# patrikhuber/superviseddescent

Hardware: AMD Instinct MI355X
Metric: faces/sec RCR-22 detect (batch 4096) (higher is better)
Workload: dtype f32; 1 GPU; RCR-22 detect, batch 4096 synthetic 256x256 u8 faces per GPU, 4 cascade levels (UoCTTI HOG 5x5 cells, cell 11/10/8/6, 4 orientations, F=8801, M=44), model trained on-GPU on 100000 synthetic faces (shipped .bin absent from the reference checkout); batch_per_gpu=4096, levels=4

## Files before the change

include/sdm.h:

```cpp
#ifndef SDM_H_
#define SDM_H_

#include <stddef.h>
#include <stdint.h>

#ifdef __cplusplus
extern "C" {
#endif

#define SDM_OK 0
#define SDM_ERR_INVALID (-1)
#define SDM_ERR_NO_DEVICE (-2)
#define SDM_ERR_HIP (-3)
#define SDM_ERR_EMPTY_PATCH (-4)
#define SDM_ERR_NOT_SPD (-5)
#define SDM_ERR_COMM (-6)

#define SDM_VARIANT_DALALTRIGGS 0
#define SDM_VARIANT_UOCTTI 1

#define SDM_REG_MANUAL 0
#define SDM_REG_MATRIX_NORM 1

typedef struct sdm_hog_param {
// ... 68 lines not shown
typedef int (*sdm_allreduce_fn)(void* dev_ptr, size_t count_f32, void* hip_stream, void* user);
int sdm_set_allreduce(sdm_ctx* ctx, sdm_allreduce_fn fn, void* user, int world_size);
int sdm_set_allreduce_rccl(sdm_ctx* ctx, void* nccl_comm, void* nccl_allreduce_fn, int world_size);
int sdm_allreduce_gram_rhs(sdm_ctx* ctx);
typedef int (*sdm_bcast_fn)(void* dev_ptr, size_t count_f32, int root, void* hip_stream, void* user);
typedef int (*sdm_allgather_fn)(const void* send_ptr, void* recv_ptr, size_t count_f32, void* hip_stream, void* user);
int sdm_set_solve_sharding(sdm_ctx* ctx, int rank, int world_size, sdm_bcast_fn bcast, sdm_allgather_fn allgather, void* user);
int sdm_set_solve_sharding_rccl(sdm_ctx* ctx, void* nccl_comm, int rank, int world_size, void* nccl_broadcast_fn,
                                void* nccl_allgather_fn);
typedef int (*sdm_reduce_scatter_fn)(const void* send_ptr, void* recv_ptr, size_t count_f32, void* hip_stream, void* user);
int sdm_set_reduce_scatter(sdm_ctx* ctx, sdm_reduce_scatter_fn fn, void* user);
int sdm_set_reduce_scatter_rccl(sdm_ctx* ctx, int enable, void* nccl_reduce_scatter_fn);
int sdm_solve(sdm_ctx* ctx, int level, int reg_type, float reg_param, int regularise_last_row,
              long long n_train_global, float* R_host, float* lambda_out);
#define SDM_SOLVER_CHOLESKY 0
#define SDM_SOLVER_COLPIV_QR 1
int sdm_set_solver(sdm_ctx* ctx, int solver);
int sdm_last_rank(sdm_ctx* ctx, int* rank, int* full_rank);
int sdm_solve_normal_equations(sdm_ctx* ctx, const float* A_host, int n_rows, int n_features,
                               const float* b_host, int n_outputs, int reg_type, float reg_param,
                               int regularise_last_row, float* R_host, float* lambda_out);
int sdm_solve_normal_equations_with(sdm_ctx* ctx, int solver, const float* A_host, int n_rows, int n_features,
                                    const float* b_host, int n_outputs, int reg_type, float reg_param,
                                    int regularise_last_row, float* R_host, float* lambda_out, int* rank, int* full_rank);
int sdm_train_level(sdm_ctx* ctx, int level, int reg_type, float reg_param, int regularise_last_row,
                    long long n_train_global);

int sdm_train_level_sweep(sdm_ctx* ctx, int level, int reg_type, const float* reg_params, int K, int regularise_last_row,
                          long long n_train_global, int n_fit_rows, double* holdout_err , double* fit_err ,
                          float* lambdas , int* status , int* best);
int sdm_sweep_get_regressor(sdm_ctx* ctx, int k, float* R_host);

int sdm_gram_device_ptr(sdm_ctx* ctx, void** dev_ptr, size_t* count_f32);
int sdm_x_device_ptr(sdm_ctx* ctx, void** dev_ptr, size_t* count_f32);
int sdm_features_device_ptr(sdm_ctx* ctx, void** dev_ptr, long long* ld, int* n_rows);

int sdm_enable_timing(sdm_ctx* ctx, int on);
int sdm_get_timing(sdm_ctx* ctx, float* ms , int* launches , int reset);

int sdm_debug_patch(sdm_ctx* ctx, int level, int sample, int landmark, uint8_t* resized_SxS,
                    uint8_t* bins_SxS, float* hist_2OxCxC, float* desc_P);
int sdm_debug_hog_profile(sdm_ctx* ctx, int level, unsigned long long* out8);
int sdm_debug_gradient_table(sdm_ctx* ctx, int level, float* g_511x511, int* bin_511x511);
int sdm_debug_set_option(sdm_ctx* ctx, const char* name, int value);
int sdm_debug_update_f16(sdm_ctx* ctx, const float* P_host, int rows, int wcols, int wcols_factor, float factor_bound, float* C_host);
int sdm_debug_download_images(sdm_ctx* ctx, uint8_t* out, int n, int width, int height);
int sdm_debug_set_hog_packing(sdm_ctx* ctx, int on);
int sdm_debug_gram_fallbacks(sdm_ctx* ctx);
int sdm_debug_update_fallbacks(sdm_ctx* ctx);
int sdm_debug_hog_plan(int num_cells, int cell_size, int num_bins, int num_landmarks, int* info5, unsigned* lane_tab,
                       float* wb, int* pass_info, int max_passes);
int sdm_debug_hog_plan_cut(int num_cells, int cell_size, int num_bins, int num_landmarks, int* cut);
int sdm_debug_hog_taps(sdm_ctx* ctx, int level, int* table, int* info3);
int sdm_debug_set_detect_path(sdm_ctx* ctx, int fused, int split_store);

int sdm_pose_set_model(sdm_ctx* ctx, const float* points, int K, float focal, float width, float height, float near_, float far_);
int sdm_pose_set_x(sdm_ctx* ctx, const float* x_host, int n_samples);
int sdm_pose_get_x(sdm_ctx* ctx, float* x_host);
int sdm_pose_set_x_device(sdm_ctx* ctx, const float* x_dev, int n_samples);
int sdm_pose_set_templates(sdm_ctx* ctx, const float* templates, int n_samples, int feature_dim);
int sdm_pose_templates_from_landmarks(sdm_ctx* ctx, const int* landmark_index, int K, float focal);
int sdm_pose_set_targets(sdm_ctx* ctx, const float* xstar_host, int n_samples);
int sdm_pose_features(sdm_ctx* ctx, int level, float* out_host);
int sdm_pose_train_level(sdm_ctx* ctx, int level, int reg_type, float reg_param, int regularise_last_row, float* R_host, float* lambda_out);
int sdm_pose_set_regressor(sdm_ctx* ctx, int level, const float* R_host);
int sdm_pose_get_regressor(sdm_ctx* ctx, int level, float* R_host);
int sdm_pose_test(sdm_ctx* ctx, int first_level, int n_levels);

#define SDM_TRACK_FREE 0
#define SDM_TRACK_STARTED 1
#define SDM_TRACK_TRACKED 2
#define SDM_TRACK_LOST 3
#define SDM_TRACK_INIT_PREVIOUS 0
#define SDM_TRACK_INIT_REALIGN 1
#define SDM_TRACK_LOST_NONFINITE 1
#define SDM_TRACK_LOST_SMALL 2
#define SDM_TRACK_LOST_OUTSIDE 4
#define SDM_TRACK_LOST_SCALE 8
int sdm_track_configure(sdm_ctx* ctx, int capacity, const float* mean, int init_mode, float min_size, float max_scale_change);
int sdm_track_start(sdm_ctx* ctx, const int* ids, const int* boxes, int n);
int sdm_track_stop(sdm_ctx* ctx, const int* ids, int n);
int sdm_track_step(sdm_ctx* ctx, const int* ids, int n, float* landmarks_host, int* lost_host);
int sdm_track_get(sdm_ctx* ctx, const int* ids, int n, float* landmarks_host, int* status_host);

#define SDM_ALIGN_DEGENERATE 1
#define SDM_ALIGN_PARTIAL 2
int sdm_align_set_source(sdm_ctx* ctx, const uint8_t* base, int n_images, int width, int height, int stride_bytes, int channels,
                         int on_device);
int sdm_align_crops(sdm_ctx* ctx, const int* landmark_index, const float* template_xy, int K, int out_width, int out_height,
                    uint8_t* out, int out_on_device, float* matrices_host, int* flags_host);

#ifdef __cplusplus
}
#endif
#endif
```

superviseddescent_amd/_lib.py:

```python
from __future__ import annotations

import ctypes
import os

_HERE = os.path.dirname(os.path.abspath(__file__))
LIB_PATH = os.environ.get("SDM_HIP_LIB") or os.path.join(_HERE, "lib", "libsdm_hip.so")

SDM_OK = 0
SDM_ERR_INVALID, SDM_ERR_NO_DEVICE, SDM_ERR_HIP, SDM_ERR_EMPTY_PATCH, SDM_ERR_NOT_SPD, SDM_ERR_COMM = \
    -1, -2, -3, -4, -5, -6
SDM_T_HOG, SDM_T_APPLY, SDM_T_GRAM, SDM_T_REG, SDM_T_FACTOR, SDM_T_BACKSOLVE, SDM_T_ALLREDUCE = range(7)
SDM_T_COUNT = 8
SDM_HOG_EXACT_ORDER, SDM_HOG_FAST, SDM_HOG_COLUMNS = 0, 1, 2
TIMING_NAMES = ["hog", "apply", "gram", "reg", "factor_solve", "backsolve", "allreduce", "_"]

EXPORTED = [
    "sdm_last_error", "sdm_device_count", "sdm_create", "sdm_destroy", "sdm_set_stream", "sdm_synchronize",
    "sdm_set_model_geometry", "sdm_set_hog_mode", "sdm_get_hog_info", "sdm_feature_dim", "sdm_upload_images_u8", "sdm_set_images_device",
    "sdm_set_sample_image_index", "sdm_set_x", "sdm_get_x", "sdm_set_x_device", "sdm_get_x_device",
    "sdm_hog_features", "sdm_get_patch_indices", "sdm_set_regressor", "sdm_get_regressor", "sdm_apply",
    "sdm_detect_batch", "sdm_detect_level", "sdm_set_targets", "sdm_gram_rhs", "sdm_set_allreduce", "sdm_set_allreduce_rccl", "sdm_allreduce_gram_rhs",
    "sdm_set_solve_sharding", "sdm_set_solve_sharding_rccl", "sdm_set_reduce_scatter", "sdm_set_reduce_scatter_rccl",
    "sdm_set_templates", "sdm_init_from_boxes", "sdm_normalised_errors", "sdm_solve", "sdm_set_solver", "sdm_last_rank", "sdm_solve_normal_equations", "sdm_solve_normal_equations_with", "sdm_train_level", "sdm_gram_device_ptr", "sdm_x_device_ptr", "sdm_features_device_ptr",
    "sdm_enable_timing", "sdm_get_timing", "sdm_debug_patch", "sdm_debug_hog_profile", "sdm_debug_gradient_table", "sdm_debug_update_f16", "sdm_debug_set_option",
    "sdm_debug_set_hog_packing", "sdm_debug_gram_fallbacks", "sdm_debug_update_fallbacks", "sdm_debug_hog_plan", "sdm_debug_hog_plan_cut", "sdm_debug_hog_taps", "sdm_debug_set_detect_path", "sdm_upload_images_bgr_u8", "sdm_debug_download_images",
    "sdm_pose_set_model", "sdm_pose_set_x", "sdm_pose_get_x", "sdm_pose_set_x_device", "sdm_pose_set_templates",
    "sdm_pose_templates_from_landmarks", "sdm_pose_set_targets", "sdm_pose_features", "sdm_pose_train_level",
    "sdm_pose_set_regressor", "sdm_pose_get_regressor", "sdm_pose_test",
    "sdm_track_configure", "sdm_track_start", "sdm_track_stop", "sdm_track_step", "sdm_track_get",
    "sdm_align_set_source", "sdm_align_crops",
    "sdm_train_level_sweep", "sdm_sweep_get_regressor",
]

SDM_TRACK_FREE, SDM_TRACK_STARTED, SDM_TRACK_TRACKED, SDM_TRACK_LOST = 0, 1, 2, 3
SDM_TRACK_INIT_PREVIOUS, SDM_TRACK_INIT_REALIGN = 0, 1
SDM_TRACK_LOST_NONFINITE, SDM_TRACK_LOST_SMALL, SDM_TRACK_LOST_OUTSIDE, SDM_TRACK_LOST_SCALE = 1, 2, 4, 8

SDM_ALIGN_DEGENERATE, SDM_ALIGN_PARTIAL = 1, 2


class SdmHogParam(ctypes.Structure):

    _fields_ = [("variant", ctypes.c_int), ("num_cells", ctypes.c_int), ("cell_size", ctypes.c_int),
                ("num_bins", ctypes.c_int), ("relative_patch_size", ctypes.c_float)]


ALLREDUCE_FN = ctypes.CFUNCTYPE(ctypes.c_int, ctypes.c_void_p, ctypes.c_size_t, ctypes.c_void_p,
                                ctypes.c_void_p)
BCAST_FN = ctypes.CFUNCTYPE(ctypes.c_int, ctypes.c_void_p, ctypes.c_size_t, ctypes.c_int, ctypes.c_void_p, ctypes.c_void_p)
ALLGATHER_FN = ctypes.CFUNCTYPE(ctypes.c_int, ctypes.c_void_p, ctypes.c_void_p, ctypes.c_size_t, ctypes.c_void_p, ctypes.c_void_p)

_LIB = None


class SdmError(RuntimeError):

    def __init__(self, code: int, msg: str):
        super().__init__(f"sdm error {code}: {msg}")
        self.code = code


def _share_hip_runtime_with_torch() -> None:
    import importlib.util
    import sys
    if "torch" in sys.modules:
        return
    try:
        spec = importlib.util.find_spec("torch")
    except (ImportError, ValueError):
        spec = None
    if spec is None or not spec.origin:
        return
    cand = os.path.join(os.path.dirname(spec.origin), "lib", "libamdhip64.so")
    if os.path.exists(cand):
        try:
            ctypes.CDLL(cand, mode=ctypes.RTLD_GLOBAL)
        except OSError:
            pass
# ... 26 lines not shown
            "sdm_upload_images_u8": [c_void_p, ctypes.POINTER(c_void_p), c_int_p, c_int_p, c_int_p, c_int],
            "sdm_set_images_device": [c_void_p, c_void_p, c_int, c_int, c_int, c_int],
            "sdm_upload_images_bgr_u8": [c_void_p, ctypes.POINTER(c_void_p), c_int_p, c_int_p, c_int_p, c_int, c_int],
            "sdm_debug_download_images": [c_void_p, c_void_p, c_int, c_int, c_int],
            "sdm_set_sample_image_index": [c_void_p, c_int_p, c_int],
            "sdm_set_x": [c_void_p, c_float_p, c_int],
            "sdm_get_x": [c_void_p, c_float_p],
            "sdm_set_x_device": [c_void_p, c_void_p, c_int],
            "sdm_get_x_device": [c_void_p, c_void_p],
            "sdm_hog_features": [c_void_p, c_int, c_float_p],
            "sdm_get_patch_indices": [c_void_p, c_int_p],
            "sdm_set_regressor": [c_void_p, c_int, c_float_p],
            "sdm_get_regressor": [c_void_p, c_int, c_float_p],
            "sdm_apply": [c_void_p, c_int],
            "sdm_detect_batch": [c_void_p, c_float_p],
            "sdm_detect_level": [c_void_p, c_int],
            "sdm_set_targets": [c_void_p, c_float_p, c_int],
            "sdm_gram_rhs": [c_void_p, c_int],
            "sdm_set_allreduce": [c_void_p, ALLREDUCE_FN, c_void_p, c_int],
            "sdm_allreduce_gram_rhs": [c_void_p],
            "sdm_set_allreduce_rccl": [c_void_p, c_void_p, c_void_p, c_int],
            "sdm_set_solve_sharding": [c_void_p, c_int, c_int, BCAST_FN, ALLGATHER_FN, c_void_p],
            "sdm_set_solve_sharding_rccl": [c_void_p, c_void_p, c_int, c_int, c_void_p, c_void_p],
            "sdm_set_reduce_scatter": [c_void_p, ALLGATHER_FN, c_void_p],
            "sdm_set_reduce_scatter_rccl": [c_void_p, c_int, c_void_p],
            "sdm_solve": [c_void_p, c_int, c_int, ctypes.c_float, c_int, ctypes.c_longlong, c_float_p, c_float_p],
            "sdm_train_level": [c_void_p, c_int, c_int, ctypes.c_float, c_int, ctypes.c_longlong],
            "sdm_set_solver": [c_void_p, c_int],
            "sdm_last_rank": [c_void_p, c_int_p, c_int_p],
            "sdm_solve_normal_equations": [c_void_p, c_float_p, c_int, c_int, c_float_p, c_int, c_int, ctypes.c_float, c_int,
                                           c_float_p, c_float_p],
            "sdm_solve_normal_equations_with": [c_void_p, c_int, c_float_p, c_int, c_int, c_float_p, c_int, c_int, ctypes.c_float, c_int,
                                                c_float_p, c_float_p, c_int_p, c_int_p],
            "sdm_set_templates": [c_void_p, c_void_p, c_int, c_int],
            "sdm_init_from_boxes": [c_void_p, c_void_p, c_void_p, c_void_p, c_int, c_void_p],
            "sdm_normalised_errors": [c_void_p, c_void_p, ctypes.POINTER(ctypes.c_double)],
            "sdm_gram_device_ptr": [c_void_p, ctypes.POINTER(c_void_p), ctypes.POINTER(ctypes.c_size_t)],
            "sdm_x_device_ptr": [c_void_p, ctypes.POINTER(c_void_p), ctypes.POINTER(ctypes.c_size_t)],
            "sdm_features_device_ptr": [c_void_p, ctypes.POINTER(c_void_p), ctypes.POINTER(ctypes.c_longlong), c_int_p],
            "sdm_enable_timing": [c_void_p, c_int],
            "sdm_get_timing": [c_void_p, c_float_p, c_int_p, c_int],
            "sdm_debug_patch": [c_void_p, c_int, c_int, c_int, ctypes.POINTER(ctypes.c_uint8),
                                ctypes.POINTER(ctypes.c_uint8), c_float_p, c_float_p],
            "sdm_debug_gradient_table": [c_void_p, c_int, c_float_p, c_int_p],
            "sdm_debug_set_option": [c_void_p, ctypes.c_char_p, c_int],
            "sdm_debug_update_f16": [c_void_p, c_float_p, c_int, c_int, c_int, ctypes.c_float, c_float_p],
            "sdm_debug_hog_profile": [c_void_p, c_int, ctypes.POINTER(ctypes.c_ulonglong)],
            "sdm_debug_set_hog_packing": [c_void_p, c_int],
            "sdm_debug_gram_fallbacks": [c_void_p],
            "sdm_debug_update_fallbacks": [c_void_p],
            "sdm_debug_hog_plan": [c_int, c_int, c_int, c_int, c_int_p, c_void_p, c_void_p, c_void_p, c_int],
            "sdm_debug_hog_plan_cut": [c_int, c_int, c_int, c_int, c_int_p],
            "sdm_debug_hog_taps": [c_void_p, c_int, c_int_p, c_int_p],
            "sdm_debug_set_detect_path": [c_void_p, c_int, c_int],
            "sdm_pose_set_model": [c_void_p, c_void_p, c_int, ctypes.c_float, ctypes.c_float, ctypes.c_float, ctypes.c_float,
                                   ctypes.c_float],
            "sdm_pose_set_x": [c_void_p, c_void_p, c_int],
            "sdm_pose_get_x": [c_void_p, c_void_p],
            "sdm_pose_set_x_device": [c_void_p, c_void_p, c_int],
            "sdm_pose_set_templates": [c_void_p, c_void_p, c_int, c_int],
            "sdm_pose_templates_from_landmarks": [c_void_p, c_void_p, c_int, ctypes.c_float],
            "sdm_pose_set_targets": [c_void_p, c_void_p, c_int],
            "sdm_pose_features": [c_void_p, c_int, c_void_p],
            "sdm_pose_train_level": [c_void_p, c_int, c_int, ctypes.c_float, c_int, c_void_p, c_float_p],
            "sdm_pose_set_regressor": [c_void_p, c_int, c_void_p],
            "sdm_pose_get_regressor": [c_void_p, c_int, c_void_p],
            "sdm_pose_test": [c_void_p, c_int, c_int],
            "sdm_track_configure": [c_void_p, c_int, c_void_p, c_int, ctypes.c_float, ctypes.c_float],
            "sdm_track_start": [c_void_p, c_void_p, c_void_p, c_int],
            "sdm_track_stop": [c_void_p, c_void_p, c_int],
            "sdm_track_step": [c_void_p, c_void_p, c_int, c_void_p, c_void_p],
            "sdm_track_get": [c_void_p, c_void_p, c_int, c_void_p, c_void_p],
            "sdm_align_set_source": [c_void_p, c_void_p, c_int, c_int, c_int, c_int, c_int, c_int],
            "sdm_align_crops": [c_void_p, c_void_p, c_void_p, c_int, c_int, c_int, c_void_p, c_int, c_void_p, c_void_p],
            "sdm_train_level_sweep": [c_void_p, c_int, c_int, c_void_p, c_int, c_int, ctypes.c_longlong, c_int, c_void_p, c_void_p,
                                      c_void_p, c_void_p, c_int_p],
            "sdm_sweep_get_regressor": [c_void_p, c_int, c_float_p],
        }
        for name, args in sigs.items():
            fn = getattr(L, name)
            fn.argtypes = args
            fn.restype = c_int
        L.sdm_device_count.restype = c_int
        _LIB = L
    return _LIB


def check(rc: int) -> int:
    if rc < 0:
        raise SdmError(rc, lib().sdm_last_error().decode("utf-8", "replace"))
    return rc
```

superviseddescent_amd/csrc/sdm_apply.hip:

```cpp
#include "sdm_kernels.h"
#include <stdlib.h>

#pragma clang fp contract(off)
#include "sdm_ied.h"

namespace {

typedef float f32x4 __attribute__((ext_vector_type(4)));

#define APPLY_WAVES 4

template <int RT, int NT>
__global__ void __launch_bounds__(APPLY_WAVES * 64)
apply_partial_kernel(const float* __restrict__ feat, long long ldf, int N, int kgroups,
                     const float* __restrict__ Rt, long long ldr, float* __restrict__ partial, int splits)
{
    __shared__ float red[APPLY_WAVES - 1][RT * NT][4][64];
    const int lane = threadIdx.x & 63, wave = threadIdx.x >> 6;
    const int li = lane & 15, lq = lane >> 4;
    const int row0 = blockIdx.x * (16 * RT);
    const int split = blockIdx.y;
    const int g0 = (int)(((long long)kgroups * split) / splits);
    const int g1 = (int)(((long long)kgroups * (split + 1)) / splits);

    f32x4 acc[RT][NT];
#pragma unroll
    for (int r = 0; r < RT; ++r)
#pragma unroll
        for (int c = 0; c < NT; ++c) acc[r][c] = (f32x4){0.f, 0.f, 0.f, 0.f};

    const float* arow[RT];
#pragma unroll
    for (int r = 0; r < RT; ++r) {
        int row = row0 + 16 * r + li;
        if (row > N - 1) row = N - 1;
        arow[r] = feat + (long long)row * ldf + 4 * lq;
    }
    const float* brow[NT];
#pragma unroll
    for (int c = 0; c < NT; ++c) brow[c] = Rt + (long long)(16 * c + li) * ldr + 4 * lq;

    f32x4 a[RT], b[NT], an[RT], bn[NT];
    int g = g0 + wave;
    if (g < g1) {
        const long long k0 = (long long)g * 16;
#pragma unroll
        for (int r = 0; r < RT; ++r) a[r] = *(const f32x4*)(arow[r] + k0);
#pragma unroll
        for (int c = 0; c < NT; ++c) b[c] = *(const f32x4*)(brow[c] + k0);
    }
    for (; g < g1; g += APPLY_WAVES) {
        const int gn = g + APPLY_WAVES;
        if (gn < g1) {
            const long long k1 = (long long)gn * 16;
#pragma unroll
            for (int r = 0; r < RT; ++r) an[r] = *(const f32x4*)(arow[r] + k1);
#pragma unroll
// ... 229 lines not shown
    const float* row = Rt + (long long)blockIdx.x * ldr;
    float v = 0.0f;
    for (long long i = threadIdx.x; i < ldr; i += 256) v = __builtin_fmaxf(v, __builtin_fabsf(row[i]));
    for (int o = 32; o; o >>= 1) v = __builtin_fmaxf(v, __shfl_xor(v, o));
    if ((threadIdx.x & 63) == 0) part[threadIdx.x >> 6] = v;
    __syncthreads();
    if (threadIdx.x == 0) out[blockIdx.x] = __builtin_bit_cast(unsigned, __builtin_fmaxf(__builtin_fmaxf(part[0], part[1]), __builtin_fmaxf(part[2], part[3])));
}

__global__ void __launch_bounds__(256) apply_planes_kernel(const float* __restrict__ Rt, long long ldr, int Mp, int KG, af16x8* __restrict__ planes,
                                                           const unsigned* __restrict__ rmax)
{
    const long long u = (long long)blockIdx.x * 256 + threadIdx.x;
    if (u >= (long long)KG * Mp) return;
    const int kg = (int)(u / Mp), col = (int)(u % Mp);
    const float scale = __builtin_ldexpf(1.0f, 14 - apply_f16_exponent(rmax[col]));
    const float* src = Rt + (long long)col * ldr + 8 * kg;
    af16x8 p1, p2;
#pragma unroll
    for (int j = 0; j < 8; ++j) {
        const float v = src[j] * scale;
        const _Float16 h1 = (_Float16)v;
        p1[j] = h1; p2[j] = (_Float16)(v - (float)h1);
    }
    planes[u] = p1; planes[(size_t)KG * Mp + u] = p2;
}

__global__ void apply_reduce_kernel(const float* __restrict__ partial, int splits, int N, int Mp, int M,
                                    const float* __restrict__ x_in, float* __restrict__ x_out, int L,
                                    EyeIdxDev eyes)
{
    const long long t = (long long)blockIdx.x * blockDim.x + threadIdx.x;
    if (t >= (long long)N * M) return;
    const int row = (int)(t / M), col = (int)(t - (long long)row * M);
    const float* xr = x_in + (long long)row * M;
    const float xc = xr[col];
    float scale = 1.0f;
    if (eyes.nre > 0) {
        const float n = (float)(1.0 / device_ied_rows(xr, L, eyes));
        scale = 1.0f / n;
    }
    float u = 0.0f;
    const float* pp = partial + (long long)row * Mp + col;
    const long long sstride = (long long)N * Mp;
    constexpr int RB = 24;
    for (int s0 = 0; s0 < splits; s0 += RB) {
        float v[RB];
#pragma unroll
        for (int j = 0; j < RB; ++j) v[j] = pp[(long long)(s0 + j < splits ? s0 + j : splits - 1) * sstride];
#pragma unroll
        for (int j = 0; j < RB; ++j) u = s0 + j < splits ? u + v[j] : u;
    }
    x_out[t] = xc - u * scale;
}

__global__ void targets_kernel(const float* __restrict__ x, const float* __restrict__ xstar, int N, int L,
                               EyeIdxDev eyes, float* __restrict__ feat, long long ldf, int bcol0)
{
    const int M = 2 * L;
    const long long t = (long long)blockIdx.x * blockDim.x + threadIdx.x;
    if (t >= (long long)N * M) return;
    const int row = (int)(t / M), col = (int)(t - (long long)row * M);
    const float* xr = x + (long long)row * M;
    float n = 1.0f;
    if (eyes.nre > 0) n = (float)(1.0 / device_ied_rows(xr, L, eyes));
    feat[(long long)row * ldf + bcol0 + col] = (xr[col] - xstar[t]) * n;
}

__global__ void pack_regressor_kernel(const float* __restrict__ Rsol, int F, int M, int Mp, float* __restrict__ Rt,
                                      long long ldf, float* __restrict__ Rc)
{
    const long long t = (long long)blockIdx.x * blockDim.x + threadIdx.x;
    if (t >= (long long)Mp * ldf) return;
    const int j = (int)(t / ldf);
    const long long k = t - (long long)j * ldf;
    const float v = (k < F && j < M) ? Rsol[k * Mp + j] : 0.0f;
    Rt[t] = v;
    if (Rc && k < F && j < M) Rc[k * M + j] = v;
}

__global__ void subtract_templates_kernel(float* __restrict__ feat, long long ldf, const float* __restrict__ tmpl, int N, int F)
{
    const long long t = (long long)blockIdx.x * blockDim.x + threadIdx.x;
    if (t >= (long long)N * F) return;
    const int row = (int)(t / F), col = (int)(t - (long long)row * F);
    feat[(long long)row * ldf + col] -= tmpl[t];
}

__global__ void init_boxes_kernel(const float* __restrict__ mean, const int* __restrict__ boxes,
                                  const float* __restrict__ pert, int N, int L, float* __restrict__ x)
{
    const int M = 2 * L;
    const long long t = (long long)blockIdx.x * blockDim.x + threadIdx.x;
    if (t >= (long long)N * M) return;
    const int row = (int)(t / M), col = (int)(t - (long long)row * M);
    int bx = boxes[4 * row], by = boxes[4 * row + 1], bw = boxes[4 * row + 2], bh = boxes[4 * row + 3];
    if (pert) {
        const float tx = pert[3 * row], ty = pert[3 * row + 1], sc = pert[3 * row + 2];
        const float tx_pixel = tx * (float)bw, ty_pixel = ty * (float)bh;
        const float pw = (float)bw * sc, ph = (float)bh * sc;
        const float nx = (float)bx + ((float)bw - pw) / 2.0f + tx_pixel;
        const float ny = (float)by + ((float)bh - ph) / 2.0f + ty_pixel;
        bx = (int)nx; by = (int)ny; bw = (int)pw; bh = (int)ph;
    }
    const float m = mean[col];
    x[t] = col < L ? (m * 1.0f + 0.5f + 0.0f) * (float)bw + (float)bx
// ... 169 lines not shown
        if (planes && rmax) {
            static unsigned long long attr16 = 0;
            if (sdm_first_use_on_device(attr16)) {
#define AFATTR(...) SDM_SET_ATTR((const void*)apply_tiled_f16_kernel<__VA_ARGS__>, hipFuncAttributeMaxDynamicSharedMemorySize, 160 * 1024)
                AFATTR(1, 64); AFATTR(2, 64); AFATTR(3, 64); AFATTR(1, 128); AFATTR(2, 128); AFATTR(3, 128); AFATTR(4, 128); AFATTR(5, 128); AFATTR(6, 128); AFATTR(7, 128); AFATTR(8, 128); AFATTR(9, 128);
#undef AFATTR
            }
#define AFL(...) hipLaunchKernelGGL((apply_tiled_f16_kernel<__VA_ARGS__>), grid, dim3(bm * 4), lds, stream, feat, ldf, N, kslabs, \
                                    (const f32x4*)planes, (int)(ldr / 8), rmax, partial, splits)
            switch (NT) {
                case 1: if (bm == 128) AFL(1, 128); else AFL(1, 64); break;
                case 2: if (bm == 128) AFL(2, 128); else AFL(2, 64); break;
                case 3: if (bm == 128) AFL(3, 128); else AFL(3, 64); break;
                case 4: AFL(4, 128); break; case 5: AFL(5, 128); break; case 6: AFL(6, 128); break;
                case 7: AFL(7, 128); break; case 8: AFL(8, 128); break; default: AFL(9, 128); break;
            }
#undef AFL
        } else {
#define ATL(...) hipLaunchKernelGGL((apply_tiled_kernel<__VA_ARGS__>), grid, dim3(bm * 4), lds, stream, feat, ldf, N, kslabs, Rt, ldr, partial, splits)
        switch (NT) {
            case 1: ATL(1); break; case 2: ATL(2); break; case 3: ATL(3); break;
            case 4: ATL(4, 128); break; case 5: ATL(5, 128); break; case 6: ATL(6, 128); break;
            case 7: ATL(7, 128); break; case 8: ATL(8, 128); break; default: ATL(9, 128); break;
        }
#undef ATL
        }
    } else
    switch (NT) {
        case 1: launch_partial<2, 1>(feat, ldf, N, kgroups, Rt, ldr, partial, splits, stream); break;
        case 2: launch_partial<2, 2>(feat, ldf, N, kgroups, Rt, ldr, partial, splits, stream); break;
        case 3: launch_partial<2, 3>(feat, ldf, N, kgroups, Rt, ldr, partial, splits, stream); break;
        case 4: launch_partial<2, 4>(feat, ldf, N, kgroups, Rt, ldr, partial, splits, stream); break;
        case 5: launch_partial<2, 5>(feat, ldf, N, kgroups, Rt, ldr, partial, splits, stream); break;
        case 6: launch_partial<2, 6>(feat, ldf, N, kgroups, Rt, ldr, partial, splits, stream); break;
        case 7: launch_partial<2, 7>(feat, ldf, N, kgroups, Rt, ldr, partial, splits, stream); break;
        case 8: launch_partial<2, 8>(feat, ldf, N, kgroups, Rt, ldr, partial, splits, stream); break;
        case 9: launch_partial<2, 9>(feat, ldf, N, kgroups, Rt, ldr, partial, splits, stream); break;
        default: return;
    }
    const long long total = (long long)N * M;
    hipLaunchKernelGGL(apply_reduce_kernel, dim3((unsigned)((total + 255) / 256)), dim3(256), 0, stream,
                       partial, splits, N, NT * 16, M, x_in, x_out, L, eyes);
}

void sdm_launch_apply_reduce(const float* partial, int splits, int N, int M, const float* x_in, float* x_out, int L,
                             const EyeIdxDev& eyes, hipStream_t stream)
{
    const long long total = (long long)N * M;
    if (total <= 0) return;
    hipLaunchKernelGGL(apply_reduce_kernel, dim3((unsigned)((total + 255) / 256)), dim3(256), 0, stream,
                       partial, splits, N, ((M + 15) / 16) * 16, M, x_in, x_out, L, eyes);
}

void sdm_launch_targets(const float* x, const float* xstar, int N, int L, const EyeIdxDev& eyes,
                        float* feat, long long ldf, int bcol0, hipStream_t stream)
{
    const long long total = (long long)N * 2 * L;
    if (total <= 0) return;
    hipLaunchKernelGGL(targets_kernel, dim3((unsigned)((total + 255) / 256)), dim3(256), 0, stream, x, xstar,
                       N, L, eyes, feat, ldf, bcol0);
}
```

superviseddescent_amd/csrc/sdm_capi_align.hip:

```cpp
#include "sdm_capi_internal.h"

#include <cmath>

extern "C" {

int sdm_align_set_source(sdm_ctx* c, const uint8_t* base, int n_images, int width, int height, int stride_bytes, int channels,
                         int on_device)
{
    if (!c) return fail(SDM_ERR_INVALID, "null context");
    sdm_ctx::Align& a = c->align;
    if (!base) { a.base = nullptr; a.n = 0; a.C = 1; return SDM_OK; }
    if (n_images < 1 || width < 1 || height < 1) return fail(SDM_ERR_INVALID, "an image stack needs n_images, width and height >= 1");
    if (channels != 1 && channels != 3 && channels != 4) return fail(SDM_ERR_INVALID, "channels must be 1, 3 or 4");
    if ((long long)stride_bytes < (long long)width * channels) return fail(SDM_ERR_INVALID, "stride_bytes < width * channels");
    HIP_TRY(hipSetDevice(c->device));
    const uint8_t* dev = base;
    if (!on_device) {
        const size_t bytes = ((size_t)n_images * height - 1) * (size_t)stride_bytes + (size_t)width * channels;
        if (a.base == a.owned.p) { a.base = nullptr; a.n = 0; a.C = 1; }
        int rc = a.owned.ensure(bytes);
        if (rc) return rc;
        HIP_TRY(hipMemcpyAsync(a.owned.p, base, bytes, hipMemcpyHostToDevice, c->stream));
        HIP_TRY(hipStreamSynchronize(c->stream));
        dev = a.owned.p;
// ... 8 lines not shown
    if (!c) return fail(SDM_ERR_INVALID, "null context");
    if (c->L <= 0) return fail(SDM_ERR_INVALID, "geometry not set");
    const int L = c->L, N = c->N;
    if (N < 1) return fail(SDM_ERR_INVALID, "no current rows (sdm_set_x, sdm_detect_batch or sdm_track_step first)");
    if (!lm || !tmpl) return fail(SDM_ERR_INVALID, "no landmark indices or template");
    if (K < 2 || K > L) return fail(SDM_ERR_INVALID, "K must be in [2, L]");
    std::vector<char> seen(L, 0);
    for (int k = 0; k < K; ++k) {
        if (lm[k] < 0 || lm[k] >= L) return fail(SDM_ERR_INVALID, "landmark index " + std::to_string(lm[k]) + " out of range");
        if (seen[lm[k]]) return fail(SDM_ERR_INVALID, "landmark index " + std::to_string(lm[k]) + " named twice");
        seen[lm[k]] = 1;
    }
    bool spread = false;
    for (int k = 0; k < 2 * K; ++k)
        if (!std::isfinite(tmpl[k])) return fail(SDM_ERR_INVALID, "a template point is not finite");
    for (int k = 1; k < K && !spread; ++k) spread = tmpl[2 * k] != tmpl[0] || tmpl[2 * k + 1] != tmpl[1];
    if (!spread) return fail(SDM_ERR_INVALID, "the K template points coincide");
    if (out_w < 1 || out_w > 1024 || out_h < 1 || out_h > 1024) return fail(SDM_ERR_INVALID, "crop width and height must be in [1, 1024]");
    sdm_ctx::Align& a = c->align;
    const bool external = a.base != nullptr;
    const int C = external ? a.C : 1;
    if (!out) return fail(SDM_ERR_INVALID, "no output");
    if (out_on_device && ((uintptr_t)out % (C == 4 ? 16 : 4)) != 0)
        return fail(SDM_ERR_INVALID, "a device output must be 4-byte aligned (16 when C = 4)");
    if (!c->img_base || c->n_images < 1) return fail(SDM_ERR_INVALID, "no images set");
    const int n_src = external ? std::min(a.n, c->n_images) : c->n_images;
    if (c->idx_identity && N > n_src) return fail(SDM_ERR_INVALID, "more rows than source images and no sample->image index set");
    if (!c->idx_identity && N > c->n_idx) return fail(SDM_ERR_INVALID, "sample->image index is shorter than the rows");
    for (int r = 0; r < N; ++r) {
        const int im = c->idx_identity ? r : c->img_idx_host[r];
        if (im >= n_src) return fail(SDM_ERR_INVALID, "row " + std::to_string(r) + " maps to image " + std::to_string(im) + ", beyond the source");
        if (external && (c->img_w_host[im] != a.w || c->img_h_host[im] != a.h))
            return fail(SDM_ERR_INVALID, "the source stack's image size differs from image " + std::to_string(im) + " of the context");
    }
    HIP_TRY(hipSetDevice(c->device));
    const size_t crop_bytes = (size_t)N * out_w * out_h * C;
    int rc;
    if ((rc = a.in.ensure((size_t)3 * K)) || (rc = a.faces.ensure((size_t)N)) || (!out_on_device && (rc = a.crops.ensure(crop_bytes))))
        return rc;
    std::vector<int> in((size_t)3 * K);
    memcpy(in.data(), lm, (size_t)K * sizeof(int));
    memcpy(in.data() + K, tmpl, (size_t)2 * K * sizeof(float));
    HIP_TRY(hipMemcpyAsync(a.in.p, in.data(), in.size() * sizeof(int), hipMemcpyHostToDevice, c->stream));
    AlignSourceDev src{};
    const uint8_t* img;
    if (external) {
        src.ctx.base = nullptr;
        src.width = a.w; src.height = a.h; src.stride = a.stride;
        img = a.base;
    } else {
        src.ctx = image_set(c);
        img = c->img_base;
    }
    sdm_launch_align_fit(c->x[c->cur].p, N, L, a.in.p, (const float*)(a.in.p + K), K, src, c->idx_identity ? nullptr : c->img_idx.p,
                         out_w, out_h, a.faces.p, c->stream);
    HIP_TRY(hipGetLastError());
    uint8_t* dst = out_on_device ? out : a.crops.p;
    sdm_launch_align_warp(img, a.faces.p, N, out_w, out_h, C, dst, c->stream);
    HIP_TRY(hipGetLastError());
    std::vector<AlignFace> faces;
    if (matrices_host || flags_host) {
        faces.resize((size_t)N);
        HIP_TRY(hipMemcpyAsync(faces.data(), a.faces.p, (size_t)N * sizeof(AlignFace), hipMemcpyDeviceToHost, c->stream));
    }
    if (!out_on_device) HIP_TRY(hipMemcpyAsync(out, a.crops.p, crop_bytes, hipMemcpyDeviceToHost, c->stream));
    HIP_TRY(hipStreamSynchronize(c->stream));
    for (int r = 0; r < (int)faces.size(); ++r) {
        if (matrices_host) memcpy(matrices_host + (size_t)6 * r, faces[r].m, 6 * sizeof(float));
        if (flags_host) flags_host[r] = faces[r].flags;
    }
    return SDM_OK;
}

}
```

superviseddescent_amd/csrc/sdm_capi_context.hip:

```cpp
#include "sdm_capi_internal.h"

extern "C" {

const char* sdm_last_error(void) { return err_string().c_str(); }

int sdm_device_count(void)
{
    int n = 0;
    if (hipGetDeviceCount(&n) != hipSuccess) return 0;
    return n;
}

sdm_ctx* sdm_create(int device)
{
    int n = 0;
    if (hipGetDeviceCount(&n) != hipSuccess || n <= 0) {
        fail(SDM_ERR_NO_DEVICE, "no HIP device available: this engine has no CPU fallback");
        return nullptr;
    }
    if (device < 0 || device >= n) { fail(SDM_ERR_INVALID, "device index out of range"); return nullptr; }
    hipDeviceProp_t prop;
    if (hipGetDeviceProperties(&prop, device) != hipSuccess) { fail(SDM_ERR_HIP, "hipGetDeviceProperties failed"); return nullptr; }
    if (strncmp(prop.gcnArchName, "gfx950", 6) != 0) {
        fail(SDM_ERR_NO_DEVICE, std::string("device is ") + prop.gcnArchName + ", kernels are built for gfx950 only");
        return nullptr;
    }
    if (hipSetDevice(device) != hipSuccess) { fail(SDM_ERR_HIP, "hipSetDevice failed"); return nullptr; }
    sdm_ctx* c = new sdm_ctx();
    c->device = device;
    if (hipStreamCreateWithFlags(&c->stream, hipStreamNonBlocking) != hipSuccess) {
        fail(SDM_ERR_HIP, "hipStreamCreate failed"); delete c; return nullptr;
    }
    c->own_stream = true;
    int prio_least = 0, prio_greatest = 0;
    (void)hipDeviceGetStreamPriorityRange(&prio_least, &prio_greatest);
    if (hipStreamCreateWithPriority(&c->solve_aux.stream, hipStreamNonBlocking, prio_least) != hipSuccess ||
        hipEventCreateWithFlags(&c->solve_aux.chain_done, hipEventDisableTiming) != hipSuccess ||
        hipEventCreateWithFlags(&c->solve_aux.tail_done, hipEventDisableTiming) != hipSuccess) {
        fail(SDM_ERR_HIP, "hipStreamCreate failed"); delete c; return nullptr;
    }
    if (c->status.ensure(1, true, c->stream) || c->lambda_dev.ensure(1, true, c->stream)) { delete c; return nullptr; }
    for (int b = 0; b < sdm_ctx::XBLOCKS_MAX; ++b)
        if (hipEventCreateWithFlags(&c->gram_ev[b], hipEventDisableTiming) != hipSuccess) { fail(SDM_ERR_HIP, "hipEventCreate failed"); delete c; return nullptr; }
    if (hipEventCreateWithFlags(&c->gram_xdone, hipEventDisableTiming) != hipSuccess) { fail(SDM_ERR_HIP, "hipEventCreate failed"); delete c; return nullptr; }
    return c;
}

void sdm_destroy(sdm_ctx* c)
{
    if (!c) return;
    hipError_t e = hipSetDevice(c->device); (void)e;
    e = hipStreamSynchronize(c->stream);
    if (c->solve_aux.stream) {
        e = hipStreamSynchronize(c->solve_aux.stream);
        e = hipEventDestroy(c->solve_aux.chain_done); e = hipEventDestroy(c->solve_aux.tail_done);
        for (int b = 0; b < sdm_ctx::XBLOCKS_MAX; ++b) if (c->gram_ev[b]) e = hipEventDestroy(c->gram_ev[b]);
        if (c->gram_xdone) e = hipEventDestroy(c->gram_xdone);
        e = hipStreamDestroy(c->solve_aux.stream);
    }
    drain_timing(c);
    for (auto ev : c->pool) { e = hipEventDestroy(ev); }
    c->img_owned.release(); c->img_off.release(); c->img_w.release(); c->img_h.release();
    c->img_stride.release(); c->img_idx.release(); c->x[0].release(); c->x[1].release();
    c->xstar.release(); c->tmpl.release(); c->feat.release(); c->patch_idx.release(); c->status.release();
    c->partial.release(); c->shard_stage.release(); c->G.release(); c->gpack.release(); c->fro.release(); c->Rsol.release(); c->winv.release(); c->gram_planes.release(); c->gram_flag.release(); c->upd_planes.release(); c->upd_maxdiag.release(); c->lambda_dev.release();
    for (auto& r : c->Rp) r.release();
    for (auto& r : c->Rd) r.release();
    c->cells.release(); c->qr_work.release();
    c->Rmax.release();
    c->pose.release();
    c->track.release();
    c->align.release();
    c->sweep.release();
    for (auto& r : c->Rt) r.release();
    for (auto& q : c->plans) { q.lane_tab.release(); q.wb.release(); q.wb16.release(); q.pass_info.release(); q.cut.release(); q.taps.release(); }
    if (c->own_stream) e = hipStreamDestroy(c->stream);
    delete c;
}

int sdm_set_stream(sdm_ctx* c, void* hip_stream)
{
    if (!c) return fail(SDM_ERR_INVALID, "null context");
    HIP_TRY(hipStreamSynchronize(c->stream));
    if (c->own_stream) { HIP_TRY(hipStreamDestroy(c->stream)); c->own_stream = false; }
    c->stream = (hipStream_t)hip_stream;
    return SDM_OK;
}

int sdm_synchronize(sdm_ctx* c)
{
    if (!c) return fail(SDM_ERR_INVALID, "null context");
    HIP_TRY(hipStreamSynchronize(c->stream));
    drain_timing(c);
    return SDM_OK;
}

int sdm_set_model_geometry(sdm_ctx* c, int L, const int* re, int nre, const int* le, int nle, int n_levels,
                           const sdm_hog_param* levels)
{
    if (!c) return fail(SDM_ERR_INVALID, "null context");
    if (L <= 0 || n_levels <= 0 || !levels) return fail(SDM_ERR_INVALID, "bad geometry");
    if (nre < 0 || nle < 0 || nre > SDM_MAX_EYE || nle > SDM_MAX_EYE || ((nre == 0) != (nle == 0)))
        return fail(SDM_ERR_INVALID, "eye index lists must both be empty or hold 1..4 entries each");
    if (2 * L > 144) return fail(SDM_ERR_INVALID, "at most 72 landmarks (2L <= 144) supported");
    for (int i = 0; i < nre; ++i) if (re[i] < 0 || re[i] >= L) return fail(SDM_ERR_INVALID, "right eye index out of range");
    for (int i = 0; i < nle; ++i) if (le[i] < 0 || le[i] >= L) return fail(SDM_ERR_INVALID, "left eye index out of range");
    if (c->L == L && (int)c->params.size() == n_levels && c->eyes.nre == nre && c->eyes.nle == nle) {
        bool same = true;
        for (int i = 0; i < nre && same; ++i) same = c->eyes.re[i] == re[i];
        for (int i = 0; i < nle && same; ++i) same = c->eyes.le[i] == le[i];
        for (int l = 0; l < n_levels && same; ++l)
            same = c->params[l].variant == levels[l].variant && c->params[l].num_cells == levels[l].num_cells &&
                   c->params[l].cell_size == levels[l].cell_size && c->params[l].num_bins == levels[l].num_bins &&
                   c->params[l].relative_patch_size == levels[l].relative_patch_size;
        if (same) return SDM_OK;
    }
// ... 57 lines not shown
                verdict = mism[1] == 0 ? 2 : (mism[0] == 0 ? 1 : 0);
                raw_ok = (mism[2] == 0 && (lv.O != 4 || mism[3] == 0)) ? 1 : 0;
            }
            n_fast_bins.push_back(verdict);
            n_raw_sqrt.push_back(raw_ok);
            n_fast_kernel.push_back(sdm_hog_fast_supported(lv) ? 1 : 0);
        }
        const int F = L * lv.P + (lv.fixed_h > 0 ? 0 : 1);
        if (F > Fmax) Fmax = F;
    }
    std::vector<sdm_ctx::Plan> n_plans(n_levels);
    struct PlanGuard {
        std::vector<sdm_ctx::Plan>& v;
        ~PlanGuard() { for (auto& q : v) { q.lane_tab.release(); q.wb.release(); q.wb16.release(); q.pass_info.release(); q.cut.release(); q.taps.release(); } }
    } plan_guard{n_plans};
    for (int l = 0; l < n_levels; ++l) {
        HogPlanHost hp;
        if (!n_fast_kernel[l] || n_fast_bins[l] != 2 || !sdm_hog_plan_build(n_levels_dev[l], L, hp)) continue;
        sdm_ctx::Plan& pl = n_plans[l];
        int rcp;
        if ((rcp = pl.lane_tab.ensure(hp.lane_tab.size())) || (rcp = pl.wb.ensure(hp.wb.size())) || (rcp = pl.wb16.ensure(hp.wb16.size())) ||
            (rcp = pl.pass_info.ensure(hp.pass_info.size())) || (rcp = pl.cut.ensure(hp.cut.size())))
            return rcp;
        HIP_TRY(hipMemcpyAsync(pl.cut.p, hp.cut.data(), hp.cut.size() * sizeof(int), hipMemcpyHostToDevice, c->stream));
        if ((rcp = pl.taps.ensure((size_t)SDM_SCALE_TAB * 64 * 8))) return rcp;
        sdm_launch_taps_table(n_levels_dev[l], pl.taps.p, c->stream);
        HIP_TRY(hipMemcpyAsync(pl.lane_tab.p, hp.lane_tab.data(), hp.lane_tab.size() * sizeof(unsigned), hipMemcpyHostToDevice, c->stream));
        HIP_TRY(hipMemcpyAsync(pl.wb.p, hp.wb.data(), hp.wb.size() * sizeof(float), hipMemcpyHostToDevice, c->stream));
        HIP_TRY(hipMemcpyAsync(pl.wb16.p, hp.wb16.data(), hp.wb16.size() * sizeof(unsigned short), hipMemcpyHostToDevice, c->stream));
        HIP_TRY(hipMemcpyAsync(pl.pass_info.p, hp.pass_info.data(), hp.pass_info.size() * sizeof(int), hipMemcpyHostToDevice, c->stream));
        HIP_TRY(hipStreamSynchronize(c->stream));
        pl.dev.G = hp.G; pl.dev.P = hp.P; pl.dev.n_main = hp.n_main; pl.dev.Gt = hp.Gt; pl.dev.Pt = hp.Pt; pl.dev.hist_slots = hp.hist_slots;
        pl.dev.raw_sqrt = n_raw_sqrt[l];
        pl.dev.lane_tab = pl.lane_tab.p; pl.dev.wb = pl.wb.p; pl.dev.wb16 = pl.wb16.p; pl.dev.pass_info = pl.pass_info.p; pl.dev.taps = pl.taps.p;
        pl.ok = true;
    }
    c->plans.swap(n_plans);
    c->L = L; c->M = 2 * L;
    c->eyes = eyes;
    c->levels.swap(n_levels_dev); c->params.swap(n_params); c->fast_kernel.swap(n_fast_kernel); c->fast_bins.swap(n_fast_bins);
    c->Fmax = Fmax;
    c->rhs_tiles = (round_up(c->M, 16) + 127) / 128;
    c->ldf = (long long)round_up(c->Fmax, 128) + 128 * c->rhs_tiles;
    for (auto& r : c->Rt) r.release();
    c->Rt.assign(n_levels, DevBuf<float>());
    for (auto& r : c->Rp) r.release();
    c->Rp.assign(n_levels, DevBuf<unsigned char>());
    for (auto& r : c->Rd) r.release();
    c->Rd.assign(n_levels, DevBuf<unsigned char>());
    c->cells.release();
    c->have_R.assign(n_levels, false);
    c->feat.release(); c->feat_level = -1; c->feat_wide_F = 0; c->feat_wide_N = 0; c->have_patch_idx = false;
    c->N = 0; c->have_targets = false; c->g_level = -1;
    c->sweep.K = 0; c->sweep.level = -1; c->sweep.ok = 0;
    return SDM_OK;
}

int sdm_set_hog_mode(sdm_ctx* c, int mode)
{
    if (!c || (mode != SDM_HOG_EXACT_ORDER && mode != SDM_HOG_FAST && mode != SDM_HOG_COLUMNS)) return fail(SDM_ERR_INVALID, "bad HOG mode");
    c->hog_mode = mode;
    return SDM_OK;
}

int sdm_get_hog_info(sdm_ctx* c, int level, int* fast_kernel, int* fast_bins)
{
    if (!c || level < 0 || level >= (int)c->levels.size()) return fail(SDM_ERR_INVALID, "bad level");
    if (fast_kernel) *fast_kernel = c->fast_kernel[level];
    if (fast_bins) *fast_bins = c->fast_bins[level];
    return SDM_OK;
}

int sdm_feature_dim(const sdm_ctx* c, int level)
{
    if (!c || level < 0 || level >= (int)c->levels.size()) return fail(SDM_ERR_INVALID, "bad level");
    return level_F(c, level);
}

int sdm_upload_images_u8(sdm_ctx* c, const uint8_t* const* images, const int* w, const int* h,
                         const int* stride, int n)
{
    if (!c || !images || n <= 0) return fail(SDM_ERR_INVALID, "bad image list");
    HIP_TRY(hipSetDevice(c->device));
    std::vector<long long> off(n);
    long long total = 0;
    for (int i = 0; i < n; ++i) {
        if (w[i] <= 0 || h[i] <= 0 || stride[i] < w[i]) return fail(SDM_ERR_INVALID, "bad image size");
        off[i] = total;
        total += (long long)w[i] * h[i];
    }
    int rc;
    if ((rc = c->img_owned.ensure((size_t)total))) return rc;
    if ((rc = c->img_off.ensure(n)) || (rc = c->img_w.ensure(n)) || (rc = c->img_h.ensure(n)) || (rc = c->img_stride.ensure(n)))
        return rc;
    bool contiguous = true;
    for (int i = 0; i < n && contiguous; ++i)
        contiguous = stride[i] == w[i] && images[i] == images[0] + off[i];
    if (contiguous) {
        HIP_TRY(hipMemcpyAsync(c->img_owned.p, images[0], (size_t)total, hipMemcpyHostToDevice, c->stream));
    } else {
        for (int i = 0; i < n; ++i)
            HIP_TRY(hipMemcpy2DAsync(c->img_owned.p + off[i], w[i], images[i], stride[i], w[i], h[i],
                                     hipMemcpyHostToDevice, c->stream));
    }
    std::vector<int> dense(w, w + n);
    HIP_TRY(hipMemcpyAsync(c->img_off.p, off.data(), n * sizeof(long long), hipMemcpyHostToDevice, c->stream));
    HIP_TRY(hipMemcpyAsync(c->img_w.p, w, n * sizeof(int), hipMemcpyHostToDevice, c->stream));
    HIP_TRY(hipMemcpyAsync(c->img_h.p, h, n * sizeof(int), hipMemcpyHostToDevice, c->stream));
    HIP_TRY(hipMemcpyAsync(c->img_stride.p, dense.data(), n * sizeof(int), hipMemcpyHostToDevice, c->stream));
    HIP_TRY(hipStreamSynchronize(c->stream));
    c->img_base = c->img_owned.p;
    c->n_images = n;
    c->img_w_host.assign(w, w + n); c->img_h_host.assign(h, h + n);
    c->narrow_images = false;
    for (int i = 0; i < n; ++i) c->narrow_images = c->narrow_images || w[i] < 2 || h[i] > 65535;
    return SDM_OK;
}

int sdm_upload_images_bgr_u8(sdm_ctx* c, const uint8_t* const* images, const int* w, const int* h, const int* stride, int n,
                             int gray_shift)
{
    if (!c || !images || n <= 0) return fail(SDM_ERR_INVALID, "bad image list");
    if (gray_shift != 14 && gray_shift != 15) return fail(SDM_ERR_INVALID, "gray_shift must be 14 (OpenCV 2.4 - 3.x) or 15");
    HIP_TRY(hipSetDevice(c->device));
    std::vector<long long> off(n);
    long long total = 0;
    for (int i = 0; i < n; ++i) {
        if (w[i] <= 0 || h[i] <= 0 || stride[i] < 3 * w[i]) return fail(SDM_ERR_INVALID, "bad image size");
        off[i] = total;
        total += (long long)w[i] * h[i];
    }
    int rc;
    ScopedBuf<uint8_t> staging;
    if ((rc = staging.ensure((size_t)total * 3 + 16))) return rc;
    if ((rc = c->img_owned.ensure((size_t)total + 16))) return rc;
    if ((rc = c->img_off.ensure(n)) || (rc = c->img_w.ensure(n)) || (rc = c->img_h.ensure(n)) || (rc = c->img_stride.ensure(n)))
        return rc;
    bool contiguous = true;
    for (int i = 0; i < n && contiguous; ++i)
        contiguous = stride[i] == 3 * w[i] && images[i] == images[0] + 3 * off[i];
    if (contiguous) {
        HIP_TRY(hipMemcpyAsync(staging.p, images[0], (size_t)total * 3, hipMemcpyHostToDevice, c->stream));
    } else {
        for (int i = 0; i < n; ++i)
            HIP_TRY(hipMemcpy2DAsync(staging.p + 3 * off[i], (size_t)3 * w[i], images[i], stride[i], (size_t)3 * w[i], h[i],
                                     hipMemcpyHostToDevice, c->stream));
    }
    sdm_launch_bgr2gray(staging.p, c->img_owned.p, total, gray_shift, c->stream);
    HIP_TRY(hipGetLastError());
    std::vector<int> dense(w, w + n);
    HIP_TRY(hipMemcpyAsync(c->img_off.p, off.data(), n * sizeof(long long), hipMemcpyHostToDevice, c->stream));
    HIP_TRY(hipMemcpyAsync(c->img_w.p, w, n * sizeof(int), hipMemcpyHostToDevice, c->stream));
    HIP_TRY(hipMemcpyAsync(c->img_h.p, h, n * sizeof(int), hipMemcpyHostToDevice, c->stream));
    HIP_TRY(hipMemcpyAsync(c->img_stride.p, dense.data(), n * sizeof(int), hipMemcpyHostToDevice, c->stream));
    HIP_TRY(hipStreamSynchronize(c->stream));
    staging.release();
    c->img_base = c->img_owned.p;
    c->n_images = n;
    c->img_w_host.assign(w, w + n); c->img_h_host.assign(h, h + n);
    c->narrow_images = false;
    for (int i = 0; i < n; ++i) c->narrow_images = c->narrow_images || w[i] < 2 || h[i] > 65535;
    return SDM_OK;
}

int sdm_debug_download_images(sdm_ctx* c, uint8_t* out, int n, int w, int h)
{
    if (!c || !out || n <= 0 || n > c->n_images || w <= 0 || h <= 0) return fail(SDM_ERR_INVALID, "bad arguments");
    if (c->img_base != c->img_owned.p) return fail(SDM_ERR_INVALID, "the image set is not owned by the context");
    HIP_TRY(hipMemcpyAsync(out, c->img_owned.p, (size_t)n * w * h, hipMemcpyDeviceToHost, c->stream));
    HIP_TRY(hipStreamSynchronize(c->stream));
    return SDM_OK;
}

int sdm_set_images_device(sdm_ctx* c, const uint8_t* dev_base, int n, int w, int h, int stride)
{
    if (!c || !dev_base || n <= 0 || w <= 0 || h <= 0 || stride < w) return fail(SDM_ERR_INVALID, "bad device image stack");
    HIP_TRY(hipSetDevice(c->device));
    int rc;
    if ((rc = c->img_off.ensure(n)) || (rc = c->img_w.ensure(n)) || (rc = c->img_h.ensure(n)) || (rc = c->img_stride.ensure(n)))
        return rc;
    std::vector<long long> off(n);
    std::vector<int> vw(n, w), vh(n, h), vs(n, stride);
    for (int i = 0; i < n; ++i) off[i] = (long long)i * h * stride;
    HIP_TRY(hipMemcpyAsync(c->img_off.p, off.data(), n * sizeof(long long), hipMemcpyHostToDevice, c->stream));
    HIP_TRY(hipMemcpyAsync(c->img_w.p, vw.data(), n * sizeof(int), hipMemcpyHostToDevice, c->stream));
    HIP_TRY(hipMemcpyAsync(c->img_h.p, vh.data(), n * sizeof(int), hipMemcpyHostToDevice, c->stream));
    HIP_TRY(hipMemcpyAsync(c->img_stride.p, vs.data(), n * sizeof(int), hipMemcpyHostToDevice, c->stream));
    HIP_TRY(hipStreamSynchronize(c->stream));
    c->img_base = dev_base;
    c->n_images = n;
    c->img_w_host.assign(n, w); c->img_h_host.assign(n, h);
    c->narrow_images = w < 2 || h > 65535;
    return SDM_OK;
}

int sdm_set_sample_image_index(sdm_ctx* c, const int* idx, int n)
{
    if (!c) return fail(SDM_ERR_INVALID, "null context");
    if (!idx) { c->idx_identity = true; c->n_idx = 0; c->max_idx = -1; return SDM_OK; }
    if (n <= 0) return fail(SDM_ERR_INVALID, "bad sample count");
    int mx = -1;
    for (int i = 0; i < n; ++i) {
        if (idx[i] < 0 || (c->n_images > 0 && idx[i] >= c->n_images)) return fail(SDM_ERR_INVALID, "image index out of range");
        if (idx[i] > mx) mx = idx[i];
    }
    HIP_TRY(hipSetDevice(c->device));
    int rc = c->img_idx.ensure(n);
    if (rc) return rc;
    HIP_TRY(hipMemcpyAsync(c->img_idx.p, idx, n * sizeof(int), hipMemcpyHostToDevice, c->stream));
    HIP_TRY(hipStreamSynchronize(c->stream));
    c->idx_identity = false; c->n_idx = n; c->max_idx = mx;
    c->img_idx_host.assign(idx, idx + n);
    return SDM_OK;
}

static int set_x_common(sdm_ctx* c, const float* x, int N, hipMemcpyKind kind)
{
    if (!c || !x || N <= 0) return fail(SDM_ERR_INVALID, "bad x");
    if (c->L <= 0) return fail(SDM_ERR_INVALID, "geometry not set");
    HIP_TRY(hipSetDevice(c->device));
    int rc = ensure_sample_buffers(c, N);
    if (rc) return rc;
    if (N != c->N) { c->have_targets = false; c->feat_level = -1; c->have_patch_idx = false; }
    c->N = N; c->cur = 0;
    HIP_TRY(hipMemcpyAsync(c->x[0].p, x, (size_t)N * c->M * sizeof(float), kind, c->stream));
    if (kind == hipMemcpyHostToDevice) HIP_TRY(hipStreamSynchronize(c->stream));
    return SDM_OK;
}

int sdm_set_x(sdm_ctx* c, const float* x, int N) { return set_x_common(c, x, N, hipMemcpyHostToDevice); }
int sdm_set_x_device(sdm_ctx* c, const float* x, int N) { return set_x_common(c, x, N, hipMemcpyDeviceToDevice); }

int sdm_set_templates(sdm_ctx* c, const float* templates, int n_samples, int feature_dim)
{
    if (!c) return fail(SDM_ERR_INVALID, "null context");
    if (!templates) { c->tmpl_N = 0; c->tmpl_F = 0; return SDM_OK; }
    if (n_samples <= 0 || feature_dim <= 0) return fail(SDM_ERR_INVALID, "bad template matrix");
    HIP_TRY(hipSetDevice(c->device));
    int rc = c->tmpl.ensure((size_t)n_samples * feature_dim);
    if (rc) return rc;
    HIP_TRY(hipMemcpyAsync(c->tmpl.p, templates, (size_t)n_samples * feature_dim * sizeof(float), hipMemcpyHostToDevice, c->stream));
    HIP_TRY(hipStreamSynchronize(c->stream));
    c->tmpl_N = n_samples; c->tmpl_F = feature_dim;
    return SDM_OK;
}

int sdm_init_from_boxes(sdm_ctx* c, const float* mean, const int* boxes, const float* perturbations, int N, float* x_host)
{
    if (!c || !mean || !boxes || N <= 0) return fail(SDM_ERR_INVALID, "bad initialisation arguments");
    if (c->L <= 0) return fail(SDM_ERR_INVALID, "geometry not set");
    HIP_TRY(hipSetDevice(c->device));
    int rc = ensure_sample_buffers(c, N);
    if (rc) return rc;
    ScopedBuf<float> d_mean, d_pert;
    ScopedBuf<int> d_box;
    if ((rc = d_mean.ensure(c->M)) || (rc = d_box.ensure((size_t)4 * N))) return rc;
    if (perturbations && (rc = d_pert.ensure((size_t)3 * N))) return rc;
    HIP_TRY(hipMemcpyAsync(d_mean.p, mean, c->M * sizeof(float), hipMemcpyHostToDevice, c->stream));
    HIP_TRY(hipMemcpyAsync(d_box.p, boxes, (size_t)4 * N * sizeof(int), hipMemcpyHostToDevice, c->stream));
    if (perturbations)
        HIP_TRY(hipMemcpyAsync(d_pert.p, perturbations, (size_t)3 * N * sizeof(float), hipMemcpyHostToDevice, c->stream));
    if (N != c->N) { c->have_targets = false; c->feat_level = -1; c->have_patch_idx = false; }
    c->N = N; c->cur = 0;
    sdm_launch_init_boxes(d_mean.p, d_box.p, perturbations ? d_pert.p : nullptr, N, c->L, c->x[0].p, c->stream);
    HIP_TRY(hipGetLastError());
    if (x_host)
        HIP_TRY(hipMemcpyAsync(x_host, c->x[0].p, (size_t)N * c->M * sizeof(float), hipMemcpyDeviceToHost, c->stream));
    HIP_TRY(hipStreamSynchronize(c->stream));
    d_mean.release(); d_box.release(); d_pert.release();
    return SDM_OK;
}

int sdm_normalised_errors(sdm_ctx* c, float* errors_host, double* mean_out)
{
    if (!c || c->N <= 0) return fail(SDM_ERR_INVALID, "no x to evaluate");
    if (!c->have_targets) return fail(SDM_ERR_INVALID, "sdm_normalised_errors: no targets set");
    if (c->eyes.nre <= 0 || c->eyes.nle <= 0) return fail(SDM_ERR_INVALID, "sdm_normalised_errors: no eye landmarks");
    HIP_TRY(hipSetDevice(c->device));
    ScopedBuf<float> d_err;
    ScopedBuf<double> d_work;
    int rc;
    if ((rc = d_err.ensure((size_t)c->N * c->L)) || (rc = d_work.ensure(SDM_SUM_PARTS + 2))) return rc;
    sdm_launch_landmark_errors(c->x[c->cur].p, c->xstar.p, c->N, c->L, c->eyes, d_err.p, d_work.p, c->stream);
    HIP_TRY(hipGetLastError());
    double res[2] = {0.0, 0.0};
    HIP_TRY(hipMemcpyAsync(res, d_work.p + SDM_SUM_PARTS, 2 * sizeof(double), hipMemcpyDeviceToHost, c->stream));
    if (errors_host)
        HIP_TRY(hipMemcpyAsync(errors_host, d_err.p, (size_t)c->N * c->L * sizeof(float), hipMemcpyDeviceToHost, c->stream));
    HIP_TRY(hipStreamSynchronize(c->stream));
    d_err.release(); d_work.release();
    if (mean_out) *mean_out = res[1];
    return SDM_OK;
}

int sdm_get_x(sdm_ctx* c, float* x)
{
    if (!c || !x || c->N <= 0) return fail(SDM_ERR_INVALID, "no x to get");
    HIP_TRY(hipMemcpyAsync(x, c->x[c->cur].p, (size_t)c->N * c->M * sizeof(float), hipMemcpyDeviceToHost, c->stream));
    HIP_TRY(hipStreamSynchronize(c->stream));
    return check_status(c);
}

int sdm_get_x_device(sdm_ctx* c, float* x)
{
    if (!c || !x || c->N <= 0) return fail(SDM_ERR_INVALID, "no x to get");
    HIP_TRY(hipMemcpyAsync(x, c->x[c->cur].p, (size_t)c->N * c->M * sizeof(float), hipMemcpyDeviceToDevice, c->stream));
    return SDM_OK;
}


}
```

superviseddescent_amd/csrc/sdm_capi_debug.hip:

```cpp
#include "sdm_capi_internal.h"

extern "C" {

int sdm_gram_device_ptr(sdm_ctx* c, void** p, size_t* count)
{
    if (!c || c->g_level < 0) return fail(SDM_ERR_INVALID, "no Gram matrix");
    *p = c->G.p; *count = (size_t)c->g_fp * c->g_ncols;
    return SDM_OK;
}

int sdm_x_device_ptr(sdm_ctx* c, void** p, size_t* count)
{
    if (!c || c->N <= 0) return fail(SDM_ERR_INVALID, "no x");
    *p = c->x[c->cur].p; *count = (size_t)c->N * c->M;
    return SDM_OK;
}

int sdm_features_device_ptr(sdm_ctx* c, void** p, long long* ld, int* n_rows)
{
    if (!c || c->feat_level < 0) return fail(SDM_ERR_INVALID, "no features");
    *p = c->feat.p; *ld = c->ldf; *n_rows = c->N;
    c->feat_bounded = false;
    return SDM_OK;
}

int sdm_enable_timing(sdm_ctx* c, int on)
{
    if (!c) return fail(SDM_ERR_INVALID, "null context");
    c->timing = on != 0;
    return SDM_OK;
}

int sdm_get_timing(sdm_ctx* c, float* ms, int* launches, int reset)
{
    if (!c) return fail(SDM_ERR_INVALID, "null context");
    HIP_TRY(hipStreamSynchronize(c->stream));
    drain_timing(c);
    for (int i = 0; i < SDM_T_COUNT; ++i) {
        if (ms) ms[i] = c->t_ms[i];
        if (launches) launches[i] = c->t_n[i];
        if (reset) { c->t_ms[i] = 0.f; c->t_n[i] = 0; }
    }
    return SDM_OK;
}

int sdm_debug_patch(sdm_ctx* c, int level, int sample, int landmark, uint8_t* rsz, uint8_t* bins, float* hist, float* desc)
{
    if (!c || level < 0 || level >= (int)c->levels.size()) return fail(SDM_ERR_INVALID, "bad level");
    if (sample < 0 || sample >= c->N || landmark < 0 || landmark >= c->L) return fail(SDM_ERR_INVALID, "bad patch");
    if (!c->img_base) return fail(SDM_ERR_INVALID, "no images set");
    { const int rci = check_sample_index(c); if (rci) return rci; }
    HIP_TRY(hipSetDevice(c->device));
    const HogLevelDev& lv = c->levels[level];
    const size_t nS = (size_t)lv.S * lv.S, nH = (size_t)2 * lv.O * lv.C * lv.C, nP = lv.P;
    ScopedBuf<uint8_t> d_r, d_b; ScopedBuf<float> d_h, d_d;
    int rc;
    if ((rc = d_r.ensure(nS)) || (rc = d_b.ensure(nS)) || (rc = d_h.ensure(nH)) || (rc = d_d.ensure(nP))) return rc;
    sdm_launch_hog_debug(image_set(c), c->idx_identity ? nullptr : c->img_idx.p, c->x[c->cur].p, c->N, c->L,
                         c->eyes, lv, sample, landmark, d_r.p, d_b.p, d_h.p, d_d.p, c->status.p, c->stream);
    HIP_TRY(hipGetLastError());
    if (rsz) HIP_TRY(hipMemcpyAsync(rsz, d_r.p, nS, hipMemcpyDeviceToHost, c->stream));
    if (bins) HIP_TRY(hipMemcpyAsync(bins, d_b.p, nS, hipMemcpyDeviceToHost, c->stream));
    if (hist) HIP_TRY(hipMemcpyAsync(hist, d_h.p, nH * sizeof(float), hipMemcpyDeviceToHost, c->stream));
    if (desc) HIP_TRY(hipMemcpyAsync(desc, d_d.p, nP * sizeof(float), hipMemcpyDeviceToHost, c->stream));
    HIP_TRY(hipStreamSynchronize(c->stream));
    d_r.release(); d_b.release(); d_h.release(); d_d.release();
    return SDM_OK;
}

int sdm_debug_hog_profile(sdm_ctx* c, int level, unsigned long long* out8)
{
    if (!c || level < 0 || level >= (int)c->levels.size() || !out8) return fail(SDM_ERR_INVALID, "bad arguments");
    if (!c->img_base || c->N <= 0) return fail(SDM_ERR_INVALID, "no images / samples set");
    { const int rci = check_sample_index(c); if (rci) return rci; }
    HIP_TRY(hipSetDevice(c->device));
    ScopedBuf<unsigned long long> d;
    int rc = d.ensure(8, true, c->stream);
    if (rc) return rc;
    sdm_launch_hog_fast_profile(image_set(c), c->idx_identity ? nullptr : c->img_idx.p, c->x[c->cur].p, c->N, c->L,
                                c->eyes, c->levels[level], c->feat.p, c->ldf, c->status.p, d.p, c->stream);
    HIP_TRY(hipGetLastError());
    HIP_TRY(hipMemcpyAsync(out8, d.p, 8 * sizeof(unsigned long long), hipMemcpyDeviceToHost, c->stream));
    HIP_TRY(hipStreamSynchronize(c->stream));
    d.release();
    c->feat_level = level;
    if (level_F(c, level) > c->feat_wide_F) c->feat_wide_F = level_F(c, level);
    if (c->N > c->feat_wide_N) c->feat_wide_N = c->N;
    return SDM_OK;
}

int sdm_debug_gram_fallbacks(sdm_ctx* c)
{
    if (!c) return fail(SDM_ERR_INVALID, "null context");
    return c->gram_fallbacks;
}

int sdm_debug_update_fallbacks(sdm_ctx* c)
{
    if (!c) return fail(SDM_ERR_INVALID, "null context");
    return c->update_range_fallbacks;
}

int sdm_debug_set_hog_packing(sdm_ctx* c, int on)
{
    if (!c) return fail(SDM_ERR_INVALID, "null context");
    c->packing = on != 0;
    return SDM_OK;
}

int sdm_debug_hog_plan(int num_cells, int cell_size, int num_bins, int num_landmarks, int* info5, unsigned* lane_tab,
                       float* wb, int* pass_info, int max_passes)
{
    HogLevelDev lv;
    memset(&lv, 0, sizeof(lv));
    lv.variant = SDM_VARIANT_UOCTTI; lv.C = num_cells; lv.cell = cell_size; lv.O = num_bins; lv.S = num_cells * cell_size;
    fill_row_tab(lv);
    HogPlanHost hp;
    if (!info5) return fail(SDM_ERR_INVALID, "bad arguments");
    if (!sdm_hog_plan_build(lv, num_landmarks, hp)) { info5[0] = 0; return SDM_OK; }
    info5[0] = hp.G; info5[1] = hp.P; info5[2] = hp.n_main; info5[3] = hp.Gt; info5[4] = hp.Pt;
    const int np = hp.P + hp.Pt;
    if (np > max_passes) return fail(SDM_ERR_INVALID, "plan has more passes than the output buffers hold");
    if (lane_tab) memcpy(lane_tab, hp.lane_tab.data(), hp.lane_tab.size() * sizeof(unsigned));
    if (wb) memcpy(wb, hp.wb.data(), hp.wb.size() * sizeof(float));
    if (pass_info) memcpy(pass_info, hp.pass_info.data(), hp.pass_info.size() * sizeof(int));
    return SDM_OK;
}

int sdm_debug_hog_plan_cut(int num_cells, int cell_size, int num_bins, int num_landmarks, int* cut)
{
    if (!cut || num_landmarks <= 0) return fail(SDM_ERR_INVALID, "bad arguments");
    HogLevelDev lv;
    memset(&lv, 0, sizeof(lv));
    lv.variant = SDM_VARIANT_UOCTTI; lv.C = num_cells; lv.cell = cell_size; lv.O = num_bins; lv.S = num_cells * cell_size;
    fill_row_tab(lv);
    HogPlanHost hp;
    if (!sdm_hog_plan_build(lv, num_landmarks, hp)) return fail(SDM_ERR_INVALID, "no packed instance for this geometry");
    memcpy(cut, hp.cut.data(), (size_t)num_landmarks * sizeof(int));
    return SDM_OK;
}

int sdm_debug_hog_taps(sdm_ctx* c, int level, int* table, int* info3)
{
    if (!c || level < 0 || level >= (int)c->levels.size() || !table || !info3) return fail(SDM_ERR_INVALID, "bad arguments");
    if (!c->plans[level].ok || !c->plans[level].taps.p) return fail(SDM_ERR_INVALID, "no packed plan for this level");
    HIP_TRY(hipSetDevice(c->device));
    HIP_TRY(hipMemcpyAsync(table, c->plans[level].taps.p, (size_t)SDM_SCALE_TAB * 64 * 8 * sizeof(int), hipMemcpyDeviceToHost, c->stream));
    HIP_TRY(hipStreamSynchronize(c->stream));
    info3[0] = split_ok(c, level) ? 1 : 0;
    info3[1] = sdm_hog_cells_row_carry(c->levels[level], c->plans[level].dev) ? 1 : 0;
    info3[2] = c->hog_two_load ? 1 : 0;
    return SDM_OK;
}

int sdm_debug_set_detect_path(sdm_ctx* c, int fused, int split_store)
{
    if (!c) return fail(SDM_ERR_INVALID, "null context");
    c->fuse_apply = fused != 0;
    c->fuse_wide = fused == 2;
    c->split_store = split_store != 0;
    return SDM_OK;
}

int sdm_debug_gradient_table(sdm_ctx* c, int level, float* g, int* bin)
{
    if (!c || level < 0 || level >= (int)c->levels.size() || !g || !bin) return fail(SDM_ERR_INVALID, "bad arguments");
    HIP_TRY(hipSetDevice(c->device));
    const size_t n = 511 * 511;
    ScopedBuf<float> d_g; ScopedBuf<int> d_b;
    int rc;
    if ((rc = d_g.ensure(n)) || (rc = d_b.ensure(n))) return rc;
    sdm_launch_gradient_table(c->levels[level], d_g.p, d_b.p, c->stream);
    HIP_TRY(hipGetLastError());
    HIP_TRY(hipMemcpyAsync(g, d_g.p, n * sizeof(float), hipMemcpyDeviceToHost, c->stream));
    HIP_TRY(hipMemcpyAsync(bin, d_b.p, n * sizeof(int), hipMemcpyDeviceToHost, c->stream));
    HIP_TRY(hipStreamSynchronize(c->stream));
    d_g.release(); d_b.release();
    return SDM_OK;
}

int sdm_debug_set_option(sdm_ctx* c, const char* name, int value)
{
    if (!c || !name) return fail(SDM_ERR_INVALID, "bad arguments");
    const std::string n(name);
    if (n == "hog_no_pack") c->packing = value == 0;
    else if (n == "hog_two_load") c->hog_two_load = value != 0;
    else if (n == "hog_split_store") c->split_store = value != 0;
    else if (n == "detect_unfused") c->fuse_apply = value == 0;
    else if (n == "detect_fuse_wide") c->env_fuse_wide = value != 0;
    else if (n == "apply_f32") c->env_apply_f32 = value != 0;
    else if (n == "gram_f32") c->env_gram_f32 = value != 0;
// ... 38 lines not shown
```

superviseddescent_amd/csrc/sdm_capi_detect.hip:

```cpp
#include "sdm_capi_internal.h"

namespace sdm_capi {

void fill_row_tab(HogLevelDev& lv)
{
    for (int d = 0; d < 64 && d < lv.S; ++d) {
        const float hx = (float)((d + 0.5) / (double)lv.cell - 0.5);
        int b = (int)hx;
        if (!(hx >= 0.0f || (float)b == hx)) b -= 1;
        const float w2 = hx - (float)b, w1 = (float)(1.0 - w2);
        const float wlo = b >= 0 ? w1 : 0.0f, whi = b + 1 <= lv.C - 1 ? w2 : 0.0f;
        lv.row_tab[d][0] = (b & 1) ? whi : wlo;
        lv.row_tab[d][1] = (b & 1) ? wlo : whi;
        memcpy(&lv.row_tab[d][2], &b, sizeof(int));
        lv.row_tab[d][3] = w2;
    }
}



void drain_timing(sdm_ctx* c)
{
    for (auto& p : c->pending) {
        hipError_t e = hipEventSynchronize(p.b); (void)e;
        float ms = 0.f;
        if (hipEventElapsedTime(&ms, p.a, p.b) == hipSuccess) { c->t_ms[p.slot] += ms; c->t_n[p.slot] += 1; }
        if (!p.a_shared) c->pool.push_back(p.a);
        c->pool.push_back(p.b);
    }
    c->pending.clear();
    c->ev_fresh = false;
}

int check_status(sdm_ctx* c)
{
    int st = 0;
    HIP_TRY(hipMemcpyAsync(&st, c->status.p, sizeof(int), hipMemcpyDeviceToHost, c->stream));
    HIP_TRY(hipStreamSynchronize(c->stream));
    if (st) {
        HIP_TRY(hipMemsetAsync(c->status.p, 0, sizeof(int), c->stream));
        if (st & SDM_DEV_ERR_EMPTY_PATCH)
            return fail(SDM_ERR_EMPTY_PATCH, "patch_width_half <= 0 for at least one sample (inter-eye distance too small)");
        if (st & 2) return fail(SDM_ERR_NOT_SPD, "regularised Gram matrix is not positive definite; increase lambda");
        if (st & 4) return fail(SDM_ERR_HIP, "back substitution: a tile row waited for its predecessor beyond the spin limit");
        if (st & 8) return fail(SDM_ERR_NOT_SPD, "Cholesky update: a factor entry exceeds the square root of the largest diagonal entry (matrix not positive definite?)");
    }
    return SDM_OK;
}


ImageSetDev image_set(const sdm_ctx* c)
{
    ImageSetDev s;
    s.base = c->img_base; s.offset = c->img_off.p; s.w = c->img_w.p; s.h = c->img_h.p;
    s.stride = c->img_stride.p; s.n_images = c->n_images;
    return s;
}

int ensure_sample_buffers(sdm_ctx* c, int N)
{
    int rc;
    const size_t nx = (size_t)N * c->M;
    if ((rc = c->x[0].ensure(nx))) return rc;
    if ((rc = c->x[1].ensure(nx))) return rc;
    const size_t nf = (size_t)N * (size_t)c->ldf;
    if (nf > c->feat.cap) {
        if ((rc = c->feat.ensure(nf, true, c->stream))) return rc;
        c->feat_level = -1; c->feat_wide_F = 0; c->feat_wide_N = 0;
    }
    if ((rc = c->patch_idx.ensure((size_t)N * (1 + 2 * c->L)))) return rc;
    return SDM_OK;
}

int check_sample_index(const sdm_ctx* c)
{
    if (c->idx_identity && c->N > c->n_images)
        return fail(SDM_ERR_INVALID, "more samples than images and no sample->image index set");
    if (!c->idx_identity && c->N > c->n_idx)
        return fail(SDM_ERR_INVALID, "sample->image index is shorter than the sample count");
    if (!c->idx_identity && c->max_idx >= c->n_images)
        return fail(SDM_ERR_INVALID, "sample->image index refers to an image beyond the current image set");
    return SDM_OK;
}

bool packed_ok(const sdm_ctx* c, int level)
{
    return c->fast_kernel[level] && !c->narrow_images && c->packing && c->hog_mode == SDM_HOG_COLUMNS &&
           c->fast_bins[level] == 2 && c->plans[level].ok;
}
bool split_ok(const sdm_ctx* c, int level) { return packed_ok(c, level) && sdm_desc_supported(c->levels[level]); }

int hog_checks(sdm_ctx* c, int level)
{
    if (!c->img_base) return fail(SDM_ERR_INVALID, "no images set");
    if (c->N <= 0) return fail(SDM_ERR_INVALID, "no samples set (sdm_set_x)");
    if (c->levels[level].fixed_h == 0 && (c->eyes.nre <= 0 || c->eyes.nle <= 0))
        return fail(SDM_ERR_INVALID, "HOG features need eye landmark indices (IED-adaptive patch size)");
    return check_sample_index(c);
}

static HogPlanDev cells_plan(const sdm_ctx* c, int level)
{
    HogPlanDev pd = c->plans[level].dev;
    pd.two_load = c->hog_two_load ? 1 : 0;
    return pd;
}

int launch_cells(sdm_ctx* c, int level)
{
    int rc = c->cells.ensure(sdm_cells_floats(c->levels[level], c->N, c->L));
    if (rc) return rc;
    sdm_launch_hog_cells(image_set(c), c->idx_identity ? nullptr : c->img_idx.p, c->x[c->cur].p, c->N, c->L, c->eyes,
                         c->levels[level], cells_plan(c, level), c->cells.p, c->patch_idx.p, c->status.p, c->stream);
    return SDM_OK;
}

int do_hog(sdm_ctx* c, int level)
{
    { const int rci = hog_checks(c, level); if (rci) return rci; }
    if (c->feat_wide_F > level_F(c, level)) {
        const size_t rows = (size_t)(c->feat_wide_N > c->N ? c->feat_wide_N : c->N);
        HIP_TRY(hipMemsetAsync(c->feat.p, 0, rows * c->ldf * sizeof(float), c->stream));
        c->feat_wide_F = 0; c->feat_wide_N = 0;
        c->ev_fresh = false;
    }
    {
        Timer t(c, SDM_T_HOG);
        if (c->split_store && split_ok(c, level)) {
            const int rcc = launch_cells(c, level);
            if (rcc) return rcc;
            sdm_launch_desc_store(c->levels[level], c->cells.p, c->plans[level].cut.p, c->N, c->L, c->feat.p, c->ldf, c->stream);
        } else if (packed_ok(c, level))
            sdm_launch_hog_packed(image_set(c), c->idx_identity ? nullptr : c->img_idx.p, c->x[c->cur].p, c->N, c->L,
                                  c->eyes, c->levels[level], c->plans[level].dev, c->feat.p, c->ldf, c->patch_idx.p,
                                  c->status.p, c->stream);
        else if (c->fast_kernel[level] && !c->narrow_images)
            sdm_launch_hog_fast(image_set(c), c->idx_identity ? nullptr : c->img_idx.p, c->x[c->cur].p, c->N, c->L,
                                c->eyes, c->levels[level], c->feat.p, c->ldf, c->patch_idx.p, c->status.p,
                                c->hog_mode , c->fast_bins[level], c->stream);
        else
            sdm_launch_hog(image_set(c), c->idx_identity ? nullptr : c->img_idx.p, c->x[c->cur].p, c->N, c->L,
                           c->eyes, c->levels[level], c->feat.p, c->ldf, c->patch_idx.p, c->status.p, c->stream);
    }
    if (c->tmpl_N > 0) {
        if (c->tmpl_N != c->N || c->tmpl_F != level_F(c, level))
            return fail(SDM_ERR_INVALID, "templates do not match the sample count / feature dimension of this level");
        sdm_launch_subtract_templates(c->feat.p, c->ldf, c->tmpl.p, c->N, c->tmpl_F, c->stream);
        c->ev_fresh = false;
    }
    HIP_TRY(hipGetLastError());
    c->feat_level = level;
    if (level_F(c, level) > c->feat_wide_F) c->feat_wide_F = level_F(c, level);
    if (c->N > c->feat_wide_N) c->feat_wide_N = c->N;
    c->feat_bounded = c->tmpl_N == 0;
    c->have_patch_idx = true;
    return SDM_OK;
}

int build_apply_planes(sdm_ctx* c, int level)
{
    int rc;
    if ((rc = c->Rp[level].ensure(sdm_apply_planes_bytes(c->ldf, c->M))) || (rc = c->Rmax.ensure(c->levels.size() * (size_t)Mp_of(c->M)))) return rc;
    sdm_launch_apply_planes(c->Rt[level].p, c->ldf, c->M, c->Rp[level].p, c->Rmax.p + (size_t)level * Mp_of(c->M), c->stream);
    if (c->plans[level].ok && sdm_desc_supported(c->levels[level])) {
        if ((rc = c->Rd[level].ensure(sdm_desc_planes_bytes(c->levels[level], c->L, c->M)))) return rc;
        sdm_launch_desc_planes(c->levels[level], c->Rt[level].p, c->ldf, c->L, c->M, c->Rmax.p + (size_t)level * Mp_of(c->M),
                               c->Rd[level].p, c->stream);
    }
    HIP_TRY(hipGetLastError());
    return SDM_OK;
}

int do_apply(sdm_ctx* c, int level)
{
    if (c->feat_level != level) return fail(SDM_ERR_INVALID, "sdm_apply: features of this level not extracted");
    if (!c->have_R[level]) return fail(SDM_ERR_INVALID, "sdm_apply: no regressor set for this level");
    const int F = level_F(c, level);
    const int splits = sdm_apply_splits(c->N, F, c->M);
    int rc = c->partial.ensure((size_t)splits * c->N * Mp_of(c->M));
    if (rc) return rc;
    {
        Timer t(c, SDM_T_APPLY);
        sdm_launch_apply(c->feat.p, c->ldf, c->N, F, c->Rt[level].p, c->ldf, c->M, c->x[c->cur].p,
                         c->x[c->cur ^ 1].p, c->L, c->eyes, c->partial.p, splits, c->stream,
                         (c->feat_bounded && !c->env_apply_f32) ? c->Rp[level].p : nullptr,
                         (c->feat_bounded && !c->env_apply_f32 && c->Rp[level].p) ? c->Rmax.p + (size_t)level * Mp_of(c->M) : nullptr);
    }
    HIP_TRY(hipGetLastError());
    c->cur ^= 1;
    return SDM_OK;
}

bool fused_ok(const sdm_ctx* c, int level)
{
    return c->fuse_apply && (Mp_of(c->M) <= 64 || c->env_fuse_wide || c->fuse_wide) && split_ok(c, level) && c->have_R[level] && c->Rd[level].p &&
           c->Rp[level].p && c->tmpl_N == 0;
}
int detect_level_fused(sdm_ctx* c, int l)
{
    { const int rci = hog_checks(c, l); if (rci) return rci; }
    const int Mp = Mp_of(c->M);
    int rc;
    size_t cells_max = 0;
    for (size_t q = 0; q < c->levels.size(); ++q) { const size_t n = sdm_cells_floats(c->levels[q], c->N, c->L); if (n > cells_max) cells_max = n; }
    if ((rc = c->cells.ensure(cells_max)) || (rc = c->partial.ensure((size_t)c->L * c->N * Mp))) return rc;
    const HogLevelDev& lv = c->levels[l];
    {
        Timer t(c, SDM_T_HOG);
        sdm_launch_hog_cells(image_set(c), c->idx_identity ? nullptr : c->img_idx.p, c->x[c->cur].p, c->N, c->L, c->eyes, lv,
                             cells_plan(c, l), c->cells.p, c->patch_idx.p, c->status.p, c->stream);
    }
    {
        Timer t(c, SDM_T_APPLY);
        sdm_launch_desc_apply(lv, c->cells.p, c->plans[l].cut.p, c->N, c->L, c->M, c->Rd[l].p, c->Rmax.p + (size_t)l * Mp,
                              c->Rt[l].p, c->ldf, c->partial.p, c->stream);
        sdm_launch_apply_reduce(c->partial.p, c->L, c->N, c->M, c->x[c->cur].p, c->x[c->cur ^ 1].p, c->L, c->eyes, c->stream);
    }
    HIP_TRY(hipGetLastError());
    c->cur ^= 1;
    c->feat_level = -1;
    c->have_patch_idx = true;
    return SDM_OK;
}

int detect_level(sdm_ctx* c, int l)
{
    if (fused_ok(c, l)) return detect_level_fused(c, l);
    int rc = do_hog(c, l);
    if (!rc) rc = do_apply(c, l);
    return rc;
}

}

extern "C" {

int sdm_hog_features(sdm_ctx* c, int level, float* feat_host)
{
    if (!c || level < 0 || level >= (int)c->levels.size()) return fail(SDM_ERR_INVALID, "bad level");
    HIP_TRY(hipSetDevice(c->device));
    int rc = do_hog(c, level);
    if (rc) return rc;
    if (feat_host) {
        const int F = level_F(c, level);
        HIP_TRY(hipMemcpy2DAsync(feat_host, (size_t)F * sizeof(float), c->feat.p, (size_t)c->ldf * sizeof(float),
                                 (size_t)F * sizeof(float), c->N, hipMemcpyDeviceToHost, c->stream));
        HIP_TRY(hipStreamSynchronize(c->stream));
        return check_status(c);
    }
    return SDM_OK;
}

int sdm_get_patch_indices(sdm_ctx* c, int* idx)
{
    if (!c || !idx || c->N <= 0 || !c->have_patch_idx) return fail(SDM_ERR_INVALID, "no HOG call to report");
    HIP_TRY(hipMemcpyAsync(idx, c->patch_idx.p, (size_t)c->N * (1 + 2 * c->L) * sizeof(int), hipMemcpyDeviceToHost, c->stream));
    HIP_TRY(hipStreamSynchronize(c->stream));
    return SDM_OK;
}

int sdm_set_regressor(sdm_ctx* c, int level, const float* R)
{
    if (!c || !R || level < 0 || level >= (int)c->levels.size()) return fail(SDM_ERR_INVALID, "bad regressor");
    HIP_TRY(hipSetDevice(c->device));
    const int F = level_F(c, level), M = c->M, Mp = Mp_of(M);
    int rc = c->Rt[level].ensure((size_t)Mp * c->ldf);
    if (rc) return rc;
    std::vector<float> t((size_t)Mp * c->ldf, 0.0f);
    for (int k = 0; k < F; ++k)
        for (int j = 0; j < M; ++j) t[(size_t)j * c->ldf + k] = R[(size_t)k * M + j];
    HIP_TRY(hipMemcpyAsync(c->Rt[level].p, t.data(), t.size() * sizeof(float), hipMemcpyHostToDevice, c->stream));
    if ((rc = build_apply_planes(c, level))) return rc;
    HIP_TRY(hipStreamSynchronize(c->stream));
    c->have_R[level] = true;
    return SDM_OK;
}

int sdm_get_regressor(sdm_ctx* c, int level, float* R)
{
    if (!c || !R || level < 0 || level >= (int)c->levels.size() || !c->have_R[level]) return fail(SDM_ERR_INVALID, "no regressor");
    const int F = level_F(c, level), M = c->M, Mp = Mp_of(M);
    std::vector<float> t((size_t)Mp * c->ldf);
    HIP_TRY(hipMemcpyAsync(t.data(), c->Rt[level].p, t.size() * sizeof(float), hipMemcpyDeviceToHost, c->stream));
    HIP_TRY(hipStreamSynchronize(c->stream));
    for (int k = 0; k < F; ++k)
        for (int j = 0; j < M; ++j) R[(size_t)k * M + j] = t[(size_t)j * c->ldf + k];
    return SDM_OK;
}

int sdm_apply(sdm_ctx* c, int level)
{
    if (!c || level < 0 || level >= (int)c->levels.size()) return fail(SDM_ERR_INVALID, "bad level");
    HIP_TRY(hipSetDevice(c->device));
    return do_apply(c, level);
}

int sdm_detect_batch(sdm_ctx* c, float* x_host)
{
    if (!c) return fail(SDM_ERR_INVALID, "null context");
    HIP_TRY(hipSetDevice(c->device));
    c->chain_timers = true; c->ev_fresh = false;
    int rc = SDM_OK;
    for (int l = 0; l < (int)c->levels.size() && !rc; ++l) rc = detect_level(c, l);
    c->chain_timers = false; c->ev_fresh = false;
    if (rc) return rc;
    if (x_host) return sdm_get_x(c, x_host);
    return SDM_OK;
}

int sdm_detect_level(sdm_ctx* c, int level)
{
    if (!c || level < 0 || level >= (int)c->levels.size()) return fail(SDM_ERR_INVALID, "bad level");
    HIP_TRY(hipSetDevice(c->device));
    return detect_level(c, level);
}


}
```

superviseddescent_amd/csrc/sdm_capi_internal.h:

```cpp
#pragma once
#include "../../include/sdm.h"
#include "sdm_kernels.h"

#include <dlfcn.h>
#include <math.h>
#include <stdio.h>
#include <stdlib.h>
#include <string.h>
#include <string>
#include <vector>

namespace sdm_capi {


inline std::string& err_string() { static thread_local std::string e; return e; }

inline int fail(int code, const std::string& msg)
{
    err_string() = msg;
    return code;
}

#define HIP_TRY(expr)                                                                          \
    do {                                                                                       \
// ... 38 lines not shown


}
using namespace sdm_capi;

struct sdm_ctx {
    int device = 0;
    hipStream_t stream = nullptr;
    bool own_stream = false;
    SolveAux solve_aux = {nullptr, nullptr, nullptr, nullptr, nullptr, nullptr, 0, 0, 0, 0};
    DevBuf<unsigned char> upd_planes;
    DevBuf<unsigned> upd_maxdiag;

    int L = 0, M = 0;
    EyeIdxDev eyes{};
    std::vector<HogLevelDev> levels;
    std::vector<sdm_hog_param> params;
    std::vector<int> fast_kernel;
    std::vector<int> fast_bins;
    struct Plan { bool ok = false; HogPlanDev dev{}; DevBuf<unsigned> lane_tab; DevBuf<float> wb; DevBuf<unsigned short> wb16; DevBuf<int> pass_info; DevBuf<int> cut; DevBuf<int> taps; };
    std::vector<Plan> plans;
    DevBuf<float> cells;
    int solver_kind = SDM_SOLVER_CHOLESKY;
    int last_rank = -1, last_rank_full = 0;
    DevBuf<float> qr_work;
    bool split_store = false;
    bool fuse_apply = true;
    bool fuse_wide = false;
    bool hog_two_load = false;
    bool packing = true;
    bool env_fuse_wide = false;
    bool env_apply_f32 = false;
    bool env_gram_f32 = false;
    bool env_gram_bf16 = false;
    int env_shard_emulate = 0;
    int hog_mode = SDM_HOG_COLUMNS;
    int Fmax = 0;
    long long ldf = 0;
    int rhs_tiles = 1;

    DevBuf<uint8_t> img_owned;
    const uint8_t* img_base = nullptr;
    DevBuf<long long> img_off;
    DevBuf<int> img_w, img_h, img_stride;
    int n_images = 0;
    bool narrow_images = false;
    DevBuf<int> img_idx;
    bool idx_identity = true;
    int n_idx = 0, max_idx = -1;

    int N = 0;
    DevBuf<float> x[2];
    int cur = 0;
    DevBuf<float> xstar;
    DevBuf<float> tmpl;
    int tmpl_F = 0, tmpl_N = 0;
    bool have_targets = false;
    DevBuf<float> feat;
    int feat_level = -1;
    int feat_wide_F = 0, feat_wide_N = 0;
    bool feat_bounded = false;
    DevBuf<int> patch_idx;
    bool have_patch_idx = false;
    DevBuf<int> status;
    DevBuf<float> partial;

    std::vector<DevBuf<float>> Rt;
    std::vector<DevBuf<unsigned char>> Rp;
    std::vector<DevBuf<unsigned char>> Rd;
    DevBuf<unsigned> Rmax;
    std::vector<bool> have_R;

    DevBuf<float> G;
    DevBuf<float> gpack;
    int g_ncols = 0;
    int g_fp = 0;
    int g_level = -1;
    DevBuf<double> fro;
    DevBuf<float> Rsol;
    DevBuf<float> winv;
    DevBuf<int> gram_flag;
    static const int XBLOCKS_MAX = 8;
    hipEvent_t gram_ev[XBLOCKS_MAX] = {}; hipEvent_t gram_xdone = nullptr;
    int gram_blocks = 0;
    int gram_block_c[XBLOCKS_MAX + 1] = {};
    int env_xblocks = -1;
    int gram_fallbacks = 0;
    int update_range_fallbacks = 0;
    int gram_f32_fallbacks = 0;
    DevBuf<unsigned char> gram_planes;
    DevBuf<float> lambda_dev;

    sdm_allreduce_fn allreduce = nullptr;
    void* allreduce_user = nullptr;
    int world_size = 1;
    void* rccl_comm = nullptr;
    int (*rccl_allreduce)(const void*, void*, size_t, int, int, void*, hipStream_t) = nullptr;
    int shard_rank = 0, shard_world = 0;
    sdm_bcast_fn shard_bcast = nullptr;
    sdm_allgather_fn shard_allgather = nullptr;
    void* shard_user = nullptr;
    void* shard_comm = nullptr;
    int (*rccl_bcast)(const void*, void*, size_t, int, int, void*, hipStream_t) = nullptr;
    int (*rccl_allgather)(const void*, void*, size_t, int, void*, hipStream_t) = nullptr;
    DevBuf<float> shard_stage;
    sdm_reduce_scatter_fn reduce_scatter = nullptr;
// ... 57 lines not shown
        DevBuf<unsigned> Rmax;
        DevBuf<float> x;
        DevBuf<double> score;
        DevBuf<unsigned> arrived;
        int K = 0, level = -1;
        unsigned ok = 0;
        void release() { snap.release(); Rt.release(); Rp.release(); Rmax.release(); x.release(); score.release(); arrived.release(); K = 0; level = -1; ok = 0; }
    } sweep;
    std::vector<int> img_w_host, img_h_host, img_idx_host;

    bool timing = false;
    float t_ms[SDM_T_COUNT] = {0};
    int t_n[SDM_T_COUNT] = {0};
    struct Pending { int slot; hipEvent_t a, b; bool a_shared; };
    hipEvent_t last_stop = nullptr;
    bool ev_fresh = false, chain_timers = false;
    std::vector<Pending> pending;
    std::vector<hipEvent_t> pool;
};

namespace sdm_capi {

inline int Mp_of(int M) { return round_up(M, 16); }
inline int level_F(const sdm_ctx* c, int level) { return c->L * c->levels[level].P + (c->levels[level].fixed_h > 0 ? 0 : 1); }

struct Timer {
    sdm_ctx* c; int slot; hipEvent_t a = nullptr, b = nullptr; bool a_shared = false;
    Timer(sdm_ctx* ctx, int s) : c(ctx), slot(s)
    {
        if (!c->timing) return;
        if (c->chain_timers && c->ev_fresh) { a = c->last_stop; a_shared = true; }
        else { a = take(); hipError_t e = hipEventRecord(a, c->stream); (void)e; }
        b = take();
    }
    hipEvent_t take()
    {
        if (!c->pool.empty()) { hipEvent_t ev = c->pool.back(); c->pool.pop_back(); return ev; }
        hipEvent_t ev; hipError_t e = hipEventCreate(&ev); (void)e; return ev;
    }
    ~Timer()
    {
        if (!c->timing) return;
        hipError_t e = hipEventRecord(b, c->stream); (void)e;
        c->pending.push_back({slot, a, b, a_shared});
        c->last_stop = b; c->ev_fresh = true;
    }
};

void fill_row_tab(HogLevelDev& lv);
void drain_timing(sdm_ctx* c);
int check_status(sdm_ctx* c);
ImageSetDev image_set(const sdm_ctx* c);
int ensure_sample_buffers(sdm_ctx* c, int N);
int check_sample_index(const sdm_ctx* c);
bool packed_ok(const sdm_ctx* c, int level);
bool split_ok(const sdm_ctx* c, int level);
int hog_checks(sdm_ctx* c, int level);
int launch_cells(sdm_ctx* c, int level);
int do_hog(sdm_ctx* c, int level);
int build_apply_planes(sdm_ctx* c, int level);
int do_apply(sdm_ctx* c, int level);
bool fused_ok(const sdm_ctx* c, int level);
int detect_level_fused(sdm_ctx* c, int l);
int detect_level(sdm_ctx* c, int l);
int solve_update_scratch(sdm_ctx* c, int ncols);
int gram_rhs_rows(sdm_ctx* c, int level, int rows);
int qr_solve(sdm_ctx* c, float* G, int ncols, int F, int Fp, int Mp, float* R_out);
int shard_bcast_thunk(void* self, float* buf, size_t count, int root, hipStream_t stream);
int shard_allgather_thunk(void* self, const float* send, float* recv, size_t count, hipStream_t stream);

}
```

superviseddescent_amd/csrc/sdm_capi_pose.hip:

```cpp
#include "sdm_capi_internal.h"

#include <cmath>

namespace {

int pose_ready(sdm_ctx* c)
{
    if (!c) return fail(SDM_ERR_INVALID, "null context");
    if (c->pose.cam.K <= 0) return fail(SDM_ERR_INVALID, "pose model not set (sdm_pose_set_model)");
    HIP_TRY(hipSetDevice(c->device));
    return SDM_OK;
}

int pose_F(const sdm_ctx* c) { return 2 * c->pose.cam.K; }

int pose_set_x_common(sdm_ctx* c, const float* x, int N, hipMemcpyKind kind)
{
    int rc = pose_ready(c);
    if (rc) return rc;
    if (!x || N < 1) return fail(SDM_ERR_INVALID, "bad pose parameters (N x 6, N >= 1)");
    if ((rc = c->pose.x.ensure((size_t)N * 6))) return rc;
    if (N != c->pose.N) c->pose.have_targets = false;
    c->pose.N = N;
    HIP_TRY(hipMemcpyAsync(c->pose.x.p, x, (size_t)N * 6 * sizeof(float), kind, c->stream));
// ... 29 lines not shown
    const float radians = (fovy / 2.0f) * (float)3.14159265358979323846 / 180.0f;
    const float cotan = std::cos(radians) / std::sin(radians);
    const float aspect = width / height;
    PoseCamDev cam{};
    const float P[16] = {cotan / aspect, 0.f, 0.f, 0.f, 0.f, cotan, 0.f, 0.f, 0.f, 0.f, -(near_ + far_) / (far_ - near_),
                         (-2.0f * near_ * far_) / (far_ - near_), 0.f, 0.f, -1.0f, 0.f};
    memcpy(cam.P, P, sizeof(P));
    cam.f = focal; cam.W = width; cam.H = height; cam.K = K;
    p.cam = cam;
    HIP_TRY(hipMemcpyAsync(p.pts.p, points, (size_t)K * 3 * sizeof(float), hipMemcpyHostToDevice, c->stream));
    HIP_TRY(hipStreamSynchronize(c->stream));
    return SDM_OK;
}

int sdm_pose_set_x(sdm_ctx* c, const float* x_host, int n_samples) { return pose_set_x_common(c, x_host, n_samples, hipMemcpyHostToDevice); }
int sdm_pose_set_x_device(sdm_ctx* c, const float* x_dev, int n_samples) { return pose_set_x_common(c, x_dev, n_samples, hipMemcpyDeviceToDevice); }

int sdm_pose_get_x(sdm_ctx* c, float* x_host)
{
    int rc = pose_ready(c);
    if (rc) return rc;
    if (!x_host || c->pose.N < 1) return fail(SDM_ERR_INVALID, "pose parameters not set");
    HIP_TRY(hipMemcpyAsync(x_host, c->pose.x.p, (size_t)c->pose.N * 6 * sizeof(float), hipMemcpyDeviceToHost, c->stream));
    HIP_TRY(hipStreamSynchronize(c->stream));
    return SDM_OK;
}

int sdm_pose_set_templates(sdm_ctx* c, const float* templates, int n_samples, int feature_dim)
{
    int rc = pose_ready(c);
    if (rc) return rc;
    if (!templates || n_samples < 1 || feature_dim != pose_F(c)) return fail(SDM_ERR_INVALID, "pose templates must be N x 2K");
    if ((rc = c->pose.tmpl.ensure((size_t)n_samples * feature_dim))) return rc;
    HIP_TRY(hipMemcpyAsync(c->pose.tmpl.p, templates, (size_t)n_samples * feature_dim * sizeof(float), hipMemcpyHostToDevice, c->stream));
    HIP_TRY(hipStreamSynchronize(c->stream));
    c->pose.tmpl_N = n_samples;
    return SDM_OK;
}

int sdm_pose_templates_from_landmarks(sdm_ctx* c, const int* landmark_index, int K, float focal)
{
    int rc = pose_ready(c);
    if (rc) return rc;
    if (!landmark_index || K != c->pose.cam.K) return fail(SDM_ERR_INVALID, "the landmark index map must name one landmark per model point");
    if (!(focal > 0.f)) return fail(SDM_ERR_INVALID, "focal length must be positive");
    if (c->L <= 0 || c->N < 1) return fail(SDM_ERR_INVALID, "no landmark rows (set the geometry and x, or run a detect batch)");
    if (c->n_images < 1) return fail(SDM_ERR_INVALID, "no images: the gather normalises by each row's image centre");
    if ((rc = check_sample_index(c))) return rc;
    for (int k = 0; k < K; ++k)
        if (landmark_index[k] < 0 || landmark_index[k] >= c->L) return fail(SDM_ERR_INVALID, "landmark index out of range");
    sdm_ctx::Pose& p = c->pose;
    if ((rc = p.lm.ensure((size_t)K)) || (rc = p.tmpl.ensure((size_t)c->N * 2 * K))) return rc;
    HIP_TRY(hipMemcpyAsync(p.lm.p, landmark_index, (size_t)K * sizeof(int), hipMemcpyHostToDevice, c->stream));
    sdm_launch_pose_gather(c->x[c->cur].p, c->L, c->N, p.lm.p, K, c->idx_identity ? nullptr : c->img_idx.p, c->img_w.p, c->img_h.p, focal,
                           p.tmpl.p, c->stream);
    HIP_TRY(hipGetLastError());
    HIP_TRY(hipStreamSynchronize(c->stream));
    p.tmpl_N = c->N;
    return SDM_OK;
}

int sdm_pose_set_targets(sdm_ctx* c, const float* xstar_host, int n_samples)
{
    int rc = pose_ready(c);
    if (rc) return rc;
    if (!xstar_host || n_samples != c->pose.N) return fail(SDM_ERR_INVALID, "pose targets must be N x 6 for the current rows");
    if ((rc = c->pose.xstar.ensure((size_t)n_samples * 6))) return rc;
    HIP_TRY(hipMemcpyAsync(c->pose.xstar.p, xstar_host, (size_t)n_samples * 6 * sizeof(float), hipMemcpyHostToDevice, c->stream));
    HIP_TRY(hipStreamSynchronize(c->stream));
    c->pose.have_targets = true;
    return SDM_OK;
}

int sdm_pose_features(sdm_ctx* c, int level, float* out_host)
{
    int rc = pose_ready(c);
    if (rc) return rc;
    sdm_ctx::Pose& p = c->pose;
    if (level < 0 || level >= SDM_POSE_MAX_LEVELS || !out_host || p.N < 1) return fail(SDM_ERR_INVALID, "bad pose feature request");
    const int F = pose_F(c);
    if ((rc = p.Ab.ensure((size_t)p.N * F))) return rc;
    sdm_launch_pose_project(p.x.p, nullptr, p.tmpl_N == p.N ? p.tmpl.p : nullptr, p.pts.p, p.cam, p.N, p.Ab.p, F, c->stream);
    HIP_TRY(hipGetLastError());
    HIP_TRY(hipMemcpyAsync(out_host, p.Ab.p, (size_t)p.N * F * sizeof(float), hipMemcpyDeviceToHost, c->stream));
    HIP_TRY(hipStreamSynchronize(c->stream));
    return SDM_OK;
}

int sdm_pose_set_regressor(sdm_ctx* c, int level, const float* R_host)
{
    int rc = pose_ready(c);
    if (rc) return rc;
    if (level < 0 || level >= SDM_POSE_MAX_LEVELS || !R_host) return fail(SDM_ERR_INVALID, "pose level out of range (0..15)");
    const size_t n = (size_t)pose_F(c) * 6;
    HIP_TRY(hipMemcpyAsync(c->pose.R.p + (size_t)level * n, R_host, n * sizeof(float), hipMemcpyHostToDevice, c->stream));
    HIP_TRY(hipStreamSynchronize(c->stream));
    c->pose.have_R |= 1u << level;
    return SDM_OK;
}

int sdm_pose_get_regressor(sdm_ctx* c, int level, float* R_host)
{
    int rc = pose_ready(c);
    if (rc) return rc;
    if (level < 0 || level >= SDM_POSE_MAX_LEVELS || !R_host || !(c->pose.have_R >> level & 1u))
        return fail(SDM_ERR_INVALID, "pose level has no regressor");
// ... 43 lines not shown
```

superviseddescent_amd/csrc/sdm_capi_sweep.hip:

```cpp
#include "sdm_capi_internal.h"

#include <limits>

namespace {

bool collectives_installed(const sdm_ctx* c)
{
    return c->allreduce || c->rccl_comm || c->reduce_scatter || c->rccl_reduce_scatter || c->shard_bcast || c->shard_allgather || c->shard_comm;
}

}

extern "C" {

int sdm_train_level_sweep(sdm_ctx* c, int level, int reg_type, const float* reg_params, int K, int regularise_last_row,
                          long long n_train_global, int n_fit_rows, double* holdout_err, double* fit_err, float* lambdas,
                          int* status, int* best)
{
    if (!c || level < 0 || level >= (int)c->levels.size()) return fail(SDM_ERR_INVALID, "bad level");
    if (!reg_params || !holdout_err || !lambdas || !status || !best) return fail(SDM_ERR_INVALID, "sdm_train_level_sweep: null argument");
    if (K < 1 || K > 32) return fail(SDM_ERR_INVALID, "sdm_train_level_sweep: 1 ... 32 candidates");
    if (reg_type != SDM_REG_MANUAL && reg_type != SDM_REG_MATRIX_NORM) return fail(SDM_ERR_INVALID, "bad regulariser type");
    if (n_fit_rows < 1 || n_fit_rows >= c->N) return fail(SDM_ERR_INVALID, "sdm_train_level_sweep: 1 <= n_fit_rows < sample count required (the rows behind the fit rows are held out)");
    if (collectives_installed(c))
        return fail(SDM_ERR_INVALID, "sdm_train_level_sweep: a collective is installed on this handle; the sweep runs on one rank (the held-out sums are not reduced)");
    if (!c->have_targets) return fail(SDM_ERR_INVALID, "sdm_train_level_sweep: no targets set");
    if (c->eyes.nre <= 0 || c->eyes.nle <= 0) return fail(SDM_ERR_INVALID, "sdm_train_level_sweep: no eye landmarks (the score is normalised by the inter-eye distance)");
    HIP_TRY(hipSetDevice(c->device));
    int rc;
    if ((rc = sdm_hog_features(c, level, nullptr))) return rc;
    if ((rc = gram_rhs_rows(c, level, n_fit_rows))) return rc;
    const int F = level_F(c, level), M = c->M, Mp = Mp_of(M), N = c->N;
    const int Fp = round_up(F, 128), ncols = c->g_ncols;
    sdm_ctx::Sweep& sw = c->sweep;
    sw.K = 0; sw.level = -1; sw.ok = 0;
    c->g_level = -1;
    const size_t rt_floats = (size_t)Mp * c->ldf, rp_bytes = sdm_apply_planes_bytes(c->ldf, M);
    const int splits = sdm_apply_splits(N, F, M);
    if ((rc = sw.snap.ensure(sdm_packed_tiles_count(F, c->rhs_tiles))) || (rc = sw.Rt.ensure((size_t)K * rt_floats)) ||
        (rc = sw.Rp.ensure((size_t)K * rp_bytes)) || (rc = sw.Rmax.ensure((size_t)K * Mp)) || (rc = sw.x.ensure((size_t)N * M)) ||
        (rc = sw.score.ensure((size_t)2 * 32 + 2 * SDM_SWEEP_SCORE_PARTS)) || (rc = sw.arrived.ensure(2)) ||
        (rc = c->partial.ensure((size_t)splits * N * Mp)) ||
        (rc = c->fro.ensure((size_t)F + 1)) || (rc = c->Rsol.ensure((size_t)Fp * Mp)) ||
        (rc = c->winv.ensure((size_t)Fp * 128 + sdm_backsolve_flag_floats(Fp))))
        return rc;
    {
        Timer t(c, SDM_T_GRAM);
        sdm_launch_sweep_snapshot(c->G.p, ncols, F, c->rhs_tiles, sw.snap.p, c->stream);
        if (reg_type == SDM_REG_MATRIX_NORM) sdm_launch_fro2_upper(c->G.p, ncols, F, c->fro.p, c->stream);
    }
    HIP_TRY(hipGetLastError());
    const int n_reg = (int)(n_train_global > 0 ? n_train_global : n_fit_rows);
    const bool planes = c->feat_bounded && !c->env_apply_f32;
    double* score_part = sw.score.p + 2 * 32;
    for (int k = 0; k < K; ++k) {
        float* Rt_k = sw.Rt.p + (size_t)k * rt_floats;
        unsigned char* Rp_k = sw.Rp.p + (size_t)k * rp_bytes;
        unsigned* Rmax_k = sw.Rmax.p + (size_t)k * Mp;
        {
            Timer t(c, SDM_T_REG);
            if (k > 0) sdm_launch_sweep_restore(c->G.p, ncols, F, c->rhs_tiles, sw.snap.p, c->stream);
            sdm_launch_add_diag(c->G.p, ncols, F, c->fro.p + F, reg_type, reg_params[k], n_reg, regularise_last_row, c->lambda_dev.p, c->stream);
        }
        {
            Timer t(c, SDM_T_FACTOR);
            if (c->solver_kind == SDM_SOLVER_COLPIV_QR) {
                if ((rc = qr_solve(c, c->G.p, ncols, F, Fp, Mp, c->Rsol.p))) return rc;
            } else {
                if ((rc = solve_update_scratch(c, ncols))) return rc;
                (void)sdm_launch_cholesky_solve(c->G.p, ncols, F, Fp, Mp, c->Rsol.p, Mp, c->winv.p, c->status.p, c->stream, &c->solve_aux, nullptr);
            }
        }
        HIP_TRY(hipGetLastError());
        sdm_launch_pack_regressor(c->Rsol.p, F, M, Mp, Rt_k, c->ldf, nullptr, c->stream);
        sdm_launch_apply_planes(Rt_k, c->ldf, M, Rp_k, Rmax_k, c->stream);
        {
            Timer t(c, SDM_T_APPLY);
            sdm_launch_apply(c->feat.p, c->ldf, N, F, Rt_k, c->ldf, M, c->x[c->cur].p, sw.x.p, c->L, c->eyes, c->partial.p, splits, c->stream,
                             planes ? Rp_k : nullptr, planes ? Rmax_k : nullptr);
            sdm_launch_sweep_score(sw.x.p, c->xstar.p, N, n_fit_rows, c->L, c->eyes, score_part, sw.arrived.p, sw.score.p + 2 * k, c->stream);
        }
        HIP_TRY(hipGetLastError());
        HIP_TRY(hipMemcpyAsync(lambdas + k, c->lambda_dev.p, sizeof(float), hipMemcpyDeviceToHost, c->stream));
        status[k] = check_status(c);
        if (status[k] != SDM_OK && status[k] != SDM_ERR_NOT_SPD) return status[k];
        if (status[k] == SDM_OK) sw.ok |= 1u << k;
    }
    double means[2 * 32];
    HIP_TRY(hipMemcpyAsync(means, sw.score.p, (size_t)2 * K * sizeof(double), hipMemcpyDeviceToHost, c->stream));
    HIP_TRY(hipStreamSynchronize(c->stream));
    sw.K = K; sw.level = level;
    int win = -1;
    for (int k = 0; k < K; ++k) {
        const bool ok = status[k] == SDM_OK;
        holdout_err[k] = ok ? means[2 * k] : std::numeric_limits<double>::infinity();
        if (fit_err) fit_err[k] = ok ? means[2 * k + 1] : std::numeric_limits<double>::infinity();
        if (ok && (win < 0 || holdout_err[k] < holdout_err[win])) win = k;
    }
    *best = win;
    if (win < 0) return fail(SDM_ERR_NOT_SPD, "sdm_train_level_sweep: no candidate gave a positive definite system; increase the regulariser");
    if ((rc = c->Rt[level].ensure(rt_floats))) return rc;
    HIP_TRY(hipMemcpyAsync(c->Rt[level].p, sw.Rt.p + (size_t)win * rt_floats, rt_floats * sizeof(float), hipMemcpyDeviceToDevice, c->stream));
    if ((rc = build_apply_planes(c, level))) return rc;
    c->have_R[level] = true;
    return sdm_apply(c, level);
}

int sdm_sweep_get_regressor(sdm_ctx* c, int k, float* R)
{
    if (!c || !R) return fail(SDM_ERR_INVALID, "sdm_sweep_get_regressor: null argument");
    const sdm_ctx::Sweep& sw = c->sweep;
    if (sw.K <= 0 || sw.level < 0 || sw.level >= (int)c->levels.size()) return fail(SDM_ERR_INVALID, "sdm_sweep_get_regressor: no sweep has run on this handle");
    if (k < 0 || k >= sw.K) return fail(SDM_ERR_INVALID, "sdm_sweep_get_regressor: no such candidate");
    if (!(sw.ok >> k & 1u)) return fail(SDM_ERR_NOT_SPD, "sdm_sweep_get_regressor: this candidate's system was not positive definite");
    HIP_TRY(hipSetDevice(c->device));
    const int F = level_F(c, sw.level), M = c->M, Mp = Mp_of(M);
    std::vector<float> t((size_t)Mp * c->ldf);
    HIP_TRY(hipMemcpyAsync(t.data(), sw.Rt.p + (size_t)k * t.size(), t.size() * sizeof(float), hipMemcpyDeviceToHost, c->stream));
    HIP_TRY(hipStreamSynchronize(c->stream));
    for (int i = 0; i < F; ++i)
        for (int j = 0; j < M; ++j) R[(size_t)i * M + j] = t[(size_t)j * c->ldf + i];
    return SDM_OK;
}

}
```

superviseddescent_amd/csrc/sdm_capi_track.hip:

```cpp
#include "sdm_capi_internal.h"

#include <algorithm>
#include <cmath>

namespace {

int track_ready(sdm_ctx* c)
{
    if (!c) return fail(SDM_ERR_INVALID, "null context");
    if (c->track.S < 1) return fail(SDM_ERR_INVALID, "tracker not configured (sdm_track_configure)");
    if (c->L != c->track.L) return fail(SDM_ERR_INVALID, "the geometry's landmark count changed since sdm_track_configure");
    return SDM_OK;
}

int check_ids(sdm_ctx* c, const int* ids, int n)
{
    sdm_ctx::Track& t = c->track;
    if (!ids || n < 1) return fail(SDM_ERR_INVALID, "no stream ids (n >= 1)");
    if (++t.stamp == 0) { std::fill(t.seen.begin(), t.seen.end(), 0u); t.stamp = 1; }
    for (int i = 0; i < n; ++i) {
        if (ids[i] < 0 || ids[i] >= t.S) return fail(SDM_ERR_INVALID, "stream id " + std::to_string(ids[i]) + " out of range");
        if (t.seen[ids[i]] == t.stamp) return fail(SDM_ERR_INVALID, "stream id " + std::to_string(ids[i]) + " named twice in one call");
        t.seen[ids[i]] = t.stamp;
    }
// ... 55 lines not shown
    if (rc) return rc;
    if ((rc = check_ids(c, ids, n))) return rc;
    if (!boxes) return fail(SDM_ERR_INVALID, "no face boxes");
    for (int i = 0; i < n; ++i)
        if (boxes[4 * i + 2] <= 0 || boxes[4 * i + 3] <= 0) return fail(SDM_ERR_INVALID, "a face box needs width and height > 0");
    sdm_ctx::Track& t = c->track;
    HIP_TRY(hipSetDevice(c->device));
    if ((rc = ensure_pinned(t, (size_t)5 * n)) || (rc = t.ids.ensure((size_t)5 * n))) return rc;
    memcpy(t.pin, ids, (size_t)n * sizeof(int));
    memcpy(t.pin + n, boxes, (size_t)4 * n * sizeof(int));
    HIP_TRY(hipMemcpyAsync(t.ids.p, t.pin, (size_t)5 * n * sizeof(int), hipMemcpyHostToDevice, c->stream));
    sdm_launch_track_start(t.ids.p, t.ids.p + n, n, t.box.p, t.status.p, c->stream);
    HIP_TRY(hipGetLastError());
    HIP_TRY(hipStreamSynchronize(c->stream));
    for (int i = 0; i < n; ++i) t.host_status[ids[i]] = SDM_TRACK_STARTED;
    return SDM_OK;
}

int sdm_track_stop(sdm_ctx* c, const int* ids, int n)
{
    int rc = track_ready(c);
    if (rc) return rc;
    if ((rc = check_ids(c, ids, n))) return rc;
    for (int i = 0; i < n; ++i) c->track.host_status[ids[i]] = SDM_TRACK_FREE;
    return SDM_OK;
}

int sdm_track_step(sdm_ctx* c, const int* ids, int n, float* landmarks_host, int* lost_host)
{
    int rc = track_ready(c);
    if (rc) return rc;
    sdm_ctx::Track& t = c->track;
    if (c->levels.empty()) return fail(SDM_ERR_INVALID, "geometry not set");
    for (size_t l = 0; l < c->levels.size(); ++l)
        if (!c->have_R[l]) return fail(SDM_ERR_INVALID, "no regressor set for level " + std::to_string(l));
    if ((rc = check_ids(c, ids, n))) return rc;
    for (int i = 0; i < n; ++i) {
        const int st = t.host_status[ids[i]];
        if (st == SDM_TRACK_FREE) return fail(SDM_ERR_INVALID, "stream " + std::to_string(ids[i]) + " is not started");
        if (st == SDM_TRACK_LOST) return fail(SDM_ERR_INVALID, "stream " + std::to_string(ids[i]) + " is lost: start it again from a face box");
    }
    if (c->tmpl_N > 0) return fail(SDM_ERR_INVALID, "templates are set: the tracker runs the cascade without (sdm_set_templates(NULL))");
    if (!c->img_base || c->n_images < 1) return fail(SDM_ERR_INVALID, "no images set");
    if (c->idx_identity && n > c->n_images) return fail(SDM_ERR_INVALID, "more rows than images and no sample->image index set");
    if (!c->idx_identity && n > c->n_idx) return fail(SDM_ERR_INVALID, "sample->image index is shorter than the step's rows");
    if (!c->idx_identity && c->max_idx >= c->n_images)
        return fail(SDM_ERR_INVALID, "sample->image index refers to an image beyond the current image set");
    HIP_TRY(hipSetDevice(c->device));
    const int M = c->M;
    if ((rc = ensure_sample_buffers(c, n)) || (rc = t.init.ensure((size_t)n * M)) || (rc = t.ids.ensure((size_t)n)) ||
        (rc = t.masks.ensure((size_t)n + 1)) || (rc = ensure_pinned(t, (size_t)2 * n + 1)))
        return rc;
    if (n != c->N) { c->have_targets = false; c->feat_level = -1; c->have_patch_idx = false; }
    c->N = n; c->cur = 0;
    memcpy(t.pin, ids, (size_t)n * sizeof(int));
    HIP_TRY(hipMemcpyAsync(t.ids.p, t.pin, (size_t)n * sizeof(int), hipMemcpyHostToDevice, c->stream));
    sdm_launch_track_gather(t.ids.p, n, c->L, t.mode, t.status.p, t.box.p, t.x.p, t.mean.p, t.mean_bounds, c->x[0].p, t.init.p, c->stream);
    HIP_TRY(hipGetLastError());
    c->chain_timers = true; c->ev_fresh = false;
    for (int l = 0; l < (int)c->levels.size() && !rc; ++l) rc = detect_level(c, l);
    c->chain_timers = false; c->ev_fresh = false;
    if (rc) return rc;
    sdm_launch_track_commit(t.ids.p, n, c->L, c->x[c->cur].p, t.init.p, c->idx_identity ? nullptr : c->img_idx.p, c->img_w.p, c->img_h.p,
                            c->eyes, t.min_size, t.max_scale, t.x.p, t.status.p, t.masks.p, c->status.p, c->stream);
    HIP_TRY(hipGetLastError());
    int* masks = t.pin + n;
    HIP_TRY(hipMemcpyAsync(masks, t.masks.p, ((size_t)n + 1) * sizeof(int), hipMemcpyDeviceToHost, c->stream));
    if (landmarks_host)
        HIP_TRY(hipMemcpyAsync(landmarks_host, c->x[c->cur].p, (size_t)n * M * sizeof(float), hipMemcpyDeviceToHost, c->stream));
    HIP_TRY(hipStreamSynchronize(c->stream));
    for (int i = 0; i < n; ++i) t.host_status[ids[i]] = masks[i] ? SDM_TRACK_LOST : SDM_TRACK_TRACKED;
    if (lost_host) memcpy(lost_host, masks, (size_t)n * sizeof(int));
    const int st = masks[n];
    if (st) {
        HIP_TRY(hipMemsetAsync(c->status.p, 0, sizeof(int), c->stream));
        if (st & SDM_DEV_ERR_EMPTY_PATCH)
            return fail(SDM_ERR_EMPTY_PATCH, "patch_width_half <= 0 for at least one row (inter-eye distance too small)");
        return fail(SDM_ERR_HIP, "a kernel reported status " + std::to_string(st));
    }
    return SDM_OK;
}

int sdm_track_get(sdm_ctx* c, const int* ids, int n, float* landmarks_host, int* status_host)
{
    int rc = track_ready(c);
    if (rc) return rc;
    if ((rc = check_ids(c, ids, n))) return rc;
    sdm_ctx::Track& t = c->track;
    if (landmarks_host) {
        HIP_TRY(hipSetDevice(c->device));
        if ((rc = t.init.ensure((size_t)n * c->M)) || (rc = t.ids.ensure((size_t)n)) || (rc = ensure_pinned(t, (size_t)n))) return rc;
        memcpy(t.pin, ids, (size_t)n * sizeof(int));
        HIP_TRY(hipMemcpyAsync(t.ids.p, t.pin, (size_t)n * sizeof(int), hipMemcpyHostToDevice, c->stream));
        sdm_launch_track_gather(t.ids.p, n, c->L, SDM_TRACK_INIT_PREVIOUS, t.status.p, t.box.p, t.x.p, t.mean.p, t.mean_bounds, t.init.p,
                                nullptr, c->stream);
        HIP_TRY(hipGetLastError());
        HIP_TRY(hipMemcpyAsync(landmarks_host, t.init.p, (size_t)n * c->M * sizeof(float), hipMemcpyDeviceToHost, c->stream));
        HIP_TRY(hipStreamSynchronize(c->stream));
    }
    if (status_host)
        for (int i = 0; i < n; ++i) status_host[i] = t.host_status[ids[i]];
    return SDM_OK;
}

}
```

superviseddescent_amd/csrc/sdm_capi_train.hip:

```cpp
#include "sdm_capi_internal.h"

namespace sdm_capi {

int solve_update_scratch(sdm_ctx* c, int ncols)
{
    int rc;
    if ((rc = c->upd_planes.ensure(sdm_update_f16_plane_bytes(512, ncols))) || (rc = c->upd_maxdiag.ensure(4))) return rc;
    c->solve_aux.upd_planes = c->upd_planes.p;
    c->solve_aux.upd_maxdiag = c->upd_maxdiag.p;
    c->solve_aux.range_fallbacks = &c->update_range_fallbacks;
    return SDM_OK;
}

int gram_rhs_rows(sdm_ctx* c, int level, int rows)
{
    const int F = level_F(c, level);
    const int Fp = round_up(F, 128), ncols = Fp + 128 * c->rhs_tiles;
    int rc = c->G.ensure((size_t)ncols * ncols);
    if (rc) return rc;
    c->g_scattered = false;
    c->gram_blocks = 0;
    Timer t(c, SDM_T_GRAM);
    HIP_TRY(hipMemset2DAsync(c->feat.p + Fp, (size_t)c->ldf * sizeof(float), 0, 128 * c->rhs_tiles * sizeof(float), c->N, c->stream));
    sdm_launch_targets(c->x[c->cur].p, c->xstar.p, c->N, c->L, c->eyes, c->feat.p, c->ldf, Fp, c->stream);
    const bool gram_f32 = c->env_gram_f32, gram_bf16 = c->env_gram_bf16;
    int form = gram_f32 ? 0 : (gram_bf16 ? 3 : 2);
    if (form && c->gram_planes.ensure(sdm_gram_bf16x3_plane_bytes(rows, ncols, form))) { (void)hipGetLastError(); form = 0; c->gram_f32_fallbacks += 1; }
    if (form == 3) sdm_launch_gram_bf16x3(c->feat.p, c->ldf, rows, ncols, c->gram_planes.p, c->G.p, ncols, c->stream);
    else if (form == 2) {
        if ((rc = c->gram_flag.ensure(1))) return rc;
        HIP_TRY(hipMemsetAsync(c->gram_flag.p, 0, sizeof(int), c->stream));
        const int Ttot = ncols / 128, Wx = c->shard_world;
        const bool will_scatter = Wx >= 2 && (c->shard_comm || c->shard_bcast) && Wx == c->world_size &&
                                  (c->reduce_scatter || (c->rccl_reduce_scatter && c->rccl_comm)) && c->solver_kind == SDM_SOLVER_CHOLESKY;
        int nb = 1;
        if (will_scatter) nb = c->env_xblocks > 0 ? c->env_xblocks : (c->env_xblocks < 0 && Ttot >= 128 ? 4 : 1);
        const int ncolw = will_scatter ? (Ttot + Wx - 1) / Wx : 0;
        if (nb > sdm_ctx::XBLOCKS_MAX) nb = sdm_ctx::XBLOCKS_MAX;
        if (nb > ncolw) nb = ncolw > 0 ? ncolw : 1;
        if (nb > 1) {
            sdm_launch_gram_f16_split(c->feat.p, c->ldf, rows, ncols, c->gram_planes.p, c->stream, c->gram_flag.p);
            int over = 0;
            HIP_TRY(hipMemcpyAsync(&over, c->gram_flag.p, sizeof(int), hipMemcpyDeviceToHost, c->stream));
            HIP_TRY(hipStreamSynchronize(c->stream));
            if (!over) {
                c->gram_block_c[0] = 0;
                for (int b = 1; b < nb; ++b) {
                    int cb = (int)(ncolw * sqrt((double)b / nb) + 0.5);
                    if (cb <= c->gram_block_c[b - 1]) cb = c->gram_block_c[b - 1] + 1;
                    c->gram_block_c[b] = cb < ncolw ? cb : ncolw;
                }
                c->gram_block_c[nb] = ncolw;
                int off = 0;
                for (int b = 0; b < nb; ++b) {
                    const int j_lo = c->gram_block_c[b] * Wx, j_hi = b + 1 < nb ? c->gram_block_c[b + 1] * Wx : Ttot;
                    off += sdm_launch_gram_f16_product(c->gram_planes.p, rows, ncols, c->G.p, ncols, j_lo, j_hi < Ttot ? j_hi : Ttot, off, c->stream);
                    HIP_TRY(hipEventRecord(c->gram_ev[b], c->stream));
                }
                HIP_TRY(hipGetLastError());
                c->gram_blocks = nb;
                c->g_ncols = ncols; c->g_fp = Fp; c->g_level = level;
                return SDM_OK;
            }
            c->gram_fallbacks += 1;
            if (c->gram_planes.ensure(sdm_gram_bf16x3_plane_bytes(rows, ncols, 3))) { (void)hipGetLastError(); form = 0; c->gram_f32_fallbacks += 1; }
            else sdm_launch_gram_bf16x3(c->feat.p, c->ldf, rows, ncols, c->gram_planes.p, c->G.p, ncols, c->stream);
            if (form == 0) sdm_launch_syrk_tn(c->feat.p, c->ldf, rows, ncols, c->G.p, ncols, 1.0f, 0, 0, c->stream);
            HIP_TRY(hipGetLastError());
            c->g_ncols = ncols; c->g_fp = Fp; c->g_level = level;
            return SDM_OK;
        }
        sdm_launch_gram_bf16x3(c->feat.p, c->ldf, rows, ncols, c->gram_planes.p, c->G.p, ncols, c->stream, c->gram_flag.p);
        int over = 0;
        HIP_TRY(hipMemcpyAsync(&over, c->gram_flag.p, sizeof(int), hipMemcpyDeviceToHost, c->stream));
        HIP_TRY(hipStreamSynchronize(c->stream));
// ... 201 lines not shown
```

superviseddescent_amd/csrc/sdm_hog_device.h:

```cpp
#pragma once
#include "sdm_kernels.h"

#pragma clang fp contract(off)

namespace {

typedef float f32x2 __attribute__((ext_vector_type(2)));
typedef float f32x4 __attribute__((ext_vector_type(4)));

__device__ inline double ied_of(const float* __restrict__ xr, int L, const EyeIdxDev& e)
{
    float rx = 0.0f, ry = 0.0f, lx = 0.0f, ly = 0.0f;
    for (int i = 0; i < e.nre; ++i) { rx += xr[e.re[i]]; ry += xr[e.re[i] + L]; }
    if (e.inv_nre != 0.0f) { rx *= e.inv_nre; ry *= e.inv_nre; } else { rx /= (float)e.nre; ry /= (float)e.nre; }
    for (int i = 0; i < e.nle; ++i) { lx += xr[e.le[i]]; ly += xr[e.le[i] + L]; }
    if (e.inv_nle != 0.0f) { lx *= e.inv_nle; ly *= e.inv_nle; } else { lx /= (float)e.nle; ly /= (float)e.nle; }
    float dxf = rx - lx, dyf = ry - ly;
    double dx = dxf, dy = dyf;
    return sqrt(dx * dx + dy * dy);
}

__device__ inline int sat_short_f(float v)
{
    int i = __float2int_rn(v);
    return i > 32767 ? 32767 : (i < -32768 ? -32768 : i);
}

__device__ inline int vl_floor(float x)
{
    int xi = (int)x;
    if (x >= 0 || (float)xi == x) return xi;
    return xi - 1;
}

__device__ inline float from_left(float v)
{
    return __builtin_bit_cast(float, __builtin_amdgcn_update_dpp(0, __builtin_bit_cast(int, v), 0x138, 0xf, 0xf, true));
}
__device__ inline float from_right(float v)
{
    return __builtin_bit_cast(float, __builtin_amdgcn_update_dpp(0, __builtin_bit_cast(int, v), 0x130, 0xf, 0xf, true));
}

__device__ inline float sqrt_int_exact(float x)
{
    const float r = __builtin_amdgcn_sqrtf(x);
    const float rm = __builtin_bit_cast(float, __builtin_bit_cast(int, r) - 1);
    const float rp = __builtin_bit_cast(float, __builtin_bit_cast(int, r) + 1);
    const float em = __builtin_fmaf(-rm, r, x);
    const float ep = __builtin_fmaf(-rp, r, x);
    float y = (em <= 0.0f) ? rm : r;
    y = (ep > 0.0f) ? rp : y;
    return y;
}

__device__ inline float sqrt_int_up(float x)
{
    const float r = __builtin_amdgcn_sqrtf(x);
    const float rp = __builtin_bit_cast(float, __builtin_bit_cast(int, r) + 1);
    const float ep = __builtin_fmaf(-rp, r, x);
    return (ep > 0.0f) ? rp : r;
}

__device__ inline void bin_reference(float gx, float gy, float g, const HogLevelDev& lv, int& bin)
{
    float nx = g > 0.0f ? gx / g : 0.0f;
    float ny = g > 0.0f ? gy / g : 0.0f;
    float best = 0.0f;
    bin = -1;
    for (int k = 0; k < lv.O; ++k) {
        float s = nx * lv.ox[k] + ny * lv.oy[k];
        int b = k;
// ... 102 lines not shown
```

superviseddescent_amd/csrc/sdm_hog_packed.hip:

```cpp
#include "sdm_kernels.h"
#include "sdm_hog_device.h"
#include <type_traits>

#pragma clang fp contract(off)

#define HP_WAVES 4
#define HP_ST 66
#define HP_MINW 6
#define HP_MINW_CELLS 6
__host__ __device__ constexpr bool hp_row_carry(int cell) { return cell == 10 || cell == 8 || cell == 6; }

namespace {

typedef int i32x4 __attribute__((ext_vector_type(4)));
typedef int i32x2 __attribute__((ext_vector_type(2)));

__device__ inline unsigned mul_hi_u24_vv(unsigned a, unsigned b)
{
    unsigned r;
    asm("v_mul_hi_u32_u24 %0, %1, %2" : "=v"(r) : "v"(a), "v"(b));
    return r;
}

#define HP_ROWS_BYTES(O) ((size_t)2 * (O) * HP_ST * 8)
// ... 39 lines not shown
        const int byb = t / CB, bxb = t - byb * CB;
        const int xa = bxb - 1 > 0 ? bxb - 1 : 0, xb = bxb < C - 1 ? bxb : C - 1;
        const int ya = byb - 1 > 0 ? byb - 1 : 0, yb = byb < C - 1 ? byb : C - 1;
        const FT na = nrm[xa + ya * C], nb = nrm[xb + ya * C];
        const FT nc = nrm[xa + yb * C], nd = nrm[xb + yb * C];
        fac[t] = ft_rsqrt(na + nb + nc + nd + (FT)1e-4);
    }
    wave_sync();
#define CL02(v) ft_min02(v)
    for (int t = lane; t < O * CC; t += 64) {
        const int k = t / CC, c = t - k * CC;
        const int y = c / C, x = c - y * C, ct = x * C + y;
        const FT ha = hist[c + k * CC], hb = hist[c + (k + O) * CC];
        const FT f1 = fac[x + y * CB], f2 = fac[x + 1 + y * CB];
        const FT f3 = fac[x + (y + 1) * CB], f4 = fac[x + 1 + (y + 1) * CB];
        FT ha1 = f1 * ha, ha2 = f2 * ha, ha3 = f3 * ha, ha4 = f4 * ha;
        FT hb1 = f1 * hb, hb2 = f2 * hb, hb3 = f3 * hb, hb4 = f4 * hb;
        FT hc1 = ha1 + hb1, hc2 = ha2 + hb2, hc3 = ha3 + hb3, hc4 = ha4 + hb4;
        ha1 = CL02(ha1); ha2 = CL02(ha2); ha3 = CL02(ha3); ha4 = CL02(ha4);
        hb1 = CL02(hb1); hb2 = CL02(hb2); hb3 = CL02(hb3); hb4 = CL02(hb4);
        hc1 = CL02(hc1); hc2 = CL02(hc2); hc3 = CL02(hc3); hc4 = CL02(hc4);
        if (lv.variant == 1) {
            out_desc[ct + k * CC] = (float)((FT)0.5 * (ha1 + ha2 + ha3 + ha4));
            out_desc[ct + (k + O) * CC] = (float)((FT)0.5 * (hb1 + hb2 + hb3 + hb4));
            out_desc[ct + (k + 2 * O) * CC] = (float)((FT)0.5 * (hc1 + hc2 + hc3 + hc4));
            hcc[t] = hc1; hcc[O * CC + t] = hc2; hcc[2 * O * CC + t] = hc3; hcc[3 * O * CC + t] = hc4;
        } else {
            out_desc[ct + k * CC] = (float)hc1;
            out_desc[ct + (k + O) * CC] = (float)hc2;
            out_desc[ct + (k + 2 * O) * CC] = (float)hc3;
            out_desc[ct + (k + 3 * O) * CC] = (float)hc4;
        }
    }
    if (lv.variant == 1) {
        const float tex = 1.0f / sqrtf(18.0f);
        wave_sync();
        for (int t = lane; t < 4 * CC; t += 64) {
            const int j = t / CC, c = t - j * CC;
            const int y = c / C, x = c - y * C, ct = x * C + y;
            FT acc = 0;
#pragma unroll
            for (int k = 0; k < O; ++k) acc += hcc[(j * O + k) * CC + c];
            out_desc[ct + (3 * O + j) * CC] = (float)(tex * acc);
        }
    }
#undef CL02
    wave_sync();
}

template <int TO, int TC, int CELL, bool RAW, bool CELLS = false>
__global__ void __launch_bounds__(HP_WAVES * 64, CELLS ? HP_MINW_CELLS : HP_MINW)
hog_packed_kernel(ImageSetDev imgs, const int* __restrict__ img_idx, const float* __restrict__ x, int N, int L,
                  EyeIdxDev eyes, HogLevelDev lv, HogPlanDev plan, float* __restrict__ feat, long long ldf,
                  int* __restrict__ idx_out, int* __restrict__ status)
{
    extern __shared__ __attribute__((aligned(16))) unsigned char smem[];
    constexpr int O = TO, C = TC, CC = C * C;
    constexpr int ST = HP_ST;
    static_assert(2 * TO <= 32 && SDM_PLAN_MAX_SEG * TC <= 16, "16 x 16 matrix-core tiles: 2O bin rows in one or two tiles, 3 patches x C cell columns");
    constexpr int MT = (2 * TO + 15) / 16;
    const int lane = threadIdx.x & 63;
    const int wave = uni(threadIdx.x >> 6);
    const unsigned nb = gridDim.x, bid = blockIdx.x;
    const unsigned q8 = nb / 8, r8 = nb % 8, xcd = bid % 8;
    const unsigned blk = (xcd < r8 ? xcd * (q8 + 1) : r8 * (q8 + 1) + (xcd - r8) * q8) + bid / 8;
    constexpr bool SPLIT = CELLS;
    const int gpf = SPLIT ? plan.n_main * plan.P + plan.Pt : plan.n_main + (plan.Gt > 0 ? 1 : 0);
    const long long wid = (long long)blk * HP_WAVES + wave;
    if (wid >= (long long)N * gpf) return;
    const int s = (int)(wid / gpf), u = (int)(wid - (long long)s * gpf);
    const int g = SPLIT ? (u < plan.n_main * plan.P ? u / plan.P : plan.n_main) : u;
    const bool main_group = g < plan.n_main;
    const int lm0 = main_group ? g * plan.G : plan.n_main * plan.G;
    const int t_first = SPLIT ? u - g * plan.P : 0;
    const int npass = SPLIT ? t_first + 1 : (main_group ? plan.P : plan.Pt);
    const int pass0 = main_group ? 0 : plan.P;
    constexpr int SC = TC * CELL;
    const int S = CELL > 0 ? SC : lv.S;

    const int nslots = CELLS ? 0 : plan.hist_slots;
    constexpr bool SPEC = CELL > 0;
    constexpr bool ROTB = RAW && TO == 4;
    unsigned char* lds = smem + (size_t)wave * packed_lds_bytes(C, O, S, nslots, SPEC);
    float* colrows = (float*)lds;
    i32x4* rowtab = (i32x4*)(lds + al16(HP_ROWS_BYTES(O)));
    float* hist = (float*)(lds + al16(HP_ROWS_BYTES(O)) + packed_rowtab_bytes(S, SPEC));
    f32x2* wstab = (f32x2*)(smem + (size_t)HP_WAVES * packed_lds_bytes(C, O, S, nslots, SPEC));
    constexpr int HSTR = (2 * O * CC * 4 + 15) / 16 * 4;
    unsigned char* scratch = lds;
    auto hist_slot = [&](int patch_slot) { return nslots == 2 ? (patch_slot & 1) : patch_slot % 3; };

    const int im = uni(img_idx ? img_idx[s] : s);
    const float* xr = x + (long long)s * 2 * L;
    float* out_row = feat + (long long)s * ldf;
    int* idx_row = idx_out ? idx_out + (long long)s * (1 + 2 * L) : nullptr;

    const int h = lv.fixed_h > 0 ? lv.fixed_h : uni((int)round((double)lv.rel * ied_of(xr, L, eyes) / 2));
    const bool empty = h <= 0;
    if (empty && lane == 0) atomicOr(status, SDM_DEV_ERR_EMPTY_PATCH);
    const int sw = empty ? 1 : 2 * h;
    const bool area2 = (sw == 2 * S);
    const uint8_t* img = imgs.base + imgs.offset[im];
    const int iw = imgs.w[im], ih = imgs.h[im], istride = imgs.stride[im];
    const __amdgpu_buffer_rsrc_t img_rsrc = __builtin_amdgcn_make_buffer_rsrc((void*)img, 0, ih * istride, 0x00020000);

    int tab_s, tab_w;
    constexpr bool CARRY = CELLS && RAW && CELL > 0 && hp_row_carry(CELL);
    int carry_mask = 0;
    bool carry = false;
    i32x4 row_ent;
    if (CELLS && plan.taps && h < SDM_SCALE_TAB) {
        const i32x4* e = (const i32x4*)(plan.taps + ((size_t)(h > 0 ? h : 0) * 64 + lane) * 8);
        const i32x4 e0 = e[0], e1 = e[1];
        tab_s = e0.x; tab_w = e0.y;
        row_ent = (i32x4){e0.z * istride, e0.w * istride, e1.x, e1.y};
        if (CARRY) { carry_mask = e1.z; carry = uni(e1.w) != 0 && !plan.two_load; }
    } else {
        const double scale = resize_scale(lv, h, sw);
        const ResizeTaps tp = resize_taps(lane < S ? lane : S - 1, scale, sw, area2);
        tab_s = tp.s0;
        tab_w = (tp.c0 & 0xffff) | (tp.c1 << 16);
        row_ent = (i32x4){tp.sy0 * istride, tp.sy1 * istride, tp.b0 << 12, tp.b1 << 12};
    }

    {
        const f32x4 z4 = {0.0f, 0.0f, 0.0f, 0.0f};
        for (int i = lane; i < (int)(al16(HP_ROWS_BYTES(O)) / 16); i += 64) ((f32x4*)lds)[i] = z4;
    }
    wave_sync();
    if (SPEC) {
        if (lane < S) {
            const int eo = lane >= 2 ? lane - 2 : lane + S - 2;
            if (CARRY && carry) { ((int*)&rowtab[eo])[0] = row_ent.y; ((int*)&rowtab[lane])[1] = carry_mask; }
            else *(i32x2*)&rowtab[eo] = (i32x2){row_ent.x, row_ent.y};
            *((i32x2*)&rowtab[lane] + 1) = (i32x2){row_ent.z, row_ent.w};
        }
    } else if (lane < S + 2) rowtab[lane] = row_ent;
    constexpr bool F16F = TO == 4 && CELL > 0;
    static_assert(!F16F || CELL * 361 * 8 < 65504, "float16 folds: a band slot's column sum (<= cell x 255 sqrt 2) x 8 must stay a float16 number");
    if (SPEC && lane < S) wstab[lane] = (f32x2){lv.row_tab[lane][0], lv.row_tab[lane][1]} * (F16F ? 8.0f : 1.0f);
    if (!SPEC && S + 2 > 64 && lane < S + 2 - 64) {
        i32x4 last;
#pragma unroll
        for (int k = 0; k < 4; ++k) last[k] = __builtin_amdgcn_readlane(row_ent[k], 63);
        rowtab[64 + lane] = last;
    }
    wave_sync();

    unsigned spread_sel = HF_SPREAD_SEL;
    asm volatile("" : "+v"(spread_sel));
    const int li = lane & 15, lq = lane >> 4;

    for (int t = t_first; t < npass; ++t) {
        const int pt = pass0 + t;
        const unsigned desc = plan.lane_tab[pt * 64 + lane];
        const int slot = (int)(desc & 0xffu), col = (int)((desc >> 8) & 0xffu);
// ... 270 lines not shown
#pragma unroll
                for (int yrow = 2; yrow < SC; ++yrow) row_step(yrow & 1, yrow, true, one_load);
            } else two_load_rows();
        } else two_load_rows();
        *pend_p = __builtin_elementwise_fma(pend_v, (f32x2){pend_g, pend_g}, *pend_p);
        if (CELLS && TO == 4 && prev_by >= 0 && prev_by + 1 <= C - 1) fold_band(prev_by, true);
        else {
            if (prev_by >= 0) fold_band(prev_by);
            if (prev_by + 1 <= C - 1) fold_band(prev_by + 1);
        }
        wave_sync();

        const int dfirst = done & 0xff, dcount = (done >> 8) & 0xff;
        for (int j = 0; j < dcount; ++j) {
            const int ps = dfirst + j, lmp = lm0 + ps;
            if (!CELLS) {
                float* hp = hist + hist_slot(ps) * HSTR;
                hog_finish_direct<TO, TC>(hp, scratch, out_row + (long long)lmp * lv.P, lv, lane);
                for (int i = lane; i < (int)(packed_scratch_bytes(C, O) / 16); i += 64) ((f32x4*)scratch)[i] = (f32x4){0.0f, 0.0f, 0.0f, 0.0f};
            }
            if (idx_row && lane == 0) {
                if (lmp == 0) idx_row[0] = h;
                idx_row[1 + lmp] = __float2int_rn(xr[lmp]);
                idx_row[1 + L + lmp] = __float2int_rn(xr[lmp + L]);
            }
            if (!CELLS && lmp == L - 1 && lv.fixed_h == 0 && lane == 0) out_row[(long long)L * lv.P] = 1.0f;
            if (!CELLS) wave_sync();
        }
    }
}

__global__ void taps_table_kernel(HogLevelDev lv, int* __restrict__ table)
{
    const int h = blockIdx.x, d = threadIdx.x;
    const int S = lv.S;
    const bool empty = h <= 0;
    const int sw = empty ? 1 : 2 * h;
    const bool area2 = (sw == 2 * S);
    const double scale = resize_scale(lv, h, sw);
    const ResizeTaps tp = resize_taps(d < S ? d : S - 1, scale, sw, area2);
    i32x4* e = (i32x4*)(table + ((size_t)h * 64 + d) * 8);
    e[0] = (i32x4){tp.s0, (tp.c0 & 0xffff) | (tp.c1 << 16), tp.sy0, tp.sy1};
    const int p0 = __shfl_up(tp.sy0, 1), p1 = __shfl_up(tp.sy1, 1);
    const bool held = d == 0 || d >= S || tp.sy0 == p0 || tp.sy0 == p1;
    const bool eligible = !empty && !area2 && __ballot(!held) == 0;
    e[1] = (i32x4){tp.b0 << 12, tp.b1 << 12, (d >= 1 && tp.sy0 == p1) ? -1 : 0, eligible ? 1 : 0};
}

}

template <bool CELLS>
static void launch_hog_packed(const ImageSetDev& imgs, const int* img_idx, const float* x, int N, int L,
                              const EyeIdxDev& eyes, const HogLevelDev& lv, const HogPlanDev& plan, float* feat, long long ldf,
                              int* idx_out, int* status, hipStream_t stream)
{
    const int gpf = CELLS ? plan.n_main * plan.P + plan.Pt : plan.n_main + (plan.Gt > 0 ? 1 : 0);
    const long long total = (long long)N * gpf;
    if (total <= 0) return;
    const unsigned grid = (unsigned)((total + HP_WAVES - 1) / HP_WAVES);
#define HP_LAUNCH_O(TO, CELL, RAW)                                                                                              \
    hipLaunchKernelGGL((hog_packed_kernel<TO, 5, CELL, RAW, CELLS>), dim3(grid), dim3(HP_WAVES * 64),                              \
                       packed_wg_lds_bytes(5, TO, lv.S, CELLS ? 0 : plan.hist_slots, CELL > 0), stream, imgs, img_idx, x, N, L,  \
                       eyes, lv, plan, feat, ldf, idx_out, status)
#define HP_LAUNCH(CELL, RAW) HP_LAUNCH_O(4, CELL, RAW)
    if (lv.O == 9) {
        static unsigned long long attr9 = 0;
        if (sdm_first_use_on_device(attr9)) {
            SDM_SET_ATTR((const void*)hog_packed_kernel<9, 5, 0, true, CELLS>, hipFuncAttributeMaxDynamicSharedMemorySize, 160 * 1024);
            SDM_SET_ATTR((const void*)hog_packed_kernel<9, 5, 0, false, CELLS>, hipFuncAttributeMaxDynamicSharedMemorySize, 160 * 1024);
        }
        if (plan.raw_sqrt) HP_LAUNCH_O(9, 0, true); else HP_LAUNCH_O(9, 0, false);
        return;
    }
    if (!plan.raw_sqrt) { HP_LAUNCH(0, false); return; }
    switch (lv.cell) {
    case 11: HP_LAUNCH(11, true); break;
    case 10: HP_LAUNCH(10, true); break;
    case 8: HP_LAUNCH(8, true); break;
    case 6: HP_LAUNCH(6, true); break;
    default: HP_LAUNCH(0, true); break;
    }
#undef HP_LAUNCH
#undef HP_LAUNCH_O
}

void sdm_launch_hog_packed(const ImageSetDev& imgs, const int* img_idx, const float* x, int N, int L,
                           const EyeIdxDev& eyes, const HogLevelDev& lv, const HogPlanDev& plan, float* feat, long long ldf,
                           int* idx_out, int* status, hipStream_t stream)
{
    launch_hog_packed<false>(imgs, img_idx, x, N, L, eyes, lv, plan, feat, ldf, idx_out, status, stream);
}

void sdm_launch_hog_cells(const ImageSetDev& imgs, const int* img_idx, const float* x, int N, int L,
                          const EyeIdxDev& eyes, const HogLevelDev& lv, const HogPlanDev& plan, float* cells,
                          int* idx_out, int* status, hipStream_t stream)
{
    launch_hog_packed<true>(imgs, img_idx, x, N, L, eyes, lv, plan, cells, 0, idx_out, status, stream);
}

bool sdm_hog_cells_row_carry(const HogLevelDev& lv, const HogPlanDev& plan)
{
    return lv.O == 4 && plan.raw_sqrt && plan.taps && hp_row_carry(lv.cell);
}

void sdm_launch_taps_table(const HogLevelDev& lv, int* table, hipStream_t stream)
{
    hipLaunchKernelGGL(taps_table_kernel, dim3(SDM_SCALE_TAB), dim3(64), 0, stream, lv, table);
}
```

superviseddescent_amd/csrc/sdm_kernels.h:

```cpp
#pragma once
#include <hip/hip_runtime.h>
#include <cstdio>
#include <stdint.h>

#define SDM_SCALE_TAB 128
#define SDM_MAX_ORIENT 16
#define SDM_MAX_EYE 4

struct HogLevelDev {
    int variant;
    int C;
    int cell;
    int O;
    int S;
    int D;
    int P;
    float rel;
    int fixed_h;
    float ox[SDM_MAX_ORIENT];
    float oy[SDM_MAX_ORIENT];
    int n_sector;
    float sector_t[SDM_MAX_ORIENT / 2];
    alignas(16) float row_tab[64][4];
    double scale_tab[SDM_SCALE_TAB];
// ... 14 lines not shown
    const int* stride;
    int n_images;
};

#define SDM_DEV_ERR_EMPTY_PATCH 1

size_t sdm_hog_lds_bytes(const HogLevelDev& lv, int waves_per_block);

void sdm_launch_hog(const ImageSetDev& imgs, const int* img_idx, const float* x, int N, int L,
                    const EyeIdxDev& eyes, const HogLevelDev& lv, float* feat, long long ldf,
                    int* idx_out, int* status, hipStream_t stream);

bool sdm_hog_fast_supported(const HogLevelDev& lv);
void sdm_launch_verify_fast_bins(const HogLevelDev& lv, int* mismatches_dev, hipStream_t stream);
void sdm_launch_taps_table(const HogLevelDev& lv, int* table, hipStream_t stream);
void sdm_launch_hog_fast(const ImageSetDev& imgs, const int* img_idx, const float* x, int N, int L,
                         const EyeIdxDev& eyes, const HogLevelDev& lv, float* feat, long long ldf, int* idx_out,
                         int* status, int acc_mode, int fast_bins, hipStream_t stream);

#define SDM_PLAN_MAX_SEG 3
struct HogPlanDev {
    int G, P, n_main, Gt, Pt;
    int hist_slots;
    int raw_sqrt;
    const unsigned* lane_tab;
    const float* wb;
    const unsigned short* wb16;
    const int* pass_info;
    const int* taps;
    int two_load;
};
__host__ __device__ constexpr int packed_band_of(int d, int cell)
{
    return (2 * d + 1 - cell >= 0) ? (2 * d + 1 - cell) / (2 * cell) : -1;
}
#ifdef __cplusplus
#include <vector>
struct HogPlanHost {
    int G = 0, P = 0, n_main = 0, Gt = 0, Pt = 0, hist_slots = 2;
    std::vector<unsigned> lane_tab;
    std::vector<float> wb;
    std::vector<unsigned short> wb16;
    std::vector<int> pass_info;
    std::vector<int> cut;
};
bool sdm_hog_plan_build(const HogLevelDev& lv, int L, HogPlanHost& out);
#endif
void sdm_launch_hog_packed(const ImageSetDev& imgs, const int* img_idx, const float* x, int N, int L,
                           const EyeIdxDev& eyes, const HogLevelDev& lv, const HogPlanDev& plan, float* feat, long long ldf,
                           int* idx_out, int* status, hipStream_t stream);

void sdm_launch_hog_cells(const ImageSetDev& imgs, const int* img_idx, const float* x, int N, int L,
                          const EyeIdxDev& eyes, const HogLevelDev& lv, const HogPlanDev& plan, float* cells,
                          int* idx_out, int* status, hipStream_t stream);
bool sdm_hog_cells_row_carry(const HogLevelDev& lv, const HogPlanDev& plan);

bool sdm_desc_supported(const HogLevelDev& lv);
size_t sdm_cells_floats(const HogLevelDev& lv, int N, int L);
void sdm_launch_desc_store(const HogLevelDev& lv, const float* cells, const int* cut, int N, int L, float* feat, long long ldf, hipStream_t stream);
size_t sdm_desc_planes_bytes(const HogLevelDev& lv, int L, int M);
void sdm_launch_desc_planes(const HogLevelDev& lv, const float* Rt, long long ldr, int L, int M, const unsigned* rmax, void* planes, hipStream_t stream);
void sdm_launch_desc_apply(const HogLevelDev& lv, const float* cells, const int* cut, int N, int L, int M, const void* planes,
                           const unsigned* rmax, const float* Rt, long long ldr, float* partial, hipStream_t stream);
void sdm_launch_apply_reduce(const float* partial, int splits, int N, int M, const float* x_in, float* x_out, int L,
                             const EyeIdxDev& eyes, hipStream_t stream);

size_t sdm_colpiv_qr_work_floats(int F);
bool sdm_colpiv_qr_supported(int F);
void sdm_launch_colpiv_qr_solve(float* G, long long ldg, int F, int rhs0, int nrhs, float* R_out, long long ldr, int r_rows,
                                float* work, int** rank_dev_out, hipStream_t stream);

void sdm_launch_hog_fast_profile(const ImageSetDev& imgs, const int* img_idx, const float* x, int N, int L,
                                 const EyeIdxDev& eyes, const HogLevelDev& lv, float* feat, long long ldf,
                                 int* status, unsigned long long* prof_dev, hipStream_t stream);

void sdm_launch_hog_debug(const ImageSetDev& imgs, const int* img_idx, const float* x, int N, int L,
                          const EyeIdxDev& eyes, const HogLevelDev& lv, int sample, int landmark,
                          uint8_t* rsz_out, uint8_t* bins_out, float* hist_out, float* desc_out,
                          int* status, hipStream_t stream);

void sdm_launch_gradient_table(const HogLevelDev& lv, float* g_out, int* bin_out, hipStream_t stream);

int sdm_apply_splits(int N, int F, int M);
void sdm_launch_apply(const float* feat, long long ldf, int N, int F, const float* Rt, long long ldr,
                      int M, const float* x_in, float* x_out, int L, const EyeIdxDev& eyes,
                      float* partial, int splits, hipStream_t stream, const void* planes = nullptr, const unsigned* rmax = nullptr);
size_t sdm_apply_planes_bytes(long long ldr, int M);
void sdm_launch_apply_planes(const float* Rt, long long ldr, int M, void* planes, unsigned* rmax, hipStream_t stream);

void sdm_launch_pack_regressor(const float* Rsol, int F, int M, int Mp, float* Rt, long long ldf, float* Rc, hipStream_t stream);
void sdm_launch_subtract_templates(float* feat, long long ldf, const float* tmpl, int N, int F, hipStream_t stream);

void sdm_launch_bgr2gray(const uint8_t* bgr, uint8_t* gray, long long n_pixels, int shift, hipStream_t stream);

void sdm_launch_init_boxes(const float* mean, const int* boxes, const float* pert, int N, int L, float* x, hipStream_t stream);
#define SDM_SUM_PARTS 256
void sdm_launch_landmark_errors(const float* x, const float* xstar, int N, int L, const EyeIdxDev& eyes, float* err,
                                double* work, hipStream_t stream);

void sdm_launch_targets(const float* x, const float* xstar, int N, int L, const EyeIdxDev& eyes,
                        float* feat, long long ldf, int bcol0, hipStream_t stream);

void sdm_launch_syrk_tn(const float* A, long long lda, int rows, int ncols, float* C, long long ldc,
                        float alpha, int accumulate, int tile_i0, hipStream_t stream, int tile_rows = 0, int own_rank = 0,
                        int own_world = 1);

size_t sdm_gram_bf16x3_plane_bytes(int N, int ncols, int pieces = 3);
void sdm_launch_gram_bf16x3(const float* A, long long lda, int N, int ncols, void* planes, float* C, long long ldc, hipStream_t stream,
                            int* f16_flag = nullptr);

void sdm_launch_gram_f16_split(const float* A, long long lda, int N, int ncols, void* planes, hipStream_t stream, int* f16_flag);
int sdm_launch_gram_f16_product(const void* planes, int N, int ncols, float* C, long long ldc, int j_lo, int j_hi, int order_off, hipStream_t stream);

size_t sdm_packed_tiles_count(int F, int rhs_tiles);
void sdm_launch_tiles_pack(float* G, long long ldg, int F, int rhs_tiles, float* P, int unpack, hipStream_t stream);
void sdm_launch_fro2_upper(const float* G, long long ldg, int F, double* part_and_out, hipStream_t stream, int own_rank = 0, int own_world = 1);
size_t sdm_owned_chunk_tiles(int F, int rhs_tiles, int W, int c_lo = 0, int c_hi = -1);
void sdm_launch_tiles_pack_owned(float* G, long long ldg, int F, int rhs_tiles, int W, int me, float* P, int unpack, hipStream_t stream,
// ... 100 lines not shown
```

Measured before the change: 3.855 million faces/s.

## Precompute per-face patch geometry in apply-reduce and skip device x copy

Adds a packed per-face geometry record (half-width, image offset, size, stride). The apply-reduce kernel now computes the next level's record from the freshly updated landmarks, and the HOG cells kernel reads it instead of recomputing the inter-eye distance and gathering image metadata per workgroup. Device-to-device x uploads are borrowed lazily rather than copied, with a handover kernel building level-0 geometry. This adds state-tracking complexity (materialise_x, geom_level invalidation), and the device-to-device set_x path no longer synchronises.

New measurement: 3.866 million faces/s, median of 6. Within noise of the previous version (+0.3%).

```diff
diff --git a/include/sdm.h b/include/sdm.h
--- a/include/sdm.h
+++ b/include/sdm.h
@@ -144,6 +144,7 @@
                        float* wb, int* pass_info, int max_passes);
 int sdm_debug_hog_plan_cut(int num_cells, int cell_size, int num_bins, int num_landmarks, int* cut);
 int sdm_debug_hog_taps(sdm_ctx* ctx, int level, int* table, int* info3);
+int sdm_debug_half_width_host(float relative_patch_size, int fixed_h, const double* ied, int n, int* h_out);
 int sdm_debug_set_detect_path(sdm_ctx* ctx, int fused, int split_store);
 
 int sdm_pose_set_model(sdm_ctx* ctx, const float* points, int K, float focal, float width, float height, float near_, float far_);
diff --git a/superviseddescent_amd/_lib.py b/superviseddescent_amd/_lib.py
--- a/superviseddescent_amd/_lib.py
+++ b/superviseddescent_amd/_lib.py
@@ -23,7 +23,7 @@
     "sdm_set_solve_sharding", "sdm_set_solve_sharding_rccl", "sdm_set_reduce_scatter", "sdm_set_reduce_scatter_rccl",
     "sdm_set_templates", "sdm_init_from_boxes", "sdm_normalised_errors", "sdm_solve", "sdm_set_solver", "sdm_last_rank", "sdm_solve_normal_equations", "sdm_solve_normal_equations_with", "sdm_train_level", "sdm_gram_device_ptr", "sdm_x_device_ptr", "sdm_features_device_ptr",
     "sdm_enable_timing", "sdm_get_timing", "sdm_debug_patch", "sdm_debug_hog_profile", "sdm_debug_gradient_table", "sdm_debug_update_f16", "sdm_debug_set_option",
-    "sdm_debug_set_hog_packing", "sdm_debug_gram_fallbacks", "sdm_debug_update_fallbacks", "sdm_debug_hog_plan", "sdm_debug_hog_plan_cut", "sdm_debug_hog_taps", "sdm_debug_set_detect_path", "sdm_upload_images_bgr_u8", "sdm_debug_download_images",
+    "sdm_debug_set_hog_packing", "sdm_debug_gram_fallbacks", "sdm_debug_update_fallbacks", "sdm_debug_hog_plan", "sdm_debug_hog_plan_cut", "sdm_debug_hog_taps", "sdm_debug_half_width_host", "sdm_debug_set_detect_path", "sdm_upload_images_bgr_u8", "sdm_debug_download_images",
     "sdm_pose_set_model", "sdm_pose_set_x", "sdm_pose_get_x", "sdm_pose_set_x_device", "sdm_pose_set_templates",
     "sdm_pose_templates_from_landmarks", "sdm_pose_set_targets", "sdm_pose_features", "sdm_pose_train_level",
     "sdm_pose_set_regressor", "sdm_pose_get_regressor", "sdm_pose_test",
@@ -156,6 +156,7 @@
             "sdm_debug_hog_plan": [c_int, c_int, c_int, c_int, c_int_p, c_void_p, c_void_p, c_void_p, c_int],
             "sdm_debug_hog_plan_cut": [c_int, c_int, c_int, c_int, c_int_p],
             "sdm_debug_hog_taps": [c_void_p, c_int, c_int_p, c_int_p],
+            "sdm_debug_half_width_host": [ctypes.c_float, c_int, ctypes.POINTER(ctypes.c_double), c_int, c_int_p],
             "sdm_debug_set_detect_path": [c_void_p, c_int, c_int],
             "sdm_pose_set_model": [c_void_p, c_void_p, c_int, ctypes.c_float, ctypes.c_float, ctypes.c_float, ctypes.c_float,
                                    ctypes.c_float],
diff --git a/superviseddescent_amd/csrc/sdm_apply.hip b/superviseddescent_amd/csrc/sdm_apply.hip
--- a/superviseddescent_amd/csrc/sdm_apply.hip
+++ b/superviseddescent_amd/csrc/sdm_apply.hip
@@ -3,6 +3,7 @@
 
 #pragma clang fp contract(off)
 #include "sdm_ied.h"
+#include "sdm_hog_device.h"
 
 namespace {
 
@@ -338,6 +339,44 @@
         for (int j = 0; j < RB; ++j) u = s0 + j < splits ? u + v[j] : u;
     }
     x_out[t] = xc - u * scale;
+}
+
+__global__ void apply_reduce_geom_kernel(const float* __restrict__ partial, int splits, int N, int Mp, int M,
+                                         const float* __restrict__ x_in, float* __restrict__ x_out, int L, EyeIdxDev eyes,
+                                         ImageSetDev imgs, const int* __restrict__ img_idx, float rel, int fixed_h,
+                                         geom_rec* __restrict__ geom)
+{
+    const int lane = threadIdx.x & 63;
+    const int row = (int)(blockIdx.x * (blockDim.x >> 6) + (threadIdx.x >> 6));
+    if (row >= N) return;
+    const int col = lane < M ? lane : M - 1;
+    const float* xr = x_in + (long long)row * M;
+    const float xc = xr[col];
+    float scale = 1.0f;
+    if (eyes.nre > 0) {
+        const float n = (float)(1.0 / device_ied_rows(xr, L, eyes));
+        scale = 1.0f / n;
+    }
+    float u = 0.0f;
+    const float* pp = partial + (long long)row * Mp + col;
+    const long long sstride = (long long)N * Mp;
+    constexpr int RB = 24;
+    for (int s0 = 0; s0 < splits; s0 += RB) {
+        float v[RB];
+#pragma unroll
+        for (int j = 0; j < RB; ++j) v[j] = pp[(long long)(s0 + j < splits ? s0 + j : splits - 1) * sstride];
+#pragma unroll
+        for (int j = 0; j < RB; ++j) u = s0 + j < splits ? u + v[j] : u;
+    }
+    const float xn = xc - u * scale;
+    if (lane < M) x_out[(long long)row * M + col] = xn;
+    float rx = 0.0f, ry = 0.0f, lx = 0.0f, ly = 0.0f;
+    if (fixed_h <= 0) {
+        for (int i = 0; i < eyes.nre; ++i) { rx += __shfl(xn, eyes.re[i]); ry += __shfl(xn, eyes.re[i] + L); }
+        for (int i = 0; i < eyes.nle; ++i) { lx += __shfl(xn, eyes.le[i]); ly += __shfl(xn, eyes.le[i] + L); }
+    }
+    if (lane == 0)
+        geom[row] = geom_of_face(imgs, img_idx, row, hog_half_width(rel, fixed_h, fixed_h > 0 ? 0.0 : ied_of_sums(rx, ry, lx, ly, eyes)));
 }
 
 __global__ void targets_kernel(const float* __restrict__ x, const float* __restrict__ xstar, int N, int L,
@@ -613,6 +652,15 @@
                        partial, splits, N, ((M + 15) / 16) * 16, M, x_in, x_out, L, eyes);
 }
 
+void sdm_launch_apply_reduce_geom(const float* partial, int splits, int N, int M, const float* x_in, float* x_out, int L,
+                                  const EyeIdxDev& eyes, const ImageSetDev& imgs, const int* img_idx, float rel, int fixed_h,
+                                  void* geom, hipStream_t stream)
+{
+    if (N <= 0 || M <= 0 || M > 64) return;
+    hipLaunchKernelGGL(apply_reduce_geom_kernel, dim3((unsigned)((N + 3) / 4)), dim3(256), 0, stream,
+                       partial, splits, N, ((M + 15) / 16) * 16, M, x_in, x_out, L, eyes, imgs, img_idx, rel, fixed_h, (geom_rec*)geom);
+}
+
 void sdm_launch_targets(const float* x, const float* xstar, int N, int L, const EyeIdxDev& eyes,
                         float* feat, long long ldf, int bcol0, hipStream_t stream)
 {
diff --git a/superviseddescent_amd/csrc/sdm_capi_align.hip b/superviseddescent_amd/csrc/sdm_capi_align.hip
--- a/superviseddescent_amd/csrc/sdm_capi_align.hip
+++ b/superviseddescent_amd/csrc/sdm_capi_align.hip
@@ -84,6 +84,7 @@
         src.ctx = image_set(c);
         img = c->img_base;
     }
+    { const int rcx = materialise_x(c); if (rcx) return rcx; }
     sdm_launch_align_fit(c->x[c->cur].p, N, L, a.in.p, (const float*)(a.in.p + K), K, src, c->idx_identity ? nullptr : c->img_idx.p,
                          out_w, out_h, a.faces.p, c->stream);
     HIP_TRY(hipGetLastError());
diff --git a/superviseddescent_amd/csrc/sdm_capi_context.hip b/superviseddescent_amd/csrc/sdm_capi_context.hip
--- a/superviseddescent_amd/csrc/sdm_capi_context.hip
+++ b/superviseddescent_amd/csrc/sdm_capi_context.hip
@@ -61,7 +61,7 @@
     drain_timing(c);
     for (auto ev : c->pool) { e = hipEventDestroy(ev); }
     c->img_owned.release(); c->img_off.release(); c->img_w.release(); c->img_h.release();
-    c->img_stride.release(); c->img_idx.release(); c->x[0].release(); c->x[1].release();
+    c->img_stride.release(); c->img_idx.release(); c->x[0].release(); c->x[1].release(); c->geom.release();
     c->xstar.release(); c->tmpl.release(); c->feat.release(); c->patch_idx.release(); c->status.release();
     c->partial.release(); c->shard_stage.release(); c->G.release(); c->gpack.release(); c->fro.release(); c->Rsol.release(); c->winv.release(); c->gram_planes.release(); c->gram_flag.release(); c->upd_planes.release(); c->upd_maxdiag.release(); c->lambda_dev.release();
     for (auto& r : c->Rp) r.release();
@@ -225,6 +225,7 @@
     c->have_R.assign(n_levels, false);
     c->feat.release(); c->feat_level = -1; c->feat_wide_F = 0; c->feat_wide_N = 0; c->have_patch_idx = false;
     c->N = 0; c->have_targets = false; c->g_level = -1;
+    c->x_borrowed = nullptr; c->geom_level = -1;
     c->sweep.K = 0; c->sweep.level = -1; c->sweep.ok = 0;
     return SDM_OK;
 }
@@ -287,6 +288,7 @@
     c->img_w_host.assign(w, w + n); c->img_h_host.assign(h, h + n);
     c->narrow_images = false;
     for (int i = 0; i < n; ++i) c->narrow_images = c->narrow_images || w[i] < 2 || h[i] > 65535;
+    images_changed(c, 0, total);
     return SDM_OK;
 }
 
@@ -333,6 +335,7 @@
     c->img_w_host.assign(w, w + n); c->img_h_host.assign(h, h + n);
     c->narrow_images = false;
     for (int i = 0; i < n; ++i) c->narrow_images = c->narrow_images || w[i] < 2 || h[i] > 65535;
+    images_changed(c, 0, total);
     return SDM_OK;
 }
 
@@ -364,12 +367,14 @@
     c->n_images = n;
     c->img_w_host.assign(n, w); c->img_h_host.assign(n, h);
     c->narrow_images = w < 2 || h > 65535;
+    images_changed(c, stride, (long long)n * h * stride);
     return SDM_OK;
 }
 
 int sdm_set_sample_image_index(sdm_ctx* c, const int* idx, int n)
 {
     if (!c) return fail(SDM_ERR_INVALID, "null context");
+    c->geom_level = -1;
     if (!idx) { c->idx_identity = true; c->n_idx = 0; c->max_idx = -1; return SDM_OK; }
     if (n <= 0) return fail(SDM_ERR_INVALID, "bad sample count");
     int mx = -1;
@@ -396,8 +401,19 @@
     if (rc) return rc;
     if (N != c->N) { c->have_targets = false; c->feat_level = -1; c->have_patch_idx = false; }
     c->N = N; c->cur = 0;
+    c->x_borrowed = nullptr; c->geom_level = -1;
+    if (kind == hipMemcpyDeviceToDevice) {
+        c->x_borrowed = x;
+        if (!c->levels.empty() && geom_level_ok(c, 0) && c->img_base && check_sample_index(c) == SDM_OK &&
+            (c->levels[0].fixed_h > 0 || (c->eyes.nre > 0 && c->eyes.nle > 0))) {
+            sdm_launch_handover(image_set(c), c->idx_identity ? nullptr : c->img_idx.p, x, N, c->L, c->eyes, c->levels[0], c->geom.p, c->stream);
+            HIP_TRY(hipGetLastError());
+            c->geom_level = 0;
+        }
+        return SDM_OK;
+    }
     HIP_TRY(hipMemcpyAsync(c->x[0].p, x, (size_t)N * c->M * sizeof(float), kind, c->stream));
-    if (kind == hipMemcpyHostToDevice) HIP_TRY(hipStreamSynchronize(c->stream));
+    HIP_TRY(hipStreamSynchronize(c->stream));
     return SDM_OK;
 }
 
@@ -435,6 +451,7 @@
         HIP_TRY(hipMemcpyAsync(d_pert.p, perturbations, (size_t)3 * N * sizeof(float), hipMemcpyHostToDevice, c->stream));
     if (N != c->N) { c->have_targets = false; c->feat_level = -1; c->have_patch_idx = false; }
     c->N = N; c->cur = 0;
+    c->x_borrowed = nullptr; c->geom_level = -1;
     sdm_launch_init_boxes(d_mean.p, d_box.p, perturbations ? d_pert.p : nullptr, N, c->L, c->x[0].p, c->stream);
     HIP_TRY(hipGetLastError());
     if (x_host)
@@ -453,6 +470,7 @@
     ScopedBuf<float> d_err;
     ScopedBuf<double> d_work;
     int rc;
+    if ((rc = materialise_x(c))) return rc;
     if ((rc = d_err.ensure((size_t)c->N * c->L)) || (rc = d_work.ensure(SDM_SUM_PARTS + 2))) return rc;
     sdm_launch_landmark_errors(c->x[c->cur].p, c->xstar.p, c->N, c->L, c->eyes, d_err.p, d_work.p, c->stream);
     HIP_TRY(hipGetLastError());
@@ -469,6 +487,7 @@
 int sdm_get_x(sdm_ctx* c, float* x)
 {
     if (!c || !x || c->N <= 0) return fail(SDM_ERR_INVALID, "no x to get");
+    { const int rcx = materialise_x(c); if (rcx) return rcx; }
     HIP_TRY(hipMemcpyAsync(x, c->x[c->cur].p, (size_t)c->N * c->M * sizeof(float), hipMemcpyDeviceToHost, c->stream));
     HIP_TRY(hipStreamSynchronize(c->stream));
     return check_status(c);
@@ -477,6 +496,7 @@
 int sdm_get_x_device(sdm_ctx* c, float* x)
 {
     if (!c || !x || c->N <= 0) return fail(SDM_ERR_INVALID, "no x to get");
+    { const int rcx = materialise_x(c); if (rcx) return rcx; }
     HIP_TRY(hipMemcpyAsync(x, c->x[c->cur].p, (size_t)c->N * c->M * sizeof(float), hipMemcpyDeviceToDevice, c->stream));
     return SDM_OK;
 }
diff --git a/superviseddescent_amd/csrc/sdm_capi_debug.hip b/superviseddescent_amd/csrc/sdm_capi_debug.hip
--- a/superviseddescent_amd/csrc/sdm_capi_debug.hip
+++ b/superviseddescent_amd/csrc/sdm_capi_debug.hip
@@ -1,4 +1,5 @@
 #include "sdm_capi_internal.h"
+#include "sdm_hog_device.h"
 
 extern "C" {
 
@@ -12,6 +13,8 @@
 int sdm_x_device_ptr(sdm_ctx* c, void** p, size_t* count)
 {
     if (!c || c->N <= 0) return fail(SDM_ERR_INVALID, "no x");
+    { const int rcx = materialise_x(c); if (rcx) return rcx; }
+    c->geom_level = -1;
     *p = c->x[c->cur].p; *count = (size_t)c->N * c->M;
     return SDM_OK;
 }
@@ -56,6 +59,7 @@
     ScopedBuf<uint8_t> d_r, d_b; ScopedBuf<float> d_h, d_d;
     int rc;
     if ((rc = d_r.ensure(nS)) || (rc = d_b.ensure(nS)) || (rc = d_h.ensure(nH)) || (rc = d_d.ensure(nP))) return rc;
+    { const int rcx = materialise_x(c); if (rcx) return rcx; }
     sdm_launch_hog_debug(image_set(c), c->idx_identity ? nullptr : c->img_idx.p, c->x[c->cur].p, c->N, c->L,
                          c->eyes, lv, sample, landmark, d_r.p, d_b.p, d_h.p, d_d.p, c->status.p, c->stream);
     HIP_TRY(hipGetLastError());
@@ -77,6 +81,7 @@
     ScopedBuf<unsigned long long> d;
     int rc = d.ensure(8, true, c->stream);
     if (rc) return rc;
+    { const int rcx = materialise_x(c); if (rcx) return rcx; }
     sdm_launch_hog_fast_profile(image_set(c), c->idx_identity ? nullptr : c->img_idx.p, c->x[c->cur].p, c->N, c->L,
                                 c->eyes, c->levels[level], c->feat.p, c->ldf, c->status.p, d.p, c->stream);
     HIP_TRY(hipGetLastError());
@@ -137,6 +142,13 @@
     HogPlanHost hp;
     if (!sdm_hog_plan_build(lv, num_landmarks, hp)) return fail(SDM_ERR_INVALID, "no packed instance for this geometry");
     memcpy(cut, hp.cut.data(), (size_t)num_landmarks * sizeof(int));
+    return SDM_OK;
+}
+
+int sdm_debug_half_width_host(float relative_patch_size, int fixed_h, const double* ied, int n, int* h_out)
+{
+    if (!ied || !h_out || n < 0) return fail(SDM_ERR_INVALID, "bad arguments");
+    for (int i = 0; i < n; ++i) h_out[i] = hog_half_width(relative_patch_size, fixed_h, ied[i]);
     return SDM_OK;
 }
 
diff --git a/superviseddescent_amd/csrc/sdm_capi_detect.hip b/superviseddescent_amd/csrc/sdm_capi_detect.hip
--- a/superviseddescent_amd/csrc/sdm_capi_detect.hip
+++ b/superviseddescent_amd/csrc/sdm_capi_detect.hip
@@ -69,7 +69,26 @@
         c->feat_level = -1; c->feat_wide_F = 0; c->feat_wide_N = 0;
     }
     if ((rc = c->patch_idx.ensure((size_t)N * (1 + 2 * c->L)))) return rc;
-    return SDM_OK;
+    if ((rc = c->geom.ensure((size_t)N * 4))) return rc;
+    return SDM_OK;
+}
+
+int materialise_x(sdm_ctx* c)
+{
+    if (!c->x_borrowed) return SDM_OK;
+    HIP_TRY(hipSetDevice(c->device));
+    HIP_TRY(hipMemcpyAsync(c->x[0].p, c->x_borrowed, (size_t)c->N * c->M * sizeof(float), hipMemcpyDeviceToDevice, c->stream));
+    c->x_borrowed = nullptr;
+    c->ev_fresh = false;
+    return SDM_OK;
+}
+
+void images_changed(sdm_ctx* c, int max_stride, long long total_bytes)
+{
+    c->geom_level = -1;
+    bool ok = total_bytes < (1ll << 47) && max_stride <= 65535;
+    for (size_t i = 0; i < c->img_w_host.size() && ok; ++i) ok = c->img_w_host[i] <= 65535 && c->img_h_host[i] <= 65535;
+    c->geom_packable = ok;
 }
 
 int check_sample_index(const sdm_ctx* c)
@@ -89,6 +108,7 @@
            c->fast_bins[level] == 2 && c->plans[level].ok;
 }
 bool split_ok(const sdm_ctx* c, int level) { return packed_ok(c, level) && sdm_desc_supported(c->levels[level]); }
+bool geom_level_ok(const sdm_ctx* c, int level) { return c->geom_packable && c->M <= 64 && split_ok(c, level); }
 
 int hog_checks(sdm_ctx* c, int level)
 {
@@ -118,6 +138,7 @@
 int do_hog(sdm_ctx* c, int level)
 {
     { const int rci = hog_checks(c, level); if (rci) return rci; }
+    { const int rcx = materialise_x(c); if (rcx) return rcx; }
     if (c->feat_wide_F > level_F(c, level)) {
         const size_t rows = (size_t)(c->feat_wide_N > c->N ? c->feat_wide_N : c->N);
         HIP_TRY(hipMemsetAsync(c->feat.p, 0, rows * c->ldf * sizeof(float), c->stream));
@@ -179,6 +200,8 @@
     const int splits = sdm_apply_splits(c->N, F, c->M);
     int rc = c->partial.ensure((size_t)splits * c->N * Mp_of(c->M));
     if (rc) return rc;
+    if ((rc = materialise_x(c))) return rc;
+    c->geom_level = -1;
     {
         Timer t(c, SDM_T_APPLY);
         sdm_launch_apply(c->feat.p, c->ldf, c->N, F, c->Rt[level].p, c->ldf, c->M, c->x[c->cur].p,
@@ -205,19 +228,32 @@
     for (size_t q = 0; q < c->levels.size(); ++q) { const size_t n = sdm_cells_floats(c->levels[q], c->N, c->L); if (n > cells_max) cells_max = n; }
     if ((rc = c->cells.ensure(cells_max)) || (rc = c->partial.ensure((size_t)c->L * c->N * Mp))) return rc;
     const HogLevelDev& lv = c->levels[l];
+    if (!c->in_detect_batch || l != 0) { if ((rc = materialise_x(c))) return rc; }
+    const float* x_in = c->x_borrowed ? c->x_borrowed : c->x[c->cur].p;
+    const int* idx = c->idx_identity ? nullptr : c->img_idx.p;
+    const bool recs = c->in_detect_batch && c->geom_level == l && geom_level_ok(c, l);
+    const int ln = l + 1;
+    const bool recs_next = c->in_detect_batch && ln < (int)c->levels.size() && fused_ok(c, ln) && geom_level_ok(c, ln) &&
+                           (c->levels[ln].fixed_h > 0 || (c->eyes.nre > 0 && c->eyes.nle > 0));
     {
         Timer t(c, SDM_T_HOG);
-        sdm_launch_hog_cells(image_set(c), c->idx_identity ? nullptr : c->img_idx.p, c->x[c->cur].p, c->N, c->L, c->eyes, lv,
-                             cells_plan(c, l), c->cells.p, c->patch_idx.p, c->status.p, c->stream);
+        sdm_launch_hog_cells(image_set(c), idx, x_in, c->N, c->L, c->eyes, lv,
+                             cells_plan(c, l), c->cells.p, c->patch_idx.p, c->status.p, c->stream, recs ? c->geom.p : nullptr);
     }
     {
         Timer t(c, SDM_T_APPLY);
         sdm_launch_desc_apply(lv, c->cells.p, c->plans[l].cut.p, c->N, c->L, c->M, c->Rd[l].p, c->Rmax.p + (size_t)l * Mp,
                               c->Rt[l].p, c->ldf, c->partial.p, c->stream);
-        sdm_launch_apply_reduce(c->partial.p, c->L, c->N, c->M, c->x[c->cur].p, c->x[c->cur ^ 1].p, c->L, c->eyes, c->stream);
+        if (recs_next)
+            sdm_launch_apply_reduce_geom(c->partial.p, c->L, c->N, c->M, x_in, c->x[c->cur ^ 1].p, c->L, c->eyes, image_set(c), idx,
+                                         c->levels[ln].rel, c->levels[ln].fixed_h, c->geom.p, c->stream);
+        else
+            sdm_launch_apply_reduce(c->partial.p, c->L, c->N, c->M, x_in, c->x[c->cur ^ 1].p, c->L, c->eyes, c->stream);
     }
     HIP_TRY(hipGetLastError());
     c->cur ^= 1;
+    c->x_borrowed = nullptr;
+    c->geom_level = recs_next ? ln : -1;
     c->feat_level = -1;
     c->have_patch_idx = true;
     return SDM_OK;
@@ -301,7 +337,9 @@
     HIP_TRY(hipSetDevice(c->device));
     c->chain_timers = true; c->ev_fresh = false;
     int rc = SDM_OK;
+    c->in_detect_batch = true;
     for (int l = 0; l < (int)c->levels.size() && !rc; ++l) rc = detect_level(c, l);
+    c->in_detect_batch = false;
     c->chain_timers = false; c->ev_fresh = false;
     if (rc) return rc;
     if (x_host) return sdm_get_x(c, x_host);
diff --git a/superviseddescent_amd/csrc/sdm_capi_internal.h b/superviseddescent_amd/csrc/sdm_capi_internal.h
--- a/superviseddescent_amd/csrc/sdm_capi_internal.h
+++ b/superviseddescent_amd/csrc/sdm_capi_internal.h
@@ -114,6 +114,11 @@
     int N = 0;
     DevBuf<float> x[2];
     int cur = 0;
+    const float* x_borrowed = nullptr;
+    DevBuf<int> geom;
+    int geom_level = -1;
+    bool geom_packable = false;
+    bool in_detect_batch = false;
     DevBuf<float> xstar;
     DevBuf<float> tmpl;
     int tmpl_F = 0, tmpl_N = 0;
@@ -277,6 +282,9 @@
 int check_status(sdm_ctx* c);
 ImageSetDev image_set(const sdm_ctx* c);
 int ensure_sample_buffers(sdm_ctx* c, int N);
+int materialise_x(sdm_ctx* c);
+void images_changed(sdm_ctx* c, int max_stride, long long total_bytes);
+bool geom_level_ok(const sdm_ctx* c, int level);
 int check_sample_index(const sdm_ctx* c);
 bool packed_ok(const sdm_ctx* c, int level);
 bool split_ok(const sdm_ctx* c, int level);
diff --git a/superviseddescent_amd/csrc/sdm_capi_pose.hip b/superviseddescent_amd/csrc/sdm_capi_pose.hip
--- a/superviseddescent_amd/csrc/sdm_capi_pose.hip
+++ b/superviseddescent_amd/csrc/sdm_capi_pose.hip
@@ -105,6 +105,7 @@
     sdm_ctx::Pose& p = c->pose;
     if ((rc = p.lm.ensure((size_t)K)) || (rc = p.tmpl.ensure((size_t)c->N * 2 * K))) return rc;
     HIP_TRY(hipMemcpyAsync(p.lm.p, landmark_index, (size_t)K * sizeof(int), hipMemcpyHostToDevice, c->stream));
+    { const int rcx = materialise_x(c); if (rcx) return rcx; }
     sdm_launch_pose_gather(c->x[c->cur].p, c->L, c->N, p.lm.p, K, c->idx_identity ? nullptr : c->img_idx.p, c->img_w.p, c->img_h.p, focal,
                            p.tmpl.p, c->stream);
     HIP_TRY(hipGetLastError());
diff --git a/superviseddescent_amd/csrc/sdm_capi_sweep.hip b/superviseddescent_amd/csrc/sdm_capi_sweep.hip
--- a/superviseddescent_amd/csrc/sdm_capi_sweep.hip
+++ b/superviseddescent_amd/csrc/sdm_capi_sweep.hip
@@ -75,6 +75,7 @@
         sdm_launch_pack_regressor(c->Rsol.p, F, M, Mp, Rt_k, c->ldf, nullptr, c->stream);
         sdm_launch_apply_planes(Rt_k, c->ldf, M, Rp_k, Rmax_k, c->stream);
         {
+            { const int rcx = materialise_x(c); if (rcx) return rcx; }
             Timer t(c, SDM_T_APPLY);
             sdm_launch_apply(c->feat.p, c->ldf, N, F, Rt_k, c->ldf, M, c->x[c->cur].p, sw.x.p, c->L, c->eyes, c->partial.p, splits, c->stream,
                              planes ? Rp_k : nullptr, planes ? Rmax_k : nullptr);
diff --git a/superviseddescent_amd/csrc/sdm_capi_track.hip b/superviseddescent_amd/csrc/sdm_capi_track.hip
--- a/superviseddescent_amd/csrc/sdm_capi_track.hip
+++ b/superviseddescent_amd/csrc/sdm_capi_track.hip
@@ -131,7 +131,7 @@
         (rc = t.masks.ensure((size_t)n + 1)) || (rc = ensure_pinned(t, (size_t)2 * n + 1)))
         return rc;
     if (n != c->N) { c->have_targets = false; c->feat_level = -1; c->have_patch_idx = false; }
-    c->N = n; c->cur = 0;
+    c->N = n; c->cur = 0; c->x_borrowed = nullptr; c->geom_level = -1;
     memcpy(t.pin, ids, (size_t)n * sizeof(int));
     HIP_TRY(hipMemcpyAsync(t.ids.p, t.pin, (size_t)n * sizeof(int), hipMemcpyHostToDevice, c->stream));
     sdm_launch_track_gather(t.ids.p, n, c->L, t.mode, t.status.p, t.box.p, t.x.p, t.mean.p, t.mean_bounds, c->x[0].p, t.init.p, c->stream);
diff --git a/superviseddescent_amd/csrc/sdm_capi_train.hip b/superviseddescent_amd/csrc/sdm_capi_train.hip
--- a/superviseddescent_amd/csrc/sdm_capi_train.hip
+++ b/superviseddescent_amd/csrc/sdm_capi_train.hip
@@ -21,6 +21,7 @@
     c->g_scattered = false;
     c->gram_blocks = 0;
     Timer t(c, SDM_T_GRAM);
+    { const int rcx = materialise_x(c); if (rcx) return rcx; }
     HIP_TRY(hipMemset2DAsync(c->feat.p + Fp, (size_t)c->ldf * sizeof(float), 0, 128 * c->rhs_tiles * sizeof(float), c->N, c->stream));
     sdm_launch_targets(c->x[c->cur].p, c->xstar.p, c->N, c->L, c->eyes, c->feat.p, c->ldf, Fp, c->stream);
     const bool gram_f32 = c->env_gram_f32, gram_bf16 = c->env_gram_bf16;
diff --git a/superviseddescent_amd/csrc/sdm_hog_device.h b/superviseddescent_amd/csrc/sdm_hog_device.h
--- a/superviseddescent_amd/csrc/sdm_hog_device.h
+++ b/superviseddescent_amd/csrc/sdm_hog_device.h
@@ -8,16 +8,38 @@
 typedef float f32x2 __attribute__((ext_vector_type(2)));
 typedef float f32x4 __attribute__((ext_vector_type(4)));
 
+__device__ inline double ied_of_sums(float rx, float ry, float lx, float ly, const EyeIdxDev& e)
+{
+    if (e.inv_nre != 0.0f) { rx *= e.inv_nre; ry *= e.inv_nre; } else { rx /= (float)e.nre; ry /= (float)e.nre; }
+    if (e.inv_nle != 0.0f) { lx *= e.inv_nle; ly *= e.inv_nle; } else { lx /= (float)e.nle; ly /= (float)e.nle; }
+    float dxf = rx - lx, dyf = ry - ly;
+    double dx = dxf, dy = dyf;
+    return sqrt(dx * dx + dy * dy);
+}
+
 __device__ inline double ied_of(const float* __restrict__ xr, int L, const EyeIdxDev& e)
 {
     float rx = 0.0f, ry = 0.0f, lx = 0.0f, ly = 0.0f;
     for (int i = 0; i < e.nre; ++i) { rx += xr[e.re[i]]; ry += xr[e.re[i] + L]; }
-    if (e.inv_nre != 0.0f) { rx *= e.inv_nre; ry *= e.inv_nre; } else { rx /= (float)e.nre; ry /= (float)e.nre; }
     for (int i = 0; i < e.nle; ++i) { lx += xr[e.le[i]]; ly += xr[e.le[i] + L]; }
-    if (e.inv_nle != 0.0f) { lx *= e.inv_nle; ly *= e.inv_nle; } else { lx /= (float)e.nle; ly /= (float)e.nle; }
-    float dxf = rx - lx, dyf = ry - ly;
-    double dx = dxf, dy = dyf;
-    return sqrt(dx * dx + dy * dy);
+    return ied_of_sums(rx, ry, lx, ly, e);
+}
+
+__host__ __device__ inline int hog_half_width(float rel, int fixed_h, double ied)
+{
+    return fixed_h > 0 ? fixed_h : (int)round((double)rel * ied / 2);
+}
+
+typedef int geom_rec __attribute__((ext_vector_type(4)));
+__device__ inline geom_rec geom_pack(int h, long long off, int iw, int ih, int istride)
+{
+    return (geom_rec){h, (int)(unsigned)(off & 0xffffffffll), (int)((unsigned)((off >> 32) & 0xffff) | ((unsigned)ih << 16)),
+                      (int)((unsigned)iw | ((unsigned)istride << 16))};
+}
+__device__ inline geom_rec geom_of_face(const ImageSetDev& imgs, const int* __restrict__ img_idx, int s, int h)
+{
+    const int im = img_idx ? img_idx[s] : s;
+    return geom_pack(h, imgs.offset[im], imgs.w[im], imgs.h[im], imgs.stride[im]);
 }
 
 __device__ inline int sat_short_f(float v)
diff --git a/superviseddescent_amd/csrc/sdm_hog_packed.hip b/superviseddescent_amd/csrc/sdm_hog_packed.hip
--- a/superviseddescent_amd/csrc/sdm_hog_packed.hip
+++ b/superviseddescent_amd/csrc/sdm_hog_packed.hip
@@ -115,7 +115,7 @@
 __global__ void __launch_bounds__(HP_WAVES * 64, CELLS ? HP_MINW_CELLS : HP_MINW)
 hog_packed_kernel(ImageSetDev imgs, const int* __restrict__ img_idx, const float* __restrict__ x, int N, int L,
                   EyeIdxDev eyes, HogLevelDev lv, HogPlanDev plan, float* __restrict__ feat, long long ldf,
-                  int* __restrict__ idx_out, int* __restrict__ status)
+                  int* __restrict__ idx_out, int* __restrict__ status, const geom_rec* __restrict__ geom)
 {
     extern __shared__ __attribute__((aligned(16))) unsigned char smem[];
     constexpr int O = TO, C = TC, CC = C * C;
@@ -153,18 +153,28 @@
     unsigned char* scratch = lds;
     auto hist_slot = [&](int patch_slot) { return nslots == 2 ? (patch_slot & 1) : patch_slot % 3; };
 
-    const int im = uni(img_idx ? img_idx[s] : s);
     const float* xr = x + (long long)s * 2 * L;
     float* out_row = feat + (long long)s * ldf;
     int* idx_row = idx_out ? idx_out + (long long)s * (1 + 2 * L) : nullptr;
 
-    const int h = lv.fixed_h > 0 ? lv.fixed_h : uni((int)round((double)lv.rel * ied_of(xr, L, eyes) / 2));
+    int h, iw, ih, istride;
+    const uint8_t* img;
+    if (CELLS && geom) {
+        const geom_rec gr = geom[s];
+        h = uni(gr.x);
+        img = imgs.base + (long long)(((unsigned long long)(unsigned)uni(gr.z & 0xffff) << 32) | (unsigned)uni(gr.y));
+        ih = uni((int)((unsigned)gr.z >> 16));
+        iw = uni(gr.w & 0xffff); istride = uni((int)((unsigned)gr.w >> 16));
+    } else {
+        const int im = uni(img_idx ? img_idx[s] : s);
+        h = uni(hog_half_width(lv.rel, lv.fixed_h, lv.fixed_h > 0 ? 0.0 : ied_of(xr, L, eyes)));
+        img = imgs.base + imgs.offset[im];
+        iw = imgs.w[im]; ih = imgs.h[im]; istride = imgs.stride[im];
+    }
     const bool empty = h <= 0;
     if (empty && lane == 0) atomicOr(status, SDM_DEV_ERR_EMPTY_PATCH);
     const int sw = empty ? 1 : 2 * h;
     const bool area2 = (sw == 2 * S);
-    const uint8_t* img = imgs.base + imgs.offset[im];
-    const int iw = imgs.w[im], ih = imgs.h[im], istride = imgs.stride[im];
     const __amdgpu_buffer_rsrc_t img_rsrc = __builtin_amdgcn_make_buffer_rsrc((void*)img, 0, ih * istride, 0x00020000);
 
     int tab_s, tab_w;
@@ -541,7 +551,7 @@
 template <bool CELLS>
 static void launch_hog_packed(const ImageSetDev& imgs, const int* img_idx, const float* x, int N, int L,
                               const EyeIdxDev& eyes, const HogLevelDev& lv, const HogPlanDev& plan, float* feat, long long ldf,
-                              int* idx_out, int* status, hipStream_t stream)
+                              int* idx_out, int* status, const geom_rec* geom, hipStream_t stream)
 {
     const int gpf = CELLS ? plan.n_main * plan.P + plan.Pt : plan.n_main + (plan.Gt > 0 ? 1 : 0);
     const long long total = (long long)N * gpf;
@@ -550,7 +560,7 @@
 #define HP_LAUNCH_O(TO, CELL, RAW)                                                                                              \
     hipLaunchKernelGGL((hog_packed_kernel<TO, 5, CELL, RAW, CELLS>), dim3(grid), dim3(HP_WAVES * 64),                              \
                        packed_wg_lds_bytes(5, TO, lv.S, CELLS ? 0 : plan.hist_slots, CELL > 0), stream, imgs, img_idx, x, N, L,  \
-                       eyes, lv, plan, feat, ldf, idx_out, status)
+                       eyes, lv, plan, feat, ldf, idx_out, status, geom)
 #define HP_LAUNCH(CELL, RAW) HP_LAUNCH_O(4, CELL, RAW)
     if (lv.O == 9) {
         static unsigned long long attr9 = 0;
@@ -577,14 +587,33 @@
                            const EyeIdxDev& eyes, const HogLevelDev& lv, const HogPlanDev& plan, float* feat, long long ldf,
                            int* idx_out, int* status, hipStream_t stream)
 {
-    launch_hog_packed<false>(imgs, img_idx, x, N, L, eyes, lv, plan, feat, ldf, idx_out, status, stream);
+    launch_hog_packed<false>(imgs, img_idx, x, N, L, eyes, lv, plan, feat, ldf, idx_out, status, nullptr, stream);
 }
 
 void sdm_launch_hog_cells(const ImageSetDev& imgs, const int* img_idx, const float* x, int N, int L,
                           const EyeIdxDev& eyes, const HogLevelDev& lv, const HogPlanDev& plan, float* cells,
-                          int* idx_out, int* status, hipStream_t stream)
-{
-    launch_hog_packed<true>(imgs, img_idx, x, N, L, eyes, lv, plan, cells, 0, idx_out, status, stream);
+                          int* idx_out, int* status, hipStream_t stream, const void* geom)
+{
+    launch_hog_packed<true>(imgs, img_idx, x, N, L, eyes, lv, plan, cells, 0, idx_out, status, (const geom_rec*)geom, stream);
+}
+
+namespace {
+__global__ void handover_kernel(ImageSetDev imgs, const int* __restrict__ img_idx, const float* __restrict__ x, int N, int L,
+                                EyeIdxDev eyes, float rel, int fixed_h, geom_rec* __restrict__ geom)
+{
+    const int s = blockIdx.x * blockDim.x + threadIdx.x;
+    if (s >= N) return;
+    const int h = hog_half_width(rel, fixed_h, fixed_h > 0 ? 0.0 : ied_of(x + (long long)s * 2 * L, L, eyes));
+    geom[s] = geom_of_face(imgs, img_idx, s, h);
+}
+}
+
+void sdm_launch_handover(const ImageSetDev& imgs, const int* img_idx, const float* x, int N, int L, const EyeIdxDev& eyes,
+                         const HogLevelDev& lv0, void* geom, hipStream_t stream)
+{
+    if (N <= 0) return;
+    hipLaunchKernelGGL(handover_kernel, dim3((unsigned)((N + 255) / 256)), dim3(256), 0, stream, imgs, img_idx, x, N, L, eyes,
+                       lv0.rel, lv0.fixed_h, (geom_rec*)geom);
 }
 
 bool sdm_hog_cells_row_carry(const HogLevelDev& lv, const HogPlanDev& plan)
diff --git a/superviseddescent_amd/csrc/sdm_kernels.h b/superviseddescent_amd/csrc/sdm_kernels.h
--- a/superviseddescent_amd/csrc/sdm_kernels.h
+++ b/superviseddescent_amd/csrc/sdm_kernels.h
@@ -90,7 +90,9 @@
 
 void sdm_launch_hog_cells(const ImageSetDev& imgs, const int* img_idx, const float* x, int N, int L,
                           const EyeIdxDev& eyes, const HogLevelDev& lv, const HogPlanDev& plan, float* cells,
-                          int* idx_out, int* status, hipStream_t stream);
+                          int* idx_out, int* status, hipStream_t stream, const void* geom = nullptr);
+void sdm_launch_handover(const ImageSetDev& imgs, const int* img_idx, const float* x, int N, int L, const EyeIdxDev& eyes,
+                         const HogLevelDev& lv0, void* geom, hipStream_t stream);
 bool sdm_hog_cells_row_carry(const HogLevelDev& lv, const HogPlanDev& plan);
 
 bool sdm_desc_supported(const HogLevelDev& lv);
@@ -102,6 +104,9 @@
                            const unsigned* rmax, const float* Rt, long long ldr, float* partial, hipStream_t stream);
 void sdm_launch_apply_reduce(const float* partial, int splits, int N, int M, const float* x_in, float* x_out, int L,
                              const EyeIdxDev& eyes, hipStream_t stream);
+void sdm_launch_apply_reduce_geom(const float* partial, int splits, int N, int M, const float* x_in, float* x_out, int L,
+                                  const EyeIdxDev& eyes, const ImageSetDev& imgs, const int* img_idx, float rel, int fixed_h,
+                                  void* geom, hipStream_t stream);
 
 size_t sdm_colpiv_qr_work_floats(int F);
 bool sdm_colpiv_qr_supported(int F);
```
